# KarypisLab/SLIM

Measured on AMD Instinct MI355X. Metric: item-columns solved/sec (whole node), higher is better.
Workload: dtype f32

## Files before the change

### include/slim_gpu.h

```cpp
#ifndef SLIM_AMD_SLIM_GPU_H_
#define SLIM_AMD_SLIM_GPU_H_

#include "slim.h"

#ifdef __cplusplus
extern "C" {
#endif

typedef struct slim_csr_t {
  int32_t nrows, ncols;
  ssize_t *rowptr, *colptr;
  int32_t *rowind, *colind;
  int32_t *rowids, *colids;
  int32_t *rlabels, *clabels;
  int32_t *rmap, *cmap;
  float *rowval, *colval;
  float *rnorms, *cnorms;
  float *rsums, *csums;
  float *rsizes, *csizes;
  float *rvols, *cvols;
  float *rwgts, *cwgts;
} slim_csr_t;


// ... 61 lines not shown
                                           const int64_t *d_rowptr,
                                           const int32_t *d_rowind,
                                           const float *d_rowval,
                                           int32_t *ioptions, int32_t *r_status);
void SLIMGPU_MatrixFree(slimgpu_matrix_t **mat);
int32_t SLIMGPU_MatrixInfo(const slimgpu_matrix_t *mat, int32_t *nrows,
                           int32_t *ncols, int64_t *nnz);
int32_t SLIMGPU_MatrixGetColumnView(const slimgpu_matrix_t *mat, int64_t *colptr,
                                    int32_t *colind, float *colval,
                                    float *cnorms);

void SLIMGPU_MatrixExpectSolves(slimgpu_matrix_t *mat, int32_t nsolves);
int32_t SLIMGPU_MatrixDevice(const slimgpu_matrix_t *mat);

int32_t SLIMGPU_MatrixGramBuildRows(slimgpu_matrix_t *mat, int32_t row_begin, int32_t row_end);
int32_t SLIMGPU_MatrixGramView(slimgpu_matrix_t *mat, void **dptr, int64_t *ld, int32_t *nrows);
int32_t SLIMGPU_MatrixGramCommit(slimgpu_matrix_t *mat);

int32_t SLIMGPU_MatrixColumnCost(const slimgpu_matrix_t *mat, int64_t *cost);

slim_t *SLIMGPU_Learn(slimgpu_matrix_t *mat, int32_t *ioptions,
                      double *doptions, slim_t *imodel, int32_t *r_status);

slim_t *SLIMGPU_LearnColumns(slimgpu_matrix_t *mat, int32_t ncolumns,
                             const int32_t *columns, int32_t *ioptions,
                             double *doptions, slim_t *imodel, int32_t *r_status);

typedef struct slimgpu_model slimgpu_model_t;
slimgpu_model_t *SLIMGPU_LearnResident(slimgpu_matrix_t *mat, int32_t *ioptions, double *doptions,
                                       const slimgpu_model_t *warm, int32_t *r_status);
int64_t SLIMGPU_ModelNnz(const slimgpu_model_t *model);
int32_t SLIMGPU_ModelFetchBegin(slimgpu_model_t *model);
slim_t *SLIMGPU_ModelFetch(slimgpu_model_t *model, int32_t *r_status);
void SLIMGPU_ModelFree(slimgpu_model_t **model);
int32_t SLIMGPU_ModelPredict(int32_t nrcmds, const slimgpu_model_t *model, slim_t *trnhandle,
                             int32_t *output, float *scores);

int32_t SLIMGPU_Predict(int32_t nrcmds, slim_t *slimhandle, slim_t *trnhandle,
                        int32_t *output, float *scores);

int32_t SLIMGPU_Predict1vsK(int32_t nrcmds, int32_t nnegs, slim_t *slimhandle,
                            slim_t *trnhandle, int32_t *negitems, int32_t *output,
                            float *scores);

int32_t SLIMGPU_Evaluate(int32_t nusers, int32_t nrcmds, const int32_t *lists,
                         const int32_t *counts, slim_t *tsthandle,
                         const int32_t *fmarker, int32_t fm_ncols, double *metrics,
                         int32_t *nvalid);

typedef struct slimgpu_stats_t {
  int32_t ncols_solved;
  int32_t kernel;
  int32_t nwaves;
  int32_t lds_bytes;
  double setup_ms;
  double kernel_ms;
  double gather_ms;
  double total_ms;
  int64_t G, D, U, nnzW;
  int64_t sweeps;
  int64_t visits;
  double alg_bytes;
  double error, objval;
  double gram_build_ms;
  int64_t gram_rows;
  double gram_bytes;
  double gram_alloc_ms, gram_sums_ms, gram_sums_kernel_ms, gram_pack_ms;
} slimgpu_stats_t;
int32_t SLIMGPU_LastStats(slimgpu_stats_t *out);

int32_t SLIMGPU_LastColumnStats(int32_t ncols, int32_t *nacols, int32_t *sweeps,
                                int32_t *conv, int64_t *G, int64_t *D,
                                int64_t *U);

int32_t SLIMGPU_DeviceCount(void);
const char *SLIMGPU_LastError(void);

#ifdef __cplusplus
}
#endif

#include "slim_gpu_eval.h"
#include "slim_gpu_planes.h"
#include "slim_gpu_rank.h"
#include "slim_gpu_lists.h"
#include "slim_gpu_filter.h"
#include "slim_gpu_cand.h"

#endif
```

### slim_amd/_lib.py

```python
import ctypes as C
import os

import numpy as np

_HERE = os.path.dirname(os.path.abspath(__file__))
LIB_PATH = os.environ.get("SLIM_AMD_LIB") or os.path.join(_HERE, "libslim.so")

f64_1d = np.ctypeslib.ndpointer(dtype=np.float64, ndim=1, flags="C_CONTIGUOUS")
f32_1d = np.ctypeslib.ndpointer(dtype=np.float32, ndim=1, flags="C_CONTIGUOUS")
i32_1d = np.ctypeslib.ndpointer(dtype=np.int32, ndim=1, flags="C_CONTIGUOUS")
i64_1d = np.ctypeslib.ndpointer(dtype=np.int64, ndim=1, flags="C_CONTIGUOUS")
isz_1d = np.ctypeslib.ndpointer(dtype=np.intp, ndim=1, flags="C_CONTIGUOUS")


class Stats(C.Structure):
    _fields_ = [("ncols_solved", C.c_int32), ("kernel", C.c_int32), ("nwaves", C.c_int32),
                ("lds_bytes", C.c_int32), ("setup_ms", C.c_double), ("kernel_ms", C.c_double),
                ("gather_ms", C.c_double), ("total_ms", C.c_double),
                ("G", C.c_int64), ("D", C.c_int64), ("U", C.c_int64), ("nnzW", C.c_int64),
                ("sweeps", C.c_int64), ("visits", C.c_int64), ("alg_bytes", C.c_double),
                ("error", C.c_double), ("objval", C.c_double), ("gram_build_ms", C.c_double),
                ("gram_rows", C.c_int64), ("gram_bytes", C.c_double),
                ("gram_alloc_ms", C.c_double), ("gram_sums_ms", C.c_double),
                ("gram_sums_kernel_ms", C.c_double), ("gram_pack_ms", C.c_double)]

    def as_dict(self):
        return {k: getattr(self, k) for k, _ in self._fields_}


class EvalStats(C.Structure):
    _fields_ = [("path", C.c_int32), ("device_allocs", C.c_int32), ("h2d_bytes", C.c_int64),
                ("d2h_bytes", C.c_int64), ("kernel_ms", C.c_double), ("total_ms", C.c_double),
                ("w_rows_read", C.c_int64), ("w_bytes", C.c_double)]

    def as_dict(self):
        return {k: getattr(self, k) for k, _ in self._fields_}


class CsrView(C.Structure):
    _fields_ = ([("nrows", C.c_int32), ("ncols", C.c_int32),
                 ("rowptr", C.POINTER(C.c_ssize_t)), ("colptr", C.POINTER(C.c_ssize_t)),
                 ("rowind", C.POINTER(C.c_int32)), ("colind", C.POINTER(C.c_int32))] +
                [(n, C.POINTER(C.c_int32)) for n in
                 ("rowids", "colids", "rlabels", "clabels", "rmap", "cmap")] +
                [(n, C.POINTER(C.c_float)) for n in
                 ("rowval", "colval", "rnorms", "cnorms", "rsums", "csums", "rsizes",
                  "csizes", "rvols", "cvols", "rwgts", "cwgts")])


_SIGNATURES = {
    "SLIM_iSetDefaults": (C.c_int32, [i32_1d]),
    "SLIM_dSetDefaults": (C.c_int32, [f64_1d]),
    "SLIM_Learn": (C.c_void_p, [C.c_int32, isz_1d, i32_1d, C.c_void_p, C.c_void_p, C.c_void_p,
                                C.c_void_p, C.POINTER(C.c_int32)]),
    "SLIM_GetTopN": (C.c_int32, [C.c_void_p, C.c_int32, i32_1d, C.c_void_p, C.c_void_p,
                                 C.c_int32, i32_1d, f32_1d]),
    "SLIM_WriteModel": (C.c_int32, [C.c_void_p, C.c_char_p]),
    "SLIM_ReadModel": (C.c_void_p, [C.c_char_p]),
    "SLIM_FreeModel": (None, [C.POINTER(C.c_void_p)]),
    "SLIM_DetermineHeadAndTail": (C.POINTER(C.c_int32), [C.c_int32, C.c_int32, isz_1d, i32_1d]),
    "Py_csr_wrapper": (C.c_int32, [C.c_int32, isz_1d, i32_1d, C.c_void_p, C.c_void_p]),
    "Py_csr_save": (C.c_int32, [C.c_void_p, C.c_char_p]),
    "Py_csr_load": (C.c_int32, [C.c_void_p, C.c_char_p]),
    "Py_csr_free": (C.c_int32, [C.c_void_p]),
    "Py_csr_stat": (C.c_int32, [C.c_void_p, C.c_void_p]),
    "Py_csr_export": (C.c_int32, [C.c_void_p, i32_1d, i32_1d, f32_1d]),
    "Py_SLIM_Learn": (C.c_int32, [C.c_void_p, i32_1d, f64_1d, C.c_void_p]),
    "Py_SLIM_Mselect": (C.c_int32, [C.c_void_p, C.c_void_p, i32_1d, f64_1d, f64_1d, f64_1d,
                                    C.c_int32, C.c_int32] + [C.c_void_p] * 8),
    "Py_SLIM_GetTopN": (C.c_int32, [C.c_void_p, C.c_int32, i32_1d, C.c_void_p, C.c_int32,
                                    i32_1d, f32_1d, C.c_int32]),
    "Py_SLIM_GetTopN_1vsk": (C.c_int32, [C.c_void_p, C.c_int32, i32_1d, C.c_void_p, C.c_int32,
                                         i32_1d, f32_1d, C.c_int32, i32_1d, C.c_int32]),
    "Py_SLIM_Predict": (C.c_int32, [C.c_int32, C.c_void_p, C.c_void_p, i32_1d, f32_1d]),
    "Py_SLIM_Predict_1vsk": (C.c_int32, [C.c_int32, C.c_int32, C.c_void_p, C.c_void_p, i32_1d,
                                         i32_1d, f32_1d]),
    "SLIMGPU_MatrixFromHost": (C.c_void_p, [C.c_int32, isz_1d, i32_1d, C.c_void_p, C.c_void_p,
                                            C.POINTER(C.c_int32)]),
    "SLIMGPU_MatrixFromDevice": (C.c_void_p, [C.c_int32, C.c_int32, C.c_void_p, C.c_void_p,
                                              C.c_void_p, C.c_void_p, C.POINTER(C.c_int32)]),
    "SLIMGPU_MatrixFree": (None, [C.POINTER(C.c_void_p)]),
    "SLIMGPU_MatrixInfo": (C.c_int32, [C.c_void_p, C.POINTER(C.c_int32), C.POINTER(C.c_int32),
                                       C.POINTER(C.c_int64)]),
    "SLIMGPU_MatrixGetColumnView": (C.c_int32, [C.c_void_p] * 5),
    "SLIMGPU_MatrixColumnCost": (C.c_int32, [C.c_void_p, C.c_void_p]),
    "SLIMGPU_MatrixExpectSolves": (None, [C.c_void_p, C.c_int32]),
    "SLIMGPU_MatrixDevice": (C.c_int32, [C.c_void_p]),
    "SLIMGPU_MatrixGramBuildRows": (C.c_int32, [C.c_void_p, C.c_int32, C.c_int32]),
    "SLIMGPU_MatrixGramView": (C.c_int32, [C.c_void_p, C.POINTER(C.c_void_p), C.POINTER(C.c_int64),
                                           C.POINTER(C.c_int32)]),
    "SLIMGPU_MatrixGramCommit": (C.c_int32, [C.c_void_p]),
    "SLIMGPU_Learn": (C.c_void_p, [C.c_void_p, C.c_void_p, C.c_void_p, C.c_void_p,
                                   C.POINTER(C.c_int32)]),
    "SLIMGPU_LearnResident": (C.c_void_p, [C.c_void_p, C.c_void_p, C.c_void_p, C.c_void_p,
                                           C.POINTER(C.c_int32)]),
    "SLIMGPU_ModelNnz": (C.c_int64, [C.c_void_p]),
    "SLIMGPU_ModelFetchBegin": (C.c_int32, [C.c_void_p]),
    "SLIMGPU_ModelFetch": (C.c_void_p, [C.c_void_p, C.POINTER(C.c_int32)]),
    "SLIMGPU_ModelFree": (None, [C.POINTER(C.c_void_p)]),
    "SLIMGPU_ModelPredict": (C.c_int32, [C.c_int32, C.c_void_p, C.c_void_p, C.c_void_p, C.c_void_p]),
    "SLIMGPU_LearnColumns": (C.c_void_p, [C.c_void_p, C.c_int32, i32_1d, C.c_void_p, C.c_void_p,
                                          C.c_void_p, C.POINTER(C.c_int32)]),
    "SLIMGPU_Predict": (C.c_int32, [C.c_int32, C.c_void_p, C.c_void_p, i32_1d, f32_1d]),
    "SLIMGPU_Predict1vsK": (C.c_int32, [C.c_int32, C.c_int32, C.c_void_p, C.c_void_p, i32_1d,
                                        i32_1d, f32_1d]),
    "SLIMGPU_Evaluate": (C.c_int32, [C.c_int32, C.c_int32, i32_1d, i32_1d, C.c_void_p, i32_1d,
                                     C.c_int32, f64_1d, i32_1d]),
    "SLIMGPU_LastStats": (C.c_int32, [C.POINTER(Stats)]),
    "SLIMGPU_LastColumnStats": (C.c_int32, [C.c_int32] + [C.c_void_p] * 6),
    "SLIMGPU_DeviceCount": (C.c_int32, []),
    "SLIMGPU_LastError": (C.c_char_p, []),
}

EXPORTED_SYMBOLS = tuple(_SIGNATURES)

_EVAL_SIGNATURES = {
    "SLIMGPU_EvalSetCreate": (C.c_void_p, [C.c_void_p, C.c_void_p, i32_1d, C.c_int32, C.c_int32,
                                           C.POINTER(C.c_int32)]),
    "SLIMGPU_EvalSetFree": (None, [C.POINTER(C.c_void_p)]),
    "SLIMGPU_ModelEvaluate": (C.c_int32, [C.c_void_p, C.c_void_p, f64_1d, i32_1d]),
    "SLIMGPU_MatrixPredict": (C.c_int32, [C.c_int32, C.c_void_p, C.c_void_p, i32_1d, f32_1d]),
    "SLIMGPU_LastEvalStats": (C.c_int32, [C.POINTER(EvalStats)]),
}

EVAL_SYMBOLS = tuple(_EVAL_SIGNATURES)

_EVAL_AT_SIGNATURES = {
    "SLIMGPU_EvalSetCreateAt": (C.c_void_p, [C.c_void_p, C.c_void_p, i32_1d, C.c_int32, C.c_int32, C.c_void_p,
                                             C.c_int32, C.c_void_p, C.POINTER(C.c_int32)]),
    "SLIMGPU_ModelEvaluateAt": (C.c_int32, [C.c_void_p, C.c_void_p, C.c_int32, f64_1d, i32_1d]),
}

EVAL_AT_SYMBOLS = tuple(_EVAL_AT_SIGNATURES)


class GramPlanes(C.Structure):
    _fields_ = ([("ncols", C.c_int32), ("nchunks", C.c_int32), ("ldb", C.c_int64), ("hi_bytes", C.c_int64)] +
                [(n, C.c_void_p) for n in ("lo", "base", "hi", "hi_off", "hi_k", "hi2_k", "diag", "meta",
                                           "rank_of", "item_of")])


_PLANES_SIGNATURES = {
    "SLIMGPU_MatrixGramPlanes": (C.c_int32, [C.c_void_p, C.POINTER(GramPlanes)]),
}

PLANES_SYMBOLS = tuple(_PLANES_SIGNATURES)
MAX_CUTOFFS = 8

_RANK_SIGNATURES = {
    "SLIMGPU_EvalSetCreateRanked": (C.c_void_p, [C.c_void_p, C.c_void_p, i32_1d, C.c_int32, C.c_int32, C.c_void_p,
                                                 C.POINTER(C.c_int32)]),
    "SLIMGPU_EvalSetEntries": (C.c_int64, [C.c_void_p]),
    "SLIMGPU_ModelRanks": (C.c_int32, [C.c_void_p, C.c_void_p, C.c_void_p, C.c_void_p]),
    "SLIMGPU_ModelEvaluateRanked": (C.c_int32, [C.c_void_p, C.c_void_p, C.c_int32, C.c_void_p, f64_1d, i32_1d]),
    "SLIMGPU_ModelFromHost": (C.c_void_p, [C.c_void_p, C.c_void_p, C.POINTER(C.c_int32)]),
    "SLIMGPU_LastRankPrepassMs": (C.c_double, []),
}

RANK_SYMBOLS = tuple(_RANK_SIGNATURES)
MAX_RANK_CUTOFFS = 32


class ListStats(C.Structure):
    _fields_ = [("path", C.c_int32), ("slices", C.c_int32), ("candidates", C.c_int64), ("contenders", C.c_int64),
                ("refine_passes", C.c_int64), ("lds_sorts", C.c_int64), ("key_refines", C.c_int64)]

    def as_dict(self):
        return {k: getattr(self, k) for k, _ in self._fields_}


_LIST_SIGNATURES = {
    "SLIMGPU_PredictLists": (C.c_int32, [C.c_int32, C.c_void_p, C.c_void_p, C.c_void_p, C.c_void_p, C.c_void_p]),
    "SLIMGPU_ModelPredictLists": (C.c_int32, [C.c_int32, C.c_void_p, C.c_void_p, C.c_void_p, C.c_void_p,
                                              C.c_void_p]),
    "SLIMGPU_MatrixPredictLists": (C.c_int32, [C.c_int32, C.c_void_p, C.c_void_p, C.c_int32, C.c_void_p,
                                               C.c_void_p, C.c_void_p, C.c_void_p]),
    "SLIMGPU_LastListStats": (C.c_int32, [C.POINTER(ListStats)]),
}

LIST_SYMBOLS = tuple(_LIST_SIGNATURES)
MAX_LIST = 4096

_FILTER_SIGNATURES = {
    "SLIMGPU_FilterCreate": (C.c_int32, [C.c_int32, C.c_int32, C.c_void_p, C.c_int32, C.c_int32, C.c_void_p,
                                         C.c_void_p, C.POINTER(C.c_void_p)]),
    "SLIMGPU_FilterFree": (None, [C.c_void_p]),
    "SLIMGPU_PredictListsFiltered": (C.c_int32, [C.c_int32, C.c_void_p, C.c_void_p, C.c_void_p, C.c_void_p,
                                                 C.c_void_p, C.c_void_p]),
    "SLIMGPU_ModelPredictListsFiltered": (C.c_int32, [C.c_int32, C.c_void_p, C.c_void_p, C.c_void_p, C.c_void_p,
                                                      C.c_void_p, C.c_void_p]),
    "SLIMGPU_MatrixPredictListsFiltered": (C.c_int32, [C.c_int32, C.c_void_p, C.c_void_p, C.c_int32, C.c_void_p,
                                                       C.c_void_p, C.c_void_p, C.c_void_p, C.c_void_p]),
    "Py_SLIM_PredictFiltered": (C.c_int32, [C.c_int32, C.c_void_p, C.c_void_p, C.c_void_p, i32_1d, f32_1d]),
}

FILTER_SYMBOLS = tuple(_FILTER_SIGNATURES)

_FILTERED_EVAL_SIGNATURES = {
    "SLIMGPU_ModelEvaluateAtFiltered": (C.c_int32, [C.c_void_p, C.c_void_p, C.c_void_p, C.c_int32, f64_1d, i32_1d]),
    "SLIMGPU_ModelRanksFiltered": (C.c_int32, [C.c_void_p, C.c_void_p, C.c_void_p, C.c_void_p, C.c_void_p]),
    "SLIMGPU_ModelEvaluateRankedFiltered": (C.c_int32, [C.c_void_p, C.c_void_p, C.c_void_p, C.c_int32, C.c_void_p,
                                                        f64_1d, i32_1d]),
    "Py_SLIM_MselectFiltered": (C.c_int32, [C.c_void_p, C.c_void_p, i32_1d, f64_1d, f64_1d, f64_1d,
                                            C.c_int32, C.c_int32] + [C.c_void_p] * 9),
}

FILTERED_EVAL_SYMBOLS = tuple(_FILTERED_EVAL_SIGNATURES)

_CAND_SIGNATURES = {
    "SLIMGPU_CandSetCreate": (C.c_int32, [C.c_int32, C.c_int32, C.c_void_p, C.c_void_p, C.POINTER(C.c_void_p)]),
    "SLIMGPU_CandSetFree": (None, [C.c_void_p]),
    "SLIMGPU_ScoreCandidates": (C.c_int32, [C.c_void_p, C.c_void_p, C.c_void_p, C.c_int32, C.c_void_p, C.c_void_p,
                                            C.c_void_p, C.c_void_p]),
    "SLIMGPU_MatrixScoreCandidates": (C.c_int32, [C.c_void_p, C.c_void_p, C.c_void_p, C.c_int32, C.c_void_p,
                                                  C.c_int32, C.c_void_p, C.c_void_p, C.c_void_p, C.c_void_p]),
    "SLIMGPU_ModelEvaluateCandidates": (C.c_int32, [C.c_void_p, C.c_void_p, C.c_void_p, C.c_int32, f64_1d, i32_1d]),
    "Py_SLIM_ScoreCandidates": (C.c_int32, [C.c_void_p, C.c_void_p, C.c_void_p, C.c_int32, C.c_void_p, C.c_void_p,
                                            C.c_void_p, C.c_void_p]),
}

CAND_SYMBOLS = tuple(_CAND_SIGNATURES)

_SAMPLE_SIGNATURES = {
    "SLIMGPU_EvalSetSampleCandidates": (C.c_int32, [C.c_void_p, C.c_int32, C.c_uint64, C.POINTER(C.c_void_p)]),
    "SLIMGPU_CandSetSample": (C.c_int32, [C.c_int32, C.c_void_p, C.c_void_p, C.c_int32, C.c_void_p, C.c_int32,
                                          C.c_uint64, C.POINTER(C.c_void_p)]),
    "SLIMGPU_CandSetRows": (C.c_int32, [C.c_void_p, C.c_void_p, C.c_void_p]),
    "SLIMGPU_CandSetInfo": (C.c_int32, [C.c_void_p, C.POINTER(C.c_int32), C.POINTER(C.c_int32),
                                        C.POINTER(C.c_int64)]),
}

SAMPLE_SYMBOLS = tuple(_SAMPLE_SIGNATURES)

_WSAMPLE_SIGNATURES = {
    "SLIMGPU_EvalSetSampleCandidatesWeighted": (C.c_int32, [C.c_void_p, C.c_int32, C.c_uint64, C.c_void_p,
                                                            C.POINTER(C.c_void_p)]),
    "SLIMGPU_CandSetSampleWeighted": (C.c_int32, [C.c_int32, C.c_void_p, C.c_void_p, C.c_int32, C.c_void_p, C.c_int32,
                                                  C.c_uint64, C.c_void_p, C.POINTER(C.c_void_p)]),
    "SLIMGPU_LastSampleKernelMs": (C.c_double, []),
}

WSAMPLE_SYMBOLS = tuple(_WSAMPLE_SIGNATURES)

_EXPLAIN_SIGNATURES = {
    "SLIMGPU_ExplainCandidates": (C.c_int32, [C.c_void_p, C.c_void_p, C.c_void_p, C.c_int32, C.c_void_p, C.c_void_p,
                                              C.c_void_p]),
    "SLIMGPU_MatrixExplainCandidates": (C.c_int32, [C.c_void_p, C.c_void_p, C.c_void_p, C.c_int32, C.c_void_p,
                                                    C.c_int32, C.c_void_p, C.c_void_p, C.c_void_p]),
    "Py_SLIM_ExplainCandidates": (C.c_int32, [C.c_void_p, C.c_void_p, C.c_void_p, C.c_int32, C.c_void_p, C.c_void_p,
                                              C.c_void_p]),
}

EXPLAIN_SYMBOLS = tuple(_EXPLAIN_SIGNATURES)
MAX_WHY = 16

_lib = None


def load():
    global _lib
    if _lib is not None:
        return _lib
    if not os.path.exists(LIB_PATH):
        raise RuntimeError(
            "slim_amd: %s is missing -- build it with `python -c 'import __graft_entry__ as g; "
            "g.build()'` (hipcc, gfx950). There is no CPU fallback for SLIM training." % LIB_PATH)
    lib = C.CDLL(LIB_PATH)
    for name, (res, args) in (list(_SIGNATURES.items()) + list(_EVAL_SIGNATURES.items()) +
                              list(_EVAL_AT_SIGNATURES.items()) + list(_PLANES_SIGNATURES.items()) +
                              list(_RANK_SIGNATURES.items()) + list(_LIST_SIGNATURES.items()) +
                              list(_FILTER_SIGNATURES.items()) + list(_FILTERED_EVAL_SIGNATURES.items()) +
                              list(_CAND_SIGNATURES.items()) + list(_SAMPLE_SIGNATURES.items()) +
                              list(_WSAMPLE_SIGNATURES.items()) + list(_EXPLAIN_SIGNATURES.items())):
        if os.environ.get("SLIM_AMD_LIB") and not hasattr(lib, name):
            continue
        fn = getattr(lib, name)
        fn.restype = res
        fn.argtypes = args
    _lib = lib
    return lib


def last_error():
    msg = load().SLIMGPU_LastError()
    return msg.decode("utf-8", "replace") if msg else ""
```

### slim_amd/csrc/admm.hip

```cpp
#include <dlfcn.h>
#include <hip/hip_runtime.h>

#include <cstdio>
#include <cstdlib>
#include <chrono>
#include <cstring>
#include <mutex>
#include <string>
#include <vector>

#include "engine.hpp"
#include "hip_check.hpp"
#include "host_csr.hpp"

namespace slimamd {

namespace {

struct DenseLibs {
  void* blas = nullptr;
  int (*create_handle)(void**) = nullptr;
  int (*destroy_handle)(void*) = nullptr;
  int (*set_stream)(void*, hipStream_t) = nullptr;
  int (*dgemm)(void*, int, int, int, int, int, const double*, const double*, int, const double*,
// ... 134 lines not shown
  const int64_t nwaves = ((int64_t)gridDim.x * blockDim.x) >> 6;
  for (int64_t i = wave; i < m; i += nwaves) {
    int64_t n = 0;
    for (int j = lane; j < m; j += 64) n += W[i * m + j] > 0.0 ? 1 : 0;
    for (int off = 32; off > 0; off >>= 1) n += __shfl_xor(n, off);
    if (lane == 0) cnt[i] = n;
  }
}

__global__ void k_emit_rows(int32_t m, const double* __restrict__ W, const int64_t* __restrict__ ptr,
                            int32_t* __restrict__ ind, float* __restrict__ val) {
  const int lane = threadIdx.x & 63;
  const uint64_t lane_lt = (1ull << lane) - 1ull;
  const int64_t wave = ((int64_t)blockIdx.x * blockDim.x + threadIdx.x) >> 6;
  const int64_t nwaves = ((int64_t)gridDim.x * blockDim.x) >> 6;
  for (int64_t i = wave; i < m; i += nwaves) {
    int64_t at = ptr[i];
    for (int jb = 0; jb < m; jb += 64) {
      const int j = jb + lane;
      const double w = j < m ? W[i * m + j] : 0.0;
      const uint64_t mask = __ballot(w > 0.0);
      if (w > 0.0) {
        const int64_t dst = at + __popcll(mask & lane_lt);
        ind[dst] = j;
        val[dst] = (float)w;
      }
      at += __popcll(mask);
    }
  }
}

int grid_for(int64_t n, int block, int cap) {
  int64_t g = (n + block - 1) / block;
  if (g < 1) g = 1;
  if (g > cap) g = cap;
  return (int)g;
}

}

slim_csr_t* learn_admm(int32_t nrows, const ssize_t* rowptr, const int32_t* rowind,
                       const float* rowval, const LearnOptions& opt, int32_t* status) {
  auto fail = [&](int32_t code, const std::string& msg) -> slim_csr_t* {
    set_error(msg);
    if (status) *status = code;
    return nullptr;
  };
  if (nrows < 0 || !rowptr || (rowptr[nrows] > 0 && !rowind))
    return fail(SLIM_ERROR_INPUT, "SLIM_Learn(admm): bad CSR arguments");
  const int64_t nnz = rowptr[nrows];
  int32_t m = max_index_plus_one(nnz, rowind);
  if (m <= 0) m = 1;
  for (int64_t k = 0; k < nnz; ++k)
    if (rowind[k] < 0) return fail(SLIM_ERROR_INPUT, "SLIM_Learn(admm): negative item id");
  const int64_t n2 = (int64_t)m * m;
  {
    std::vector<int32_t> seen((size_t)m, -1);
    for (int32_t u = 0; u < nrows; ++u) {
      if (rowptr[u] > rowptr[u + 1] || rowptr[u] < 0 || rowptr[u + 1] > nnz)
        return fail(SLIM_ERROR_INPUT, "SLIM_Learn(admm): rowptr is not a non-decreasing offset array ending at nnz");
      for (ssize_t k = rowptr[u]; k < rowptr[u + 1]; ++k) {
        if (seen[(size_t)rowind[k]] == u)
          return fail(SLIM_ERROR_INPUT, "SLIM_Learn(admm): duplicate (user, item) entries in the rating matrix");
        seen[(size_t)rowind[k]] = u;
      }
    }
  }
  std::printf("Learning the model using ADMM... \n");
  std::fflush(stdout);
  const bool trace = std::getenv("SLIM_GPU_TRACE") != nullptr;
  const auto t_begin = std::chrono::steady_clock::now();
  auto mark = [&](const char* what) {
    if (trace)
      std::fprintf(stderr, "[trace] admm %-28s %8.1f ms\n", what,
                   std::chrono::duration<double, std::milli>(std::chrono::steady_clock::now() - t_begin).count());
  };
  try {
    (void)hipGetLastError();
    int ndev = 0;
    HIP_TRY(hipGetDeviceCount(&ndev));
    if (ndev <= 0) throw HipFail{hipErrorNoDevice, "hipGetDeviceCount"};
    if (opt.device >= 0) HIP_TRY(hipSetDevice(opt.device));
    size_t free_b = 0, total_b = 0;
    HIP_TRY(hipMemGetInfo(&free_b, &total_b));
    if ((double)n2 * 8.0 * 6.5 > (double)free_b)
      return fail(SLIM_ERROR_MEMORY, "SLIM_Learn(admm): six " + std::to_string(m) + " x " +
                                         std::to_string(m) + " fp64 matrices do not fit this GPU");
    static DenseLibs libs;
    static std::once_flag once;
    static bool loaded = false;
    static std::string load_err;
    std::call_once(once, [&]() { loaded = libs.load(&load_err); });
    if (!loaded) return fail(SLIM_ERROR, "SLIM_Learn: " + load_err);
    mark("libraries resolved");
    hipDeviceProp_t prop;
    int dev = 0;
    HIP_TRY(hipGetDevice(&dev));
    HIP_TRY(hipGetDeviceProperties(&prop, dev));
    const int cap = prop.multiProcessorCount * 8;
    hipStream_t st = nullptr;
    HIP_TRY(hipStreamCreateWithFlags(&st, hipStreamNonBlocking));
    void* handle = nullptr;
    if (libs.create_handle(&handle) != 0) {
      (void)hipStreamDestroy(st);
      return fail(SLIM_ERROR, "SLIM_Learn(admm): rocblas_create_handle failed");
    }
    libs.set_stream(handle, st);
    mark("rocblas handle");
    struct Cleanup {
      DenseLibs& l;
      void* h;
      hipStream_t s;
      ~Cleanup() {
        l.destroy_handle(h);
        (void)hipStreamDestroy(s);
      }
    } cleanup{libs, handle, st};

    DeviceBuffer<int64_t> d_ptr((size_t)nrows + 1), d_cnt((size_t)m + 1);
    DeviceBuffer<int32_t> d_ind((size_t)nnz), d_info(1);
    DeviceBuffer<float> d_val(rowval ? (size_t)nnz : 1);
    static_assert(sizeof(ssize_t) == sizeof(int64_t), "LP64 expected");
    HIP_TRY(hipMemcpyAsync(d_ptr.get(), rowptr, sizeof(int64_t) * ((size_t)nrows + 1), hipMemcpyHostToDevice, st));
    if (nnz) {
      HIP_TRY(hipMemcpyAsync(d_ind.get(), rowind, sizeof(int32_t) * (size_t)nnz, hipMemcpyHostToDevice, st));
      if (rowval)
        HIP_TRY(hipMemcpyAsync(d_val.get(), rowval, sizeof(float) * (size_t)nnz, hipMemcpyHostToDevice, st));
    }
    DeviceBuffer<double> T((size_t)n2), A((size_t)n2), P((size_t)n2), W((size_t)n2), C((size_t)n2), gam((size_t)m);
    HIP_TRY(hipMemsetAsync(T.get(), 0, sizeof(double) * (size_t)n2, st));
    HIP_TRY(hipMemsetAsync(W.get(), 0, sizeof(double) * (size_t)n2, st));
    HIP_TRY(hipMemsetAsync(C.get(), 0, sizeof(double) * (size_t)n2, st));

    const double rho = 10000.0;
    const int maxiters = 30;
    hipLaunchKernelGGL(k_gram_dense, dim3(grid_for((int64_t)nrows * 64, 256, cap)), dim3(256), 0, st,
                       nrows, m, d_ptr.get(), d_ind.get(), rowval ? d_val.get() : nullptr, T.get());
    HIP_TRY(hipGetLastError());
    hipLaunchKernelGGL(k_copy_add_diag, dim3(grid_for(n2, 256, cap)), dim3(256), 0, st, n2, m, T.get(), P.get(),
                       opt.l2r + rho);
    HIP_TRY(hipGetLastError());
    const double one = 1.0, zero = 0.0, minus_one = -1.0;
    HIP_TRY(hipMemsetAsync(d_info.get(), 0, sizeof(int32_t), st));
    for (int32_t k = 0; k < m; k += kNB) {
      const int32_t kb = std::min(kNB, m - k), rest = m - k - kb;
      double* Akk = P.get() + (int64_t)k * m + k;
      hipLaunchKernelGGL(k_potf2, dim3(1), dim3(kNB), 0, st, kb, k, m, Akk, d_info.get());
      if (rest > 0) {
        double* A21 = Akk + kb;
        double* A22 = Akk + (int64_t)kb * m + kb;
        if (libs.dtrsm(handle, kSideRight, kFillLower, kOpTrans, kNonUnit, rest, kb, &one, Akk, m, A21, m) != 0 ||
            libs.dsyrk(handle, kFillLower, kOpNone, rest, kb, &minus_one, A21, m, &one, A22, m) != 0)
          return fail(SLIM_ERROR, "SLIM_Learn(admm): rocBLAS dtrsm / dsyrk failed");
      }
    }
    HIP_TRY(hipGetLastError());
    int32_t info = 0;
    HIP_TRY(hipMemcpyAsync(&info, d_info.get(), sizeof(int32_t), hipMemcpyDeviceToHost, st));
    HIP_TRY(hipStreamSynchronize(st));
    if (info != 0) return fail(SLIM_ERROR, "SLIM_Learn(admm): R^T R + (l2 + rho) I is not positive definite");
    mark("R^T R + Cholesky");
    hipLaunchKernelGGL(k_identity, dim3(grid_for(n2, 256, cap)), dim3(256), 0, st, n2, m, W.get());
    if (libs.dtrsm(handle, kSideLeft, kFillLower, kOpNone, kNonUnit, m, m, &one, P.get(), m, W.get(), m) != 0 ||
        libs.dgemm(handle, kOpTrans, kOpNone, m, m, m, &one, W.get(), m, W.get(), m, &zero, P.get(), m) != 0)
      return fail(SLIM_ERROR, "SLIM_Learn(admm): rocBLAS dtrsm / dgemm failed");
    HIP_TRY(hipMemsetAsync(W.get(), 0, sizeof(double) * (size_t)n2, st));
    hipLaunchKernelGGL(k_symmetrize, dim3(grid_for(n2, 256, cap)), dim3(256), 0, st, m, P.get());
// ... 59 lines not shown
```

### slim_amd/csrc/engine.hip

```cpp
#include <hip/hip_runtime.h>

#include <algorithm>
#include <atomic>
#include <chrono>
#include <cmath>
#include <cstdio>
#include <cstdlib>
#include <cstring>
#include <functional>
#include <mutex>
#include <new>
#include <numeric>
#include <memory>
#include <string>
#include <thread>

#include <rocprim/device/device_radix_sort.hpp>

#include "tile_inst.hpp"
#include "gram_inst.hpp"
#include "gramr_inst.hpp"
#include "gram_sym.hpp"
#include "fslim_gram_inst.hpp"
#include "cd_wave.hpp"
#include "engine.hpp"
#include "hip_check.hpp"
#include "host_csr.hpp"

inline uint64_t slimgpu_next_uid() {
  static std::atomic<uint64_t> n{0};
  return ++n;
}

using slimamd::DeviceBuffer;

struct UserSplit {
  DeviceBuffer<int32_t> ubounds;
  DeviceBuffer<int64_t> csplit;
  int32_t nranges = 0, max_rows = 0;
};

struct slimgpu_matrix {
  const uint64_t uid = slimgpu_next_uid();
  int device = 0;
  hipStream_t stream = nullptr;
  int32_t nrows = 0, ncols = 0;
  int64_t nnz = 0;
  bool binary = false;
  bool owns_csr = false;
  bool exact_gram = false;
  bool nonpositive = false;
  bool merged = false;
  int64_t* d_rowptr = nullptr;
  int32_t* d_rowind = nullptr;
  float* d_rowval = nullptr;
  DeviceBuffer<int64_t> d_colptr;
  DeviceBuffer<int32_t> d_colind;
  DeviceBuffer<float> d_colval, d_cnorm, d_csq;
  std::vector<int64_t> h_cost;
  std::vector<int64_t> h_rowptr;
  UserSplit split[6];
  UserSplit gsplit;
  double setup_ms = 0;
  int num_cus = 256;
  std::vector<slimgpu_matrix*> replicas;
  DeviceBuffer<float> ws_gram;
  std::vector<int32_t> gram_order;
  int gram_geom[6] = {0, 0, 0, 0, 0, 0};
  DeviceBuffer<float> ws_G;
  DeviceBuffer<int32_t> ws_nunion;
  int64_t G_ld = 0;
  bool G_ready = false;
  double G_build_ms = 0, G_alloc_ms = 0, G_sums_ms = 0, G_sums_kernel_ms = 0, G_pack_ms = 0;
  DeviceBuffer<uint8_t> ws_Glo, ws_Ghi, ws_Gbase;
  DeviceBuffer<float> ws_Gdiag;
  DeviceBuffer<uint4> ws_Gmeta;
  DeviceBuffer<int64_t> ws_hioff, ws_hi2off;
  DeviceBuffer<int32_t> ws_hik, ws_hi2k, ws_rankof, ws_itemof;
  int64_t Gp_ldb = 0, Gp_pool_bytes = 0;
  int32_t Gp_nchunks = 0;
  bool Gp_ready = false, Gp_tried = false;
  bool Gf_dropped = false;
  double Gp_bytes_per_row = 0;
  int expect_solves = 0;
  std::vector<int32_t> last_order;
  DeviceBuffer<int32_t> ws_order, ws_cnt, ws_stat_i, ws_misc, ws_arena_i, ws_ulist;
  DeviceBuffer<int64_t> ws_off, ws_stat_l, ws_icolptr;
  DeviceBuffer<float> ws_stat_f, ws_arena_v, ws_slab, ws_xslab, ws_part, ws_icolval;
  DeviceBuffer<int32_t> ws_fn, ws_fid, ws_fslot;
  DeviceBuffer<float> ws_faty;
  DeviceBuffer<uint64_t> ws_trace;
  DeviceBuffer<uint4> ws_gview;
  DeviceBuffer<int64_t> ws_gvbase;
  DeviceBuffer<int32_t> ws_gvrows;
  DeviceBuffer<uint16_t> ws_gvcnt;
  DeviceBuffer<unsigned long long> ws_mailbox;
  DeviceBuffer<int32_t> ws_icolind;
  DeviceBuffer<uint32_t> ws_tkeys[2];
  DeviceBuffer<uint64_t> ws_tpay[2];
  DeviceBuffer<uint8_t> ws_ttmp;

  ~slimgpu_matrix() {
    (void)hipSetDevice(device);
    if (owns_csr) {
      (void)hipFree(d_rowptr);
      (void)hipFree(d_rowind);
      (void)hipFree(d_rowval);
    }
  }
};

struct slimgpu_model {
  int device = 0;
  int32_t n = 0;
  int64_t nnz = 0;
  int32_t max_row = 0;
  bool rows_sorted = true;
  DeviceBuffer<int64_t> d_colptr, d_rowptr;
  DeviceBuffer<int32_t> d_colind, d_rowind;
  DeviceBuffer<float> d_colval, d_rowval;
  mutable DeviceBuffer<float> d_gsave;
  mutable bool gsave_valid = false;
  int64_t gsave_stride = 0;
  double gsave_l1 = 0;
  uint64_t gsave_owner = 0;
  std::thread fetcher;
  bool fetch_begun = false;
  slim_csr_t* fetched = nullptr;
  int32_t fetch_status = 0;
  std::string fetch_error;
  double fetch_ms = 0;

  ~slimgpu_model() { (void)hipSetDevice(device); }
};

namespace slimamd {

namespace {

thread_local slimgpu_stats_t g_stats;
thread_local ColumnStats g_colstats;

struct InputError {
  std::string msg;
};

double now_ms() {
  using namespace std::chrono;
  return duration<double, std::milli>(steady_clock::now().time_since_epoch()).count();
}

void report(const HipFail& e, const char* what) {
  set_error(std::string(what) + ": HIP error '" + hipGetErrorString(e.code) + "' in " + e.where +
            " -- the SLIM CD path needs a gfx950 GPU; there is no CPU fallback");
}

void drop_screen_cache(slimgpu_matrix* m) {
  m->ws_gram.reset();
  m->gram_order.clear();
}

auto evict_cache(slimgpu_matrix* m) {
  return [m] {
    if (!m->ws_gram.get()) return false;
    drop_screen_cache(m);
    return true;
  };
}


__global__ void k_gview_rows(const int32_t* __restrict__ order, int32_t nwork, const int64_t* __restrict__ csplit,
                             int32_t stride, int32_t ngroups, int32_t nblocks, int32_t* __restrict__ rows,
                             uint16_t* __restrict__ cnt) {
  const int b = (int)blockIdx.x * ((int)blockDim.x >> 6) + ((int)threadIdx.x >> 6);
  if (b >= nblocks) return;
  const int r = b / ngroups, pl = (b % ngroups) * 64 + ((int)threadIdx.x & 63);
  int len = 0;
  if (pl < nwork) {
    const int64_t* const c = csplit + (int64_t)order[pl] * stride + r;
    len = (int)(c[1] - c[0]);
  }
  int n = (len + 7) >> 3;
  cnt[(int64_t)b * 64 + (threadIdx.x & 63)] = (uint16_t)n;
  for (int off = 32; off > 0; off >>= 1) n += __shfl_xor(n, off);
  if ((threadIdx.x & 63) == 0) rows[b] = n;
}

__global__ void k_gview_fill(const int32_t* __restrict__ order, int32_t nwork, const int64_t* __restrict__ csplit,
                             int32_t stride, const int32_t* __restrict__ ubounds, const int32_t* __restrict__ ci,
                             int32_t ngroups, int32_t nblocks, const int64_t* __restrict__ base, uint32_t sentinel,
                             uint4* __restrict__ view) {
  const int b = (int)blockIdx.x * ((int)blockDim.x >> 6) + ((int)threadIdx.x >> 6);
  if (b >= nblocks) return;
  const int lane = (int)threadIdx.x & 63;
  const int r = b / ngroups, pl = (b % ngroups) * 64 + lane;
  const int64_t end = base[b + 1];
  const int32_t u0 = ubounds[r];
  int64_t cs = 0;
  int len = 0;
  if (pl < nwork) {
    const int64_t* const c = csplit + (int64_t)order[pl] * stride + r;
    cs = c[0];
    len = (int)(c[1] - cs);
  }
  int64_t at = base[b];
  for (int c = 0;; ++c) {
    const bool mine = 8 * c < len;
    const uint64_t who = __ballot(mine);
    if (who == 0ull) break;
    if (mine) {
      const int64_t slot = at + __popcll(who & ((1ull << lane) - 1ull));
      uint32_t id[8];
#pragma unroll
      for (int j = 0; j < 8; ++j) id[j] = 8 * c + j < len ? (uint32_t)(ci[cs + 8 * c + j] - u0) : sentinel;
      if (slot < end)
        view[slot] = make_uint4(id[0] | (id[1] << 16), id[2] | (id[3] << 16), id[4] | (id[5] << 16),
                                id[6] | (id[7] << 16));
    }
    at += __popcll(who);
  }
}


__global__ void k_max_index(const int32_t* __restrict__ ind, int64_t n, int32_t* out) {
  int32_t m = -1;
  for (int64_t k = (int64_t)blockIdx.x * blockDim.x + threadIdx.x; k < n;
       k += (int64_t)gridDim.x * blockDim.x)
    m = max(m, ind[k]);
  for (int off = 32; off > 0; off >>= 1) m = max(m, __shfl_xor(m, off));
  if ((threadIdx.x & 63) == 0) atomicMax(out, m);
}

constexpr int kBadRowptr = 1;
constexpr int kBadColumn = 2;
constexpr int kDupEntry = 4;

__global__ void k_pack_rows(int32_t nrows, int32_t ncols, int64_t nnz,
// ... 255 lines not shown
}

void ensure_split(slimgpu_matrix* m, UserSplit& s, int nr, bool even_share) {
  if (s.nranges == nr) return;
  s.ubounds.reset();
  s.csplit.reset();
  s.nranges = 0;
  std::vector<int32_t> ub((size_t)nr + 1, 0);
  ub[(size_t)nr] = m->nrows;
  if (nr > 1) {
    if (m->h_rowptr.empty()) {
      m->h_rowptr.resize((size_t)m->nrows + 1);
      HIP_TRY(hipMemcpy(m->h_rowptr.data(), m->d_rowptr, sizeof(int64_t) * ((size_t)m->nrows + 1),
                        hipMemcpyDeviceToHost));
    }
    for (int j = 1; j < nr; ++j) {
      const int64_t want = even_share ? m->nnz / nr * j : (int64_t)((double)m->nnz / nr * j);
      ub[(size_t)j] = (int32_t)(std::lower_bound(m->h_rowptr.begin(), m->h_rowptr.end(), want) -
                                m->h_rowptr.begin());
      ub[(size_t)j] = std::min(std::max(ub[(size_t)j], ub[(size_t)j - 1]), m->nrows);
    }
  }
  int32_t mx = 1;
  for (int j = 0; j < nr; ++j) mx = std::max(mx, ub[(size_t)j + 1] - ub[(size_t)j]);
  s.max_rows = mx;
  s.ubounds = DeviceBuffer<int32_t>((size_t)nr + 1);
  HIP_TRY(hipMemcpy(s.ubounds.get(), ub.data(), sizeof(int32_t) * ((size_t)nr + 1), hipMemcpyHostToDevice));
  s.csplit = DeviceBuffer<int64_t>((size_t)m->ncols * ((size_t)nr + 1));
  hipLaunchKernelGGL(k_col_split, dim3(grid_for((int64_t)m->ncols * (nr + 1), 256, m->num_cus * 8)), dim3(256), 0,
                     m->stream, m->ncols, nr, s.ubounds.get(), m->d_colptr.get(), m->d_colind.get(),
                     s.csplit.get());
  HIP_TRY(hipGetLastError());
  HIP_TRY(hipStreamSynchronize(m->stream));
  s.nranges = nr;
}

void ensure_cluster_split(slimgpu_matrix* m, int lg) { ensure_split(m, m->split[lg], 1 << lg, true); }

void destroy(slimgpu_matrix* m) {
  if (!m) return;
  for (slimgpu_matrix* r : m->replicas) destroy(r);
  (void)hipSetDevice(m->device);
  if (m->stream) (void)hipStreamDestroy(m->stream);
  delete m;
}

}

slimgpu_stats_t& last_stats() { return g_stats; }
ColumnStats& last_column_stats() { return g_colstats; }

LearnOptions decode_options(const int32_t* io, const double* dopt) {
  LearnOptions o;
  auto geti = [&](int idx, int32_t def) { return (!io || io[idx] == -1) ? def : io[idx]; };
  auto getd = [&](int idx, double def) { return (!dopt || dopt[idx] == -1) ? def : dopt[idx]; };
  o.nthreads = geti(SLIM_OPTION_NTHREADS, 1);
  o.nnbrs = geti(SLIM_OPTION_NNBRS, 0);
  o.simtype = geti(SLIM_OPTION_SIMTYPE, SLIM_SIMTYPE_COS);
  o.dbglvl = geti(SLIM_OPTION_DBGLVL, 0);
  o.algo = geti(SLIM_OPTION_ALGO, SLIM_ALGO_CD);
  o.ordered = geti(SLIM_OPTION_ORDERED, 0);
  o.maxniters = geti(SLIM_OPTION_MAXNITERS, 10000);
  o.l1r = getd(SLIM_OPTION_L1R, 1.0);
  o.l2r = getd(SLIM_OPTION_L2R, 1.0);
  o.optTol = getd(SLIM_OPTION_OPTTOL, 1e-7);
  o.col_begin = geti(SLIM_OPTION_GPU_COLBEGIN, 0);
  o.col_end = geti(SLIM_OPTION_GPU_COLEND, -1);
  o.seed = (uint32_t)geti(SLIM_OPTION_GPU_SEED, 1);
  o.device = geti(SLIM_OPTION_GPU_DEVICE, -1);
  o.kernel = geti(SLIM_OPTION_GPU_KERNEL, SLIMGPU_KERNEL_AUTO);
  o.cluster = geti(SLIM_OPTION_GPU_CLUSTER, 0);
  o.heavy_tiles = geti(SLIM_OPTION_GPU_HEAVYTILES, -1);
  o.heavy_cluster = geti(SLIM_OPTION_GPU_HEAVYCLUSTER, 0);
  o.ngpus = std::max(1, geti(SLIM_OPTION_GPU_NGPUS, 1));
  o.shard_count = std::max(1, geti(SLIM_OPTION_GPU_SHARDCOUNT, 1));
  o.shard_index = geti(SLIM_OPTION_GPU_SHARDINDEX, 0);
  return o;
}

int32_t device_count() {
  int n = 0;
  if (hipGetDeviceCount(&n) != hipSuccess) return 0;
  return n;
}

namespace {
template <class Fill>
slimgpu_matrix_t* make_matrix(const char* who, int32_t* status, Fill&& fill) {
  slimgpu_matrix* m = nullptr;
  try {
    m = new slimgpu_matrix();
    fill(m);
    if (status) *status = SLIM_OK;
    return m;
  } catch (const HipFail& e) {
    report(e, who);
    if (status) *status = status_of(e);
  } catch (const InputError& e) {
    set_error(std::string(who) + ": " + e.msg);
    if (status) *status = SLIM_ERROR_INPUT;
  } catch (const std::bad_alloc&) {
    set_error(std::string(who) + ": out of host memory");
    if (status) *status = SLIM_ERROR_MEMORY;
  }
  destroy(m);
  return nullptr;
}
}

slimgpu_matrix_t* matrix_from_host(int32_t nrows, const ssize_t* rowptr, const int32_t* rowind,
                                   const float* rowval, const LearnOptions& opt,
                                   int32_t* status) {
  if (nrows < 0 || !rowptr || (rowptr[nrows] > 0 && !rowind)) {
    set_error("SLIMGPU_MatrixFromHost: bad CSR arguments");
    if (status) *status = SLIM_ERROR_INPUT;
    return nullptr;
  }
  const double t0 = now_ms();
  std::vector<int64_t> mptr;
  std::vector<int32_t> mind;
  std::vector<float> mval;
  try {
  if (const char* e = std::getenv("SLIM_GPU_DUPLICATES"); e && std::strcmp(e, "sum") == 0 && nrows > 0) {
    bool any = false;
    std::vector<std::pair<int32_t, float>> row;
    mptr.assign((size_t)nrows + 1, 0);
    mind.reserve((size_t)rowptr[nrows]);
    if (rowval) mval.reserve((size_t)rowptr[nrows]);
    for (int32_t u = 0; u < nrows; ++u) {
      const int64_t s0 = rowptr[u], e0 = rowptr[u + 1];
      row.clear();
      for (int64_t k = s0; k < e0; ++k) row.emplace_back(rowind[k], rowval ? rowval[k] : 1.0f);
      bool sorted = true;
      for (size_t k = 1; k < row.size(); ++k) sorted = sorted && row[k - 1].first < row[k].first;
      if (!sorted) {
        std::stable_sort(row.begin(), row.end(),
                         [](const auto& a, const auto& b) { return a.first < b.first; });
        size_t w = 0;
        for (size_t k = 0; k < row.size(); ++k) {
          if (w > 0 && row[w - 1].first == row[k].first) {
            if (rowval) row[w - 1].second += row[k].second;
            any = true;
          } else {
            row[w++] = row[k];
          }
        }
        row.resize(w);
      }
      for (const auto& pr : row) {
        mind.push_back(pr.first);
        if (rowval) mval.push_back(pr.second);
      }
      mptr[(size_t)u + 1] = (int64_t)mind.size();
    }
    if (any) {
      rowptr = reinterpret_cast<const ssize_t*>(mptr.data());
      rowind = mind.data();
      if (rowval) rowval = mval.data();
    }
  }
  } catch (const std::bad_alloc&) {
    set_error("SLIMGPU_MatrixFromHost: out of host memory while merging repeated pairs");
    if (status) *status = SLIM_ERROR_MEMORY;
    return nullptr;
  }
  return make_matrix("SLIMGPU_MatrixFromHost", status, [&](slimgpu_matrix* m) {
    pick_device(m, opt);
    m->nrows = nrows;
    m->nnz = rowptr[nrows];
    m->binary = rowval == nullptr;
    m->merged = !mptr.empty() && rowptr == reinterpret_cast<const ssize_t*>(mptr.data());
    m->ncols = max_index_plus_one(m->nnz, rowind);
    if (m->ncols <= 0) m->ncols = 1;
    m->owns_csr = true;
    m->d_rowptr = DeviceBuffer<int64_t>((size_t)nrows + 1).release();
    m->d_rowind = DeviceBuffer<int32_t>((size_t)m->nnz).release();
    m->d_rowval = m->binary ? nullptr : DeviceBuffer<float>((size_t)m->nnz).release();
    static_assert(sizeof(ssize_t) == sizeof(int64_t), "LP64 expected");
    HIP_TRY(hipMemcpyAsync(m->d_rowptr, rowptr, sizeof(int64_t) * ((size_t)nrows + 1),
                           hipMemcpyHostToDevice, m->stream));
    if (m->nnz > 0) {
      HIP_TRY(hipMemcpyAsync(m->d_rowind, rowind, sizeof(int32_t) * (size_t)m->nnz,
                             hipMemcpyHostToDevice, m->stream));
      if (!m->binary)
        HIP_TRY(hipMemcpyAsync(m->d_rowval, rowval, sizeof(float) * (size_t)m->nnz,
                               hipMemcpyHostToDevice, m->stream));
    }
    build_column_view(m);
    m->setup_ms = now_ms() - t0;
  });
}

slimgpu_matrix_t* matrix_from_device(int32_t nrows, int32_t ncols, const int64_t* d_rowptr,
                                     const int32_t* d_rowind, const float* d_rowval,
                                     const LearnOptions& opt, int32_t* status) {
  if (nrows < 0 || !d_rowptr) {
    set_error("SLIMGPU_MatrixFromDevice: bad CSR arguments");
    if (status) *status = SLIM_ERROR_INPUT;
    return nullptr;
  }
  const double t0 = now_ms();
  return make_matrix("SLIMGPU_MatrixFromDevice", status, [&](slimgpu_matrix* m) {
    pick_device(m, opt);
    m->nrows = nrows;
    m->owns_csr = false;
    m->d_rowptr = const_cast<int64_t*>(d_rowptr);
    m->d_rowind = const_cast<int32_t*>(d_rowind);
    m->d_rowval = const_cast<float*>(d_rowval);
    m->binary = d_rowval == nullptr;
    HIP_TRY(hipMemcpy(&m->nnz, d_rowptr + nrows, sizeof(int64_t), hipMemcpyDeviceToHost));
    if (ncols <= 0) {
      DeviceBuffer<int32_t> d_max(1);
      int32_t init = -1;
      HIP_TRY(hipMemcpy(d_max.get(), &init, sizeof(int32_t), hipMemcpyHostToDevice));
      if (m->nnz > 0) {
        hipLaunchKernelGGL(k_max_index, dim3(grid_for(m->nnz, 256, m->num_cus * 8)), dim3(256), 0,
                           m->stream, m->d_rowind, m->nnz, d_max.get());
        HIP_TRY(hipGetLastError());
        HIP_TRY(hipStreamSynchronize(m->stream));
      }
      HIP_TRY(hipMemcpy(&init, d_max.get(), sizeof(int32_t), hipMemcpyDeviceToHost));
      ncols = init + 1;
    }
    m->ncols = ncols > 0 ? ncols : 1;
    build_column_view(m);
    m->setup_ms = now_ms() - t0;
  });
}

void matrix_free(slimgpu_matrix_t* m) { destroy(m); }

slimgpu_matrix_t* matrix_clone_to_device(const slimgpu_matrix_t* src, int32_t device,
                                         int32_t* status) {
  const double t0 = now_ms();
  return make_matrix("SLIMGPU_MatrixFromHost (device-to-device copy of the staged matrix)", status,
                     [&](slimgpu_matrix* m) {
    (void)hipGetLastError();
    LearnOptions o;
    o.device = device;
    pick_device(m, o);
    m->nrows = src->nrows;
    m->ncols = src->ncols;
    m->nnz = src->nnz;
    m->binary = src->binary;
    m->exact_gram = src->exact_gram;
    m->nonpositive = src->nonpositive;
    m->merged = src->merged;
    m->owns_csr = true;
    m->h_cost = src->h_cost;
    const size_t nz = (size_t)std::max<int64_t>(m->nnz, 1);
    m->d_rowptr = DeviceBuffer<int64_t>((size_t)m->nrows + 1).release();
    m->d_rowind = DeviceBuffer<int32_t>(nz).release();
    m->d_rowval = m->binary ? nullptr : DeviceBuffer<float>(nz).release();
    m->d_colptr = DeviceBuffer<int64_t>((size_t)m->ncols + 1);
    m->d_colind = DeviceBuffer<int32_t>(nz + 64);
    if (!m->binary) m->d_colval = DeviceBuffer<float>(nz);
    m->d_cnorm = DeviceBuffer<float>((size_t)m->ncols);
    m->d_csq = DeviceBuffer<float>((size_t)m->ncols);
    int can_peer = m->device == src->device ? 1 : 0;
    if (!can_peer) {
      if (hipDeviceCanAccessPeer(&can_peer, m->device, src->device) != hipSuccess) can_peer = 0;
      (void)hipGetLastError();
    }
    if (const char* e = std::getenv("SLIM_GPU_PEER")) can_peer = can_peer && std::atoi(e) != 0;
    void* bounce = nullptr;
    const size_t bounce_bytes = size_t(256) << 20;
    struct BounceFree {
      void** p;
      ~BounceFree() {
        if (*p) (void)hipHostFree(*p);
      }
    } bounce_guard{&bounce};
    auto peer = [&](void* dst, const void* from, size_t bytes) {
      if (bytes == 0 || !dst || !from) return;
      if (can_peer) {
        HIP_TRY(hipMemcpyPeerAsync(dst, m->device, from, src->device, bytes, m->stream));
        return;
      }
      if (!bounce) HIP_TRY(hipHostMalloc(&bounce, bounce_bytes, hipHostMallocDefault));
      for (size_t off = 0; off < bytes; off += bounce_bytes) {
        const size_t n = std::min(bounce_bytes, bytes - off);
        HIP_TRY(hipSetDevice(src->device));
        HIP_TRY(hipMemcpy(bounce, static_cast<const char*>(from) + off, n, hipMemcpyDeviceToHost));
        HIP_TRY(hipSetDevice(m->device));
        HIP_TRY(hipMemcpy(static_cast<char*>(dst) + off, bounce, n, hipMemcpyHostToDevice));
      }
    };
    peer(m->d_rowptr, src->d_rowptr, sizeof(int64_t) * ((size_t)m->nrows + 1));
    peer(m->d_colptr.get(), src->d_colptr.get(), sizeof(int64_t) * ((size_t)m->ncols + 1));
    peer(m->d_cnorm.get(), src->d_cnorm.get(), sizeof(float) * (size_t)m->ncols);
    peer(m->d_csq.get(), src->d_csq.get(), sizeof(float) * (size_t)m->ncols);
    if (m->nnz > 0) {
      peer(m->d_rowind, src->d_rowind, sizeof(int32_t) * (size_t)m->nnz);
      peer(m->d_colind.get(), src->d_colind.get(), sizeof(int32_t) * (size_t)m->nnz);
      peer(m->d_rowval, src->d_rowval, sizeof(float) * (size_t)m->nnz);
      peer(m->d_colval.get(), src->d_colval.get(), sizeof(float) * (size_t)m->nnz);
    }
    HIP_TRY(hipStreamSynchronize(m->stream));
    m->setup_ms = now_ms() - t0;
  });
}

void matrix_add_replica(slimgpu_matrix_t* m, slimgpu_matrix_t* replica) {
  m->replicas.push_back(replica);
}
const std::vector<slimgpu_matrix_t*>& matrix_replicas(const slimgpu_matrix_t* m) {
  return m->replicas;
}
void matrix_adopt_csr(slimgpu_matrix_t* m) { m->owns_csr = true; }
int32_t matrix_device(const slimgpu_matrix_t* m) { return m ? m->device : -1; }
void matrix_set_setup_ms(slimgpu_matrix_t* m, double ms) { m->setup_ms = ms; }

int32_t matrix_info(const slimgpu_matrix_t* m, int32_t* nrows, int32_t* ncols, int64_t* nnz) {
  if (!m) return SLIM_ERROR_INPUT;
  if (nrows) *nrows = m->nrows;
  if (ncols) *ncols = m->ncols;
  if (nnz) *nnz = m->nnz;
  return SLIM_OK;
}

double matrix_setup_ms(const slimgpu_matrix_t* m) { return m ? m->setup_ms : 0.0; }

void matrix_expect_solves(slimgpu_matrix_t* m, int32_t n) {
  if (!m) return;
  m->expect_solves = n;
  for (slimgpu_matrix* r : m->replicas) r->expect_solves = n;
}

int32_t matrix_column_cost(const slimgpu_matrix_t* m, int64_t* cost) {
  if (!m || !cost) return SLIM_ERROR_INPUT;
  std::memcpy(cost, m->h_cost.data(), sizeof(int64_t) * m->h_cost.size());
  return SLIM_OK;
}

int32_t matrix_get_column_view(const slimgpu_matrix_t* m, int64_t* colptr, int32_t* colind,
                               float* colval, float* cnorms) {
// ... 23 lines not shown
namespace {

KernelFn pick_kernel(bool lds, bool has_val) {
  if (lds) return has_val ? cd_wave_kernel<true, true> : cd_wave_kernel<true, false>;
  return has_val ? cd_wave_kernel<false, true> : cd_wave_kernel<false, false>;
}

int round_up(int v, int q) { return (v + q - 1) / q * q; }

bool test_hook(const char* name) {
  const char* master = std::getenv("SLIM_GPU_TEST_HOOKS");
  return master && std::atoi(master) == 1 && std::getenv(name) != nullptr;
}

constexpr int kBitmapBytes = 64 * 1024;

}

namespace {

bool pack_gram(slimgpu_matrix* m) {
  if (std::getenv("SLIM_GPU_NO_GRAMR")) return false;
  m->Gp_tried = true;
  const int32_t ncols = m->ncols;
  hipStream_t st = m->stream;
  const double t0 = now_ms();
  std::vector<int64_t> cp((size_t)ncols + 1);
  HIP_TRY(hipMemcpy(cp.data(), m->d_colptr.get(), sizeof(int64_t) * cp.size(), hipMemcpyDeviceToHost));
  const int32_t nchunks = (ncols + 15) / 16;
  static_assert(kGramrMaxGroups <= 15 && kGramrMaxGroups * kPackGroup <= (1 << 17),
                "row record: 17 bits of rank, 4 bits per plane length; base bytes: 16 groups per thread");
  if ((nchunks + kGramrNT - 1) / kGramrNT > kGramrMaxGroups) return false;
  std::vector<int32_t> item_of((size_t)nchunks * 16, -1), rank_of((size_t)ncols);
  std::iota(item_of.begin(), item_of.begin() + ncols, 0);
  std::stable_sort(item_of.begin(), item_of.begin() + ncols, [&](int32_t a, int32_t b) {
    return cp[(size_t)a + 1] - cp[(size_t)a] > cp[(size_t)b + 1] - cp[(size_t)b];
  });
  for (int32_t r = 0; r < ncols; ++r) rank_of[(size_t)item_of[(size_t)r]] = r;
  int32_t* d_item_of = m->ws_itemof.reserve(item_of.size());
  int32_t* d_rank_of = m->ws_rankof.reserve(rank_of.size());
  HIP_TRY(hipMemcpyAsync(d_item_of, item_of.data(), sizeof(int32_t) * item_of.size(), hipMemcpyHostToDevice, st));
  HIP_TRY(hipMemcpyAsync(d_rank_of, rank_of.data(), sizeof(int32_t) * rank_of.size(), hipMemcpyHostToDevice, st));
  int32_t* d_hik = m->ws_hik.reserve((size_t)ncols + 1);
  int32_t* d_hi2k = m->ws_hi2k.reserve((size_t)ncols);
  int32_t* d_flag = d_hik + ncols;
  HIP_TRY(hipMemsetAsync(d_flag, 0, sizeof(int32_t), st));
  const float* dG = m->ws_G.get();
  int use_base = 1;
  if (const char* e = std::getenv("SLIM_GPU_PACK_BASE")) use_base = std::atoi(e) != 0;
  bool gather = false;
  if (const char* e = std::getenv("SLIM_GPU_PACK_GATHER")) gather = std::atoi(e) != 0;
  const dim3 tgrid(kGramrNT / kPackTS, (ncols + kPackJT - 1) / kPackJT);
  if (gather) {
    hipLaunchKernelGGL(gram_pack_scan_fn(), dim3(ncols), dim3(256), 0, st, dG, m->G_ld, ncols, d_item_of, nchunks,
                       use_base, d_hik, d_hi2k, d_flag);
    HIP_TRY(hipGetLastError());
  } else {
    HIP_TRY(hipMemsetAsync(d_hik, 0xff, sizeof(int32_t) * (size_t)ncols, st));
    HIP_TRY(hipMemsetAsync(d_hi2k, 0xff, sizeof(int32_t) * (size_t)ncols, st));
    hipLaunchKernelGGL(gram_pack_scan_t_fn(), tgrid, dim3(256), 0, st, dG, m->G_ld, ncols, d_item_of, d_rank_of,
                       nchunks, use_base, d_hik, d_hi2k, d_flag);
    HIP_TRY(hipGetLastError());
    hipLaunchKernelGGL(gram_pack_groups_fn(), dim3((ncols + 255) / 256), dim3(256), 0, st, ncols, d_hik, d_hi2k);
    HIP_TRY(hipGetLastError());
  }
  std::vector<int32_t> hk((size_t)ncols + 1), h2k((size_t)ncols);
  HIP_TRY(hipMemcpyAsync(hk.data(), d_hik, sizeof(int32_t) * hk.size(), hipMemcpyDeviceToHost, st));
  HIP_TRY(hipMemcpyAsync(h2k.data(), d_hi2k, sizeof(int32_t) * h2k.size(), hipMemcpyDeviceToHost, st));
  HIP_TRY(hipStreamSynchronize(st));
  if (hk[(size_t)ncols] != 0) return false;
  std::vector<int64_t> off1((size_t)ncols), off2((size_t)ncols);
  int64_t n1 = 0, n2 = 0, npool = 0;
  for (int32_t i = 0; i < ncols; ++i) {
    off1[(size_t)i] = npool;
    npool += (int64_t)hk[(size_t)i] * kPackGroup;
    off2[(size_t)i] = npool;
    npool += (int64_t)h2k[(size_t)i] * kPackGroup;
    n1 += (int64_t)hk[(size_t)i] * kPackGroup;
    n2 += (int64_t)h2k[(size_t)i] * kPackGroup;
  }
  const int64_t ldb = (int64_t)nchunks * 16;
  const size_t need = (size_t)ncols * ((size_t)ldb + kPackGroup) + (size_t)n1 + (size_t)n2 + 2 * (size_t)kPackGroup;
  size_t free_b = 0, total_b = 0;
  HIP_TRY(hipMemGetInfo(&free_b, &total_b));
  if (need + (size_t(4) << 30) > free_b + m->ws_Glo.bytes() + m->ws_Ghi.bytes() + m->ws_Gbase.bytes()) return false;
  uint8_t* d_lo = m->ws_Glo.reserve((size_t)ncols * (size_t)ldb);
  uint8_t* d_hi = m->ws_Ghi.reserve((size_t)npool + kPackGroup);
  uint8_t* d_hi2 = d_hi;
  uint8_t* d_base = m->ws_Gbase.reserve((size_t)ncols * kPackGroup);
  if (gather) {
    HIP_TRY(hipMemsetAsync(d_base, 0, (size_t)ncols * kPackGroup, st));
  }
  float* d_diag = m->ws_Gdiag.reserve((size_t)ncols);
  HIP_TRY(hipMemsetAsync(d_diag, 0, sizeof(float) * (size_t)ncols, st));
  int64_t* d_off1 = m->ws_hioff.reserve((size_t)ncols);
  int64_t* d_off2 = m->ws_hi2off.reserve((size_t)ncols);
  HIP_TRY(hipMemcpyAsync(d_off1, off1.data(), sizeof(int64_t) * off1.size(), hipMemcpyHostToDevice, st));
  HIP_TRY(hipMemcpyAsync(d_off2, off2.data(), sizeof(int64_t) * off2.size(), hipMemcpyHostToDevice, st));
  HIP_TRY(hipMemsetAsync(d_hi + npool, 0, kPackGroup, st));
  if (gather) {
    hipLaunchKernelGGL(gram_pack_write_fn(), dim3(ncols), dim3(256), 0, st, dG, m->G_ld, ncols, d_item_of, nchunks,
                       d_lo, ldb, d_hi, d_off1, d_hik, d_hi2, d_off2, d_hi2k, d_base, d_diag);
  } else {
    hipLaunchKernelGGL(gram_pack_write_t_fn(), tgrid, dim3(256), 0, st, dG, m->G_ld, ncols, d_item_of, d_rank_of,
                       nchunks, d_lo, ldb, d_hi, d_off1, d_hik, d_hi2, d_off2, d_hi2k, d_base, d_diag);
  }
  HIP_TRY(hipGetLastError());
  uint4* d_meta = m->ws_Gmeta.reserve((size_t)ncols);
  hipLaunchKernelGGL(gram_pack_meta_fn(), dim3((ncols + 255) / 256), dim3(256), 0, st, ncols, d_rank_of, d_hik,
                     d_hi2k, d_off1, d_diag, m->d_colptr.get(), m->d_csq.get(), m->d_cnorm.get(), d_meta, d_flag);
  HIP_TRY(hipGetLastError());
  int32_t meta_flag = 0;
  HIP_TRY(hipMemcpyAsync(&meta_flag, d_flag, sizeof(int32_t), hipMemcpyDeviceToHost, st));
  HIP_TRY(hipStreamSynchronize(st));
  if (meta_flag & 2) return false;
  m->Gp_ldb = ldb;
  m->Gp_pool_bytes = npool + kPackGroup;
  m->Gp_nchunks = nchunks;
  m->Gp_bytes_per_row = (double)ldb + 16.0 * std::min(nchunks, kGramrNT) + (double)(n1 + n2) / std::max(1, ncols);
  m->Gp_ready = true;
  if (const char* te = std::getenv("SLIM_GPU_TRACE"); te && std::atoi(te) >= 1)
    std::fprintf(stderr, "[trace] G packed (%s): lo %.2f GB + base %.2f GB + hi %.2f GB + hi2 %.3f GB = %.3f bytes per entry, %.1f ms\n",
                 gather ? "gathers" : "streamed tiles", (double)ncols * ldb * 1e-9, (double)ncols * kPackGroup * 1e-9, n1 * 1e-9, n2 * 1e-9,
                 m->Gp_bytes_per_row / std::max(1, ncols), now_ms() - t0);
  return true;
}

void drop_float_gram(slimgpu_matrix* m) {
  if (!m->Gp_ready || !m->ws_G.get() || std::getenv("SLIM_GPU_KEEP_G") || std::getenv("SLIM_GPU_NO_GRAMR")) return;
  if ((m->Gp_nchunks + kGramrNT - 1) / kGramrNT > kGramrMaxGroups) return;
  double min_gb = 8.0;
  if (const char* e = std::getenv("SLIM_GPU_DROP_G_MIN_GB")) min_gb = std::atof(e);
  if ((double)m->ws_G.bytes() < min_gb * 1073741824.0) return;
  (void)hipStreamSynchronize(m->stream);
  m->ws_G.reset();
  m->Gf_dropped = true;
}


struct Refusal {
  int32_t status;
  std::string msg;
};

int64_t gram_ld(int32_t ncols) { return round_up(round_up(ncols, 64), 64); }

struct WorkList {
  std::vector<int32_t> order;
  int32_t G_block = 0;
};

WorkList work_list(const slimgpu_matrix* m, const LearnOptions& opt, const int32_t* columns,
                   int32_t ncolumns) {
  const int32_t ncols = m->ncols;
  WorkList w;
  if (columns) {
    std::vector<char> seen((size_t)ncols, 0);
    for (int32_t k = 0; k < ncolumns; ++k) {
      if (columns[k] < 0 || columns[k] >= ncols || seen[(size_t)columns[k]])
        throw Refusal{SLIM_ERROR_INPUT, "SLIMGPU_LearnColumns: column ids must be distinct and inside [0, ncols)"};
      seen[(size_t)columns[k]] = 1;
    }
    w.order.assign(columns, columns + ncolumns);
  } else {
    int32_t cb = std::max(0, opt.col_begin);
    const int32_t ce = opt.col_end < 0 ? ncols : std::min(opt.col_end, ncols);
    if (cb > ce) cb = ce;
    w.order.resize((size_t)(ce - cb));
    std::iota(w.order.begin(), w.order.end(), cb);
  }
  if (opt.shard_index < 0 || opt.shard_index >= opt.shard_count)
    throw Refusal{SLIM_ERROR_INPUT, "SLIMGPU_Learn: shard index outside [0, shard count)"};
  std::vector<int32_t>& order = w.order;
  std::stable_sort(order.begin(), order.end(),
                   [&](int32_t a, int32_t b) { return m->h_cost[a] > m->h_cost[b]; });
  if (opt.shard_count > 1) {
    std::vector<int32_t> mine;
    for (int32_t t = 0; t < (int32_t)order.size(); ++t)
      if ((t / 32) % opt.shard_count == opt.shard_index) mine.push_back(order[(size_t)t]);
    order.swap(mine);
  }
  if (opt.build_G && opt.G_rows_end >= 0) {
    auto in_block = [&](int32_t c) { return c >= opt.G_rows_begin && c < opt.G_rows_end; };
    std::stable_partition(order.begin(), order.end(), in_block);
    w.G_block = (int32_t)std::count_if(order.begin(), order.end(), in_block);
  }
  return w;
}

int32_t build_gram(slimgpu_matrix* m, LearnOptions bo, bool zero_first, double* alloc_ms = nullptr) {
  if (zero_first) {
    const double t0 = now_ms();
    const int64_t G_ld = gram_ld(m->ncols);
    drop_screen_cache(m);
    float* dG = m->ws_G.reserve((size_t)m->ncols * (size_t)G_ld);
    if (alloc_ms) *alloc_ms = now_ms() - t0;
    HIP_TRY(hipMemsetAsync(dG, 0, sizeof(float) * (size_t)m->ncols * (size_t)G_ld, m->stream));
    m->G_ld = G_ld;
  }
  if (bo.G_rows_end >= 0 && bo.G_rows_begin == bo.G_rows_end) return SLIM_OK;
  bo.kernel = SLIMGPU_KERNEL_TILE;
  bo.build_G = true;
  bo.heavy_tiles = 0;
  int32_t st = SLIM_OK;
  if (slim_csr_t* none = learn_cd(m, bo, nullptr, &st, nullptr, 0, false)) csr_free(none);
  return st;
}

struct Path {
  int kernel = 0;
  bool use_gram = false, use_gramr = false, use_tile = false, use_lds = false;
  int nrows_pad = 0, ncols_pad = 0;
  size_t vec_floats = 0, lds_need = 0;
  int gram_nw = 0, gram_v = 0;
  GramrFn fn_r = nullptr;
  int gramr_kr = 0, gramr_kl = 0;
  size_t gram_lds = 0;
  KernelFn fn = nullptr;
  int tileP = 32, tileNW = 16;
  int req_cluster = 0;
  size_t gram_bits_lds = 0;
  size_t gram_stage_lds = 0;
  const char* gram_stage_why = "";
  int gram_passes = 1;
  int wg_slots = 0;
  int nwaves = 1;
  int trace_level = 0;
  bool has_imodel = false;
  bool exact_gram = false;
  bool use_fgram = false, f_block = false;
  int f_stride = 0, f_ustride = 0, f_tab_n = 0, f_waves = 1;
  size_t f_wave_lds = 0, f_union_lds = 0;
  FslimFn fn_f = nullptr;
};

Path choose_kernel(slimgpu_matrix* m, const LearnOptions& opt, int32_t nwork) {
  const int32_t ncols = m->ncols;
  Path p;
  p.nrows_pad = round_up(std::max(m->nrows, 1), 64);
  p.ncols_pad = round_up(ncols, 64);
  p.vec_floats = (size_t)p.nrows_pad + 2 * (size_t)p.ncols_pad;
  p.lds_need = p.vec_floats * sizeof(float);
  p.kernel = opt.kernel;
  const bool gram_fits =
      gram_geometry(p.ncols_pad, &p.gram_nw, &p.gram_v) && opt.nnbrs == 0 && !opt.build_G && ncols > 0;
  const size_t G_bytes = sizeof(float) * (size_t)ncols * (size_t)gram_ld(ncols);
  if (p.kernel == SLIMGPU_KERNEL_GRAM_FSLIM) {
    if (opt.nnbrs <= 0 || opt.build_G)
      throw Refusal{SLIM_ERROR_INPUT, "SLIMGPU_Learn: the item-space FSLIM kernel needs nnbrs > 0"};
    if (m->nonpositive)
      throw Refusal{SLIM_ERROR_INPUT, "SLIMGPU_Learn: the item-space FSLIM kernel needs ratings > 0: with a rating <= 0 "
                                      "a co-rating sum can cancel to 0 and G cannot mark the column as co-rated "
                                      "(the tile kernel solves such matrices)"};
    if (std::min(opt.nnbrs, ncols - 1) > kFslimMaxNbrs)
      throw Refusal{SLIM_ERROR_INPUT, "SLIMGPU_Learn: the item-space FSLIM kernel holds at most 4096 neighbours per "
                                      "problem in LDS (min(nnbrs, ncols - 1) is larger)"};
    if (m->G_ready && m->Gf_dropped) {
      m->G_ready = false;
      m->Gf_dropped = false;
    }
    size_t free_b = 0, total_b = 0;
    HIP_TRY(hipMemGetInfo(&free_b, &total_b));
    if (!m->G_ready && G_bytes + (size_t(4) << 30) > free_b + m->ws_gram.bytes())
      throw Refusal{SLIM_ERROR_MEMORY, "SLIMGPU_Learn: G = R^T R (4 ncols^2 bytes) does not fit the free HBM"};
    p.use_fgram = true;
    return p;
  }
  if (p.kernel == SLIMGPU_KERNEL_GRAM) {
    if (!gram_fits) throw Refusal{SLIM_ERROR_INPUT, "SLIMGPU_Learn: the item-space kernel has no FSLIM form"};
    size_t free_b = 0, total_b = 0;
    HIP_TRY(hipMemGetInfo(&free_b, &total_b));
    if (!m->G_ready && G_bytes + (size_t(4) << 30) > free_b + m->ws_gram.bytes())
      throw Refusal{SLIM_ERROR_MEMORY, "SLIMGPU_Learn: G = R^T R (4 ncols^2 bytes) does not fit the free HBM"};
    p.use_gram = true;
  } else if (p.kernel == SLIMGPU_KERNEL_AUTO && gram_fits && p.lds_need > 64 * 1024 &&
             !std::getenv("SLIM_GPU_NO_GRAMCD")) {
    const double rho = (double)ncols * (double)ncols / std::max(1.0, (double)m->nnz) / 45.0;
    const double solves = (double)std::max(1, m->expect_solves);
    const bool tile_geometry_asked = opt.cluster != 0 || opt.heavy_tiles >= 0 || opt.heavy_cluster != 0;
    bool item_space = rho < 1.0 && !tile_geometry_asked &&
                      (m->G_ready || (double)nwork * solves * (1.0 - rho) > (double)ncols / 32.0);
    if (const char* e = std::getenv("SLIM_GPU_GRAMCD"); e && std::strcmp(e, "never-first") == 0)
      item_space = item_space && (m->G_ready || m->expect_solves >= 2);
    if (item_space) {
      size_t free_b = 0, total_b = 0;
      HIP_TRY(hipMemGetInfo(&free_b, &total_b));
      p.use_gram = m->G_ready || G_bytes + (size_t(8) << 30) <= free_b + m->ws_gram.bytes();
    }
  }
  if (p.use_gram) p.kernel = SLIMGPU_KERNEL_GRAM;
  if (p.use_gram && m->G_ready && m->Gf_dropped && std::getenv("SLIM_GPU_NO_GRAMR")) {
    m->G_ready = false;
    m->Gf_dropped = false;
  }
  return p;
}

int32_t gram_for_solve(slimgpu_matrix* m, const LearnOptions& opt, int32_t trace_level, bool floats_only) {
  const double tb = now_ms();
  LearnOptions bo = opt;
  bo.col_begin = 0;
  bo.col_end = -1;
  bo.shard_count = 1;
  bo.shard_index = 0;
  bo.nnbrs = 0;
  bo.cluster = 0;
  bo.dbglvl = 0;
  double alloc_ms = 0;
  const int32_t st = build_gram(m, bo, true, &alloc_ms);
  if (st != SLIM_OK) return st;
  const double t_sums = now_ms();
  const double sums_kernel_ms = last_stats().kernel_ms;
  m->G_ready = true;
  m->Gf_dropped = false;
  if (!floats_only) {
    if (!m->Gp_ready) {
      m->Gp_tried = false;
      if (!pack_gram(m)) m->Gp_ready = false;
    }
    drop_float_gram(m);
  }
  m->G_build_ms = now_ms() - tb;
  m->G_alloc_ms = alloc_ms;
  m->G_sums_ms = t_sums - tb - alloc_ms;
  m->G_sums_kernel_ms = sums_kernel_ms;
  m->G_pack_ms = now_ms() - t_sums;
  if (trace_level >= 1)
    std::fprintf(stderr, "[trace] G = R^T R (%d x %d, %.2f GB) built in %.1f ms: allocation %.1f, sums %.1f "
                 "(kernel %.1f), byte planes %.1f\n", m->ncols, m->ncols,
                 sizeof(float) * (double)m->ncols * (double)m->G_ld * 1e-9, m->G_build_ms, m->G_alloc_ms,
                 m->G_sums_ms, sums_kernel_ms, m->G_pack_ms);
  return SLIM_OK;
}

void finish_path(slimgpu_matrix* m, const LearnOptions& opt, int32_t nwork, const slim_csr_t* imodel,
                 const slimgpu_model* warm_dev, Path& p) {
  p.exact_gram = m->exact_gram || std::getenv("SLIM_GPU_EXACT_GRAM") || (opt.nnbrs > 0 && m->nonpositive);
  if (p.kernel == SLIMGPU_KERNEL_AUTO)
    p.kernel = p.lds_need <= 64 * 1024 ? SLIMGPU_KERNEL_WAVE_LDS : SLIMGPU_KERNEL_TILE;
  if (p.kernel == SLIMGPU_KERNEL_WAVE_LDS && p.lds_need > 160 * 1024)
    throw Refusal{SLIM_ERROR_INPUT, "SLIMGPU_Learn: work vectors do not fit the 160 KiB LDS of a CU"};
  if (p.kernel < SLIMGPU_KERNEL_WAVE_LDS || p.kernel > SLIMGPU_KERNEL_GRAM_FSLIM)
    throw Refusal{SLIM_ERROR_INPUT, "SLIMGPU_Learn: unknown kernel selection"};
  if (p.use_fgram) {
    p.f_stride = std::max(64, round_up(std::min(opt.nnbrs, m->ncols - 1), 64));
    p.f_ustride = (int)std::min<int64_t>((int64_t)32 * p.f_stride, p.ncols_pad);
    p.f_block = p.f_stride <= kFslimBlockMaxStride;
    if (const char* e = std::getenv("SLIM_GPU_FSLIM_BLOCK")) p.f_block = p.f_block && std::atoi(e) != 0;
    p.f_tab_n = p.f_block ? round_up(p.f_ustride, 8) : 0;
    p.f_wave_lds = fslim_wave_lds(p.f_stride, p.f_block, p.f_tab_n);
    p.f_waves = (int)std::max<size_t>(1, std::min<size_t>(p.f_block ? kFslimMaxWaves : 4, (size_t(150) << 10) / p.f_wave_lds));
    p.fn_f = fslim_solve_fn(p.f_block);
    p.f_union_lds = fslim_union_lds(m->ncols);
    if (p.f_union_lds > (size_t(150) << 10))
      throw Refusal{SLIM_ERROR_INPUT, "SLIMGPU_Learn: the item-space FSLIM kernel's item bitmap does not fit the LDS of a CU"};
    HIP_TRY(hipFuncSetAttribute(reinterpret_cast<const void*>(fslim_union_fn()),
                                hipFuncAttributeMaxDynamicSharedMemorySize, (int)p.f_union_lds));
    const size_t lds = p.f_wave_lds * (size_t)p.f_waves;
    int per_cu = 0;
    HIP_TRY(hipFuncSetAttribute(reinterpret_cast<const void*>(p.fn_f), hipFuncAttributeMaxDynamicSharedMemorySize, (int)lds));
    HIP_TRY(hipOccupancyMaxActiveBlocksPerMultiprocessor(&per_cu, reinterpret_cast<const void*>(p.fn_f), 64 * p.f_waves, lds));
    if (per_cu < 1)
      throw Refusal{SLIM_ERROR, "SLIMGPU_Learn: the item-space FSLIM kernel does not fit a compute unit of this device"};
    p.nwaves = std::max(1, std::min((nwork + p.f_waves - 1) / p.f_waves, m->num_cus * per_cu));
    if (warm_dev && warm_dev->device != m->device)
      throw Refusal{SLIM_ERROR_INPUT, "SLIMGPU_LearnResident: the warm-start model lives on another device"};
    p.has_imodel = false;
    if (p.trace_level >= 1)
      std::fprintf(stderr, "[trace] item-space FSLIM: form %s, lists of %d, %d wavefronts per workgroup (%zu KB of LDS "
// ... 155 lines not shown
                                      hipFuncAttributeMaxDynamicSharedMemorySize, (int)stage));
          HIP_TRY(hipOccupancyMaxActiveBlocksPerMultiprocessor(&per_cu_s, reinterpret_cast<const void*>(p.fn),
                                                               64 * p.tileNW, stage));
        }
        if (per_cu_s >= std::min(per_cu, 16 / p.tileNW)) {
          p.gram_stage_lds = stage;
          per_cu = per_cu_s;
        } else {
          p.gram_stage_why = "no room in LDS";
        }
      } else {
        p.gram_stage_lds = stage;
      }
    }
    if (per_cu < 1)
      throw Refusal{SLIM_ERROR, "SLIMGPU_Learn: the tile kernel does not fit a compute unit of this device"};
    p.wg_slots = m->num_cus * std::min(per_cu, 16 / p.tileNW);
  }
}

struct TileGeom {
  bool force_k1 = false;
  int clusterK = 1, cluster_lg = 0, nclusters = 0;
  int clusterHi = 0, hi_lg = 0, nheavy = 0, nclusters_hi = 0;
  size_t tile_r = 0, tile_x = 0, tile_u = 0;
  int nwaves = 0;
};

TileGeom plan_tiles(slimgpu_matrix* m, const LearnOptions& opt, const Path& p,
                    const std::vector<int32_t>& order, bool force_k1) {
  const int32_t ncols = m->ncols, nwork = (int32_t)order.size();
  const int tileP = p.tileP;
  TileGeom t;
  t.force_k1 = force_k1;
  int auto_heavy = 0;
  const int ngroups_all = (nwork + tileP - 1) / tileP;
  const int req = p.req_cluster;
  if (force_k1) {
    t.clusterK = 1;
  } else if (req == 1 || req == 2 || req == 4 || req == 8 || req == 16 || req == 32) {
    t.clusterK = req;
  } else {
    int cap = 1;
    while (cap < 16 && (m->nnz / std::max(ncols, 1)) / (2 * cap) >= 512) cap *= 2;
    if (opt.heavy_tiles < 0 && p.tileNW == 16 && ngroups_all >= 16) {
      auto tile_cost = [&](int gI) {
        int64_t c = 0;
        for (int k = gI * tileP; k < std::min((gI + 1) * tileP, nwork); ++k) c += m->h_cost[order[(size_t)k]];
        return c;
      };
      const int64_t med = tile_cost(ngroups_all / 2);
      while (auto_heavy < ngroups_all / 16 && tile_cost(auto_heavy) >= 12 * med) ++auto_heavy;
    }
    const int64_t fill = auto_heavy > 0 ? 4 : 8;
    while (t.clusterK < cap && (int64_t)ngroups_all * t.clusterK < fill * (int64_t)p.wg_slots) t.clusterK *= 2;
  }
  while (t.clusterK > 1 && p.wg_slots / t.clusterK < 1) t.clusterK /= 2;
  for (t.cluster_lg = 0; (1 << t.cluster_lg) < t.clusterK; ++t.cluster_lg) {}
  ensure_cluster_split(m, t.cluster_lg);
  t.tile_r = (size_t)(round_up(m->split[t.cluster_lg].max_rows, 64) + 64) * tileP;
  if (opt.build_G && p.gram_bits_lds && t.clusterK == 32 && !force_k1) t.tile_r = (size_t)64 * tileP;
  t.tile_x = (size_t)p.ncols_pad * tileP;
  t.tile_u = (size_t)p.ncols_pad;
  t.nclusters = std::max(1, std::min(ngroups_all, p.wg_slots / t.clusterK));
  t.nheavy = std::min(opt.heavy_tiles < 0 ? auto_heavy : opt.heavy_tiles, ngroups_all);
  t.clusterHi = opt.heavy_cluster;
  if (const char* e = std::getenv("SLIM_GPU_HEAVY")) {
    int a = 0, b = 0;
    if (std::sscanf(e, "%d,%d", &a, &b) == 2) {
      t.nheavy = std::min(std::max(a, 0), ngroups_all);
      t.clusterHi = b;
    }
  }
  if (t.clusterHi != 2 && t.clusterHi != 4 && t.clusterHi != 8 && t.clusterHi != 16 && t.clusterHi != 32)
    t.clusterHi = std::max(16, std::min(4 * t.clusterK, kTileKMax));
  if (t.clusterHi <= t.clusterK || t.nclusters * t.clusterK < t.clusterHi || force_k1) t.nheavy = 0;
  if (t.nheavy > 0) {
    for (t.hi_lg = 0; (1 << t.hi_lg) < t.clusterHi; ++t.hi_lg) {}
    ensure_cluster_split(m, t.hi_lg);
    t.nclusters_hi = t.nclusters * t.clusterK / t.clusterHi;
    t.tile_r = std::max(t.tile_r, (size_t)(round_up(m->split[t.hi_lg].max_rows, 64) + 64) * tileP);
  }
  size_t free_b = 0, total_b = 0;
  HIP_TRY(hipMemGetInfo(&free_b, &total_b));
  const size_t per_cl = ((t.tile_r + 2 * t.tile_x) * sizeof(float) + t.tile_u * sizeof(int32_t)) * t.clusterK;
  const size_t have = free_b + m->ws_slab.bytes() + m->ws_xslab.bytes() + m->ws_ulist.bytes() +
                      m->ws_part.bytes() + m->ws_gram.bytes();
  const size_t budget = have > (size_t(6) << 30) ? have - (size_t(6) << 30) : have / 2;
  if ((size_t)t.nclusters * per_cl > budget) {
    t.nclusters = (int)std::max<size_t>(1, budget / per_cl);
    t.nclusters_hi = t.nclusters * t.clusterK / std::max(t.clusterHi, 1);
    if (t.nclusters_hi < 1) t.nheavy = 0;
  }
  t.nwaves = t.nclusters * t.clusterK;
  return t;
}

size_t mailbox_stride(int tileP) { return 2 * (size_t)kTileKMax * (size_t)tileP + 8; }

struct Slabs {
  float *slab = nullptr, *xslab = nullptr, *part = nullptr;
  int32_t *ulist = nullptr, *nunion = nullptr;
  unsigned long long* mailbox = nullptr;
  size_t mailbox_words = 0;
  int bm_shift = 0, bm_words = 1;
  size_t tile_lds = 0;
  bool gram_words = false;
  int32_t *f_n = nullptr, *f_id = nullptr, *f_slot = nullptr;
  float* f_aty = nullptr;
  int f_slice_tiles = 0;
};

Slabs alloc_slabs(slimgpu_matrix* m, const LearnOptions& opt, const Path& p, const TileGeom& t, int32_t nwork,
                  int nwaves) {
  Slabs s;
  const auto evict = evict_cache(m);
  if (p.use_fgram) {
    const size_t ngroups0 = std::max<size_t>(1, ((size_t)nwork + 31) / 32);
    const size_t per_tile = (size_t)32 * (size_t)p.f_stride * 12;
    size_t free_b = 0, total_b = 0;
    HIP_TRY(hipMemGetInfo(&free_b, &total_b));
    const size_t have = free_b + m->ws_fid.bytes() + m->ws_faty.bytes() + m->ws_fslot.bytes();
    size_t tiles = ngroups0;
    if (tiles * per_tile > have / 4) tiles = std::max<size_t>(1, have / 4 / per_tile);
    if (const char* e = std::getenv("SLIM_GPU_FSLIM_SLICE_TILES"); e && std::atoi(e) > 0)
      tiles = std::min<size_t>(tiles, (size_t)std::atoi(e));
    s.f_slice_tiles = (int)tiles;
    const size_t npos = std::min<size_t>((size_t)std::max(nwork, 1), tiles * 32);
    s.f_n = m->ws_fn.reserve(npos, evict);
    s.f_id = m->ws_fid.reserve(npos * (size_t)p.f_stride, evict);
    s.f_aty = m->ws_faty.reserve(npos * (size_t)p.f_stride, evict);
    s.f_slot = m->ws_fslot.reserve(npos * (size_t)p.f_stride, evict);
    s.ulist = m->ws_ulist.reserve((size_t)p.f_ustride * tiles, evict);
    s.nunion = m->ws_nunion.reserve(tiles, evict);
  } else if (p.use_gram) {
    const size_t ngroups0 = ((size_t)nwork + 31) / 32;
    s.xslab = m->ws_xslab.reserve((size_t)p.ncols_pad * (size_t)nwaves, evict);
    if (p.gram_v == 0) s.slab = m->ws_slab.reserve((size_t)p.ncols_pad * (size_t)nwaves, evict);
    s.ulist = m->ws_ulist.reserve((size_t)p.ncols_pad * ngroups0, evict);
    s.nunion = m->ws_nunion.reserve(ngroups0, evict);
  } else if (p.use_tile) {
    s.mailbox_words = (size_t)(std::max(t.nclusters, 1) + t.nclusters_hi) * mailbox_stride(p.tileP);
    s.slab = m->ws_slab.reserve(t.tile_r * (size_t)nwaves, evict);
    s.xslab = m->ws_xslab.reserve(t.tile_x * (size_t)nwaves, evict);
    s.ulist = m->ws_ulist.reserve(t.tile_u * (size_t)nwaves, evict);
    s.mailbox = m->ws_mailbox.reserve(s.mailbox_words, evict);
    s.part = m->ws_part.reserve(t.tile_x * (size_t)nwaves, evict);
    const int64_t range = (int64_t)(t.tile_r / (size_t)p.tileP);
    auto words_at = [&](int sh) { return ((range >> sh) + 1 + 31) / 32; };
    while (words_at(s.bm_shift) * 4 > kBitmapBytes) ++s.bm_shift;
    s.bm_words = (int)words_at(s.bm_shift);
    if (opt.nnbrs > 0) s.bm_words = std::max(s.bm_words, p.tileP * 256);
    s.tile_lds = sizeof(uint32_t) * (size_t)s.bm_words;
    if (p.gram_bits_lds && t.clusterK == 32 && !t.force_k1) {
      s.bm_shift = 0;
      s.bm_words = (int)(p.gram_bits_lds / sizeof(uint32_t));
      s.tile_lds = p.gram_bits_lds;
      s.gram_words = true;
    }
    if (opt.build_G) s.tile_lds = std::max(s.tile_lds, p.gram_stage_lds);
  } else if (!p.use_lds) {
    s.slab = m->ws_slab.reserve(p.vec_floats * (size_t)nwaves);
  }
  return s;
}

struct ArenaSeg {
  const int32_t* ind;
  const float* val;
  int64_t n;
  DeviceBuffer<int32_t> own_i;
  DeviceBuffer<float> own_v;
};

struct Launch {
  Path p;
  TileGeom t;
  Slabs s;
  int nwaves = 1;
  int32_t *order = nullptr, *cnt = nullptr, *sti = nullptr, *misc = nullptr;
  int64_t *off = nullptr, *stl = nullptr;
  float* stf = nullptr;
  const int64_t* icolptr = nullptr;
  const int32_t* icolind = nullptr;
  const float* icolval = nullptr;
  int32_t incols = 0;
  int gram_mode = 0;
  float* gram = nullptr;
  int gram_geom[6] = {0, 0, 0, 0, 0, 0};
  int gram_pass = 0;
  DeviceBuffer<float> carry;
  int64_t carry_stride = 0;
  bool carry_from_warm = false;
  bool cluster_fallback = false;
  int64_t arena_cap = 0;
  int32_t G_block = 0;
  bool gview_tried = false;
  const uint4* gview = nullptr;
  const int64_t* gview_base = nullptr;
  const uint16_t* gview_cnt = nullptr;
  int32_t gview_ngroups = 0, gview_sentinel = 0;
  size_t gview_bytes = 0;
  double gview_ms = 0;
  const char* gview_why = "";
};

void prepare_launch(slimgpu_matrix* m, const LearnOptions& opt, const std::vector<int32_t>& order,
                    const slim_csr_t* imodel, const slimgpu_model* warm_dev, bool resident, bool all_columns,
                    Launch& L) {
  const int32_t ncols = m->ncols, nwork = (int32_t)order.size();
  const Path& p = L.p;
  hipStream_t stream = m->stream;
  L.nwaves = p.nwaves;
  if (p.use_tile) {
    L.t = plan_tiles(m, opt, p, order, false);
    L.nwaves = L.t.nwaves;
  }
  L.order = m->ws_order.reserve((size_t)nwork);
  L.cnt = m->ws_cnt.reserve((size_t)ncols);
  L.off = m->ws_off.reserve((size_t)ncols);
  L.sti = m->ws_stat_i.reserve(3 * (size_t)ncols);
  L.stl = m->ws_stat_l.reserve(4 * (size_t)ncols);
  L.stf = m->ws_stat_f.reserve(2 * (size_t)ncols);
  L.misc = m->ws_misc.reserve(16);
  L.s = alloc_slabs(m, opt, p, L.t, nwork, L.nwaves);

  L.arena_cap = std::max<int64_t>(1 << 20, (int64_t)nwork * std::min<int64_t>(ncols, 8192));
  if (const char* env_cap = std::getenv("SLIM_GPU_ARENA")) L.arena_cap = std::max<int64_t>(1, std::atoll(env_cap));

  if (p.has_imodel && warm_dev) {
    L.incols = warm_dev->n;
    L.icolptr = warm_dev->d_colptr.get();
    L.icolind = warm_dev->d_colind.get();
    L.icolval = warm_dev->d_colval.get();
  } else if (p.has_imodel) {
    L.incols = imodel->ncols;
    const int64_t innz = imodel->colptr[L.incols];
    int64_t* cp = m->ws_icolptr.reserve((size_t)L.incols + 1);
    int32_t* ci = m->ws_icolind.reserve((size_t)innz);
    float* cv = m->ws_icolval.reserve((size_t)innz);
    HIP_TRY(hipMemcpyAsync(cp, imodel->colptr, sizeof(int64_t) * ((size_t)L.incols + 1),
                           hipMemcpyHostToDevice, stream));
    if (innz > 0) {
      HIP_TRY(hipMemcpyAsync(ci, imodel->colind, sizeof(int32_t) * (size_t)innz, hipMemcpyHostToDevice, stream));
      HIP_TRY(hipMemcpyAsync(cv, imodel->colval, sizeof(float) * (size_t)innz, hipMemcpyHostToDevice, stream));
    }
    L.icolptr = cp;
    L.icolind = ci;
    L.icolval = cv;
  }
  HIP_TRY(hipMemsetAsync(L.cnt, 0, sizeof(int32_t) * (size_t)ncols, stream));
  HIP_TRY(hipMemsetAsync(L.off, 0, sizeof(int64_t) * (size_t)ncols, stream));
  HIP_TRY(hipMemsetAsync(L.sti, 0, sizeof(int32_t) * 3 * (size_t)ncols, stream));
  HIP_TRY(hipMemsetAsync(L.stl, 0, sizeof(int64_t) * 4 * (size_t)ncols, stream));
  HIP_TRY(hipMemsetAsync(L.stf, 0, sizeof(float) * 2 * (size_t)ncols, stream));

  const TileGeom& t = L.t;
  const int geom[6] = {p.tileP, t.clusterK, t.nheavy > 0 ? t.clusterHi : 0, t.nheavy, opt.shard_count,
                       opt.shard_index};
  std::copy(geom, geom + 6, L.gram_geom);
  if (p.use_tile && !opt.build_G && !std::getenv("SLIM_GPU_NO_GRAM")) {
    const size_t ngroups0 = ((size_t)nwork + p.tileP - 1) / p.tileP;
    const size_t need = ngroups0 * t.tile_x * sizeof(float);
    if (!m->gram_order.empty() && m->gram_order == order && m->ws_gram.bytes() >= need &&
        std::equal(geom, geom + 6, m->gram_geom)) {
      L.gram_mode = 2;
      L.gram = m->ws_gram.get();
    } else {
      size_t free_b = 0, total_b = 0;
      HIP_TRY(hipMemGetInfo(&free_b, &total_b));
      if (need <= (size_t(32) << 30) && need <= (free_b + m->ws_gram.bytes()) / 4) {
        m->gram_order.clear();
        L.gram = m->ws_gram.reserve(need / sizeof(float));
        L.gram_mode = 1;
      }
    }
  }

  const int carry_groups = std::max(p.gramr_kr, 1) + p.gramr_kl;
  if (resident && p.use_gramr && carry_groups <= kGramrCarryMaxGroups && all_columns && nwork == ncols &&
      opt.shard_count == 1 && !std::getenv("SLIM_GPU_NO_CARRY")) {
    L.carry_stride = (int64_t)carry_groups * 8192;
    const size_t carry_bytes = sizeof(float) * (size_t)ncols * (size_t)L.carry_stride;
    if (warm_dev && warm_dev->d_gsave.get() && warm_dev->gsave_owner == m->uid &&
        warm_dev->gsave_stride == L.carry_stride && warm_dev->n == ncols) {
      L.carry_from_warm = warm_dev->gsave_valid && warm_dev->gsave_l1 == opt.l1r;
      L.carry = std::move(warm_dev->d_gsave);
      warm_dev->gsave_valid = false;
    } else {
      size_t free_b = 0, total_b = 0;
      HIP_TRY(hipMemGetInfo(&free_b, &total_b));
      if (carry_bytes <= (size_t(8) << 30) && carry_bytes * 4 <= free_b)
        L.carry = DeviceBuffer<float>((size_t)ncols * (size_t)L.carry_stride);
    }
  }
}

SolveArgs solve_args(slimgpu_matrix* m, const LearnOptions& opt, Launch& L, const std::vector<int32_t>& pending,
                     int attempt, int32_t* d_ai, float* d_av) {
  const Path& p = L.p;
  const TileGeom& t = L.t;
  const int32_t ncols = m->ncols, npend = (int32_t)pending.size();
  hipStream_t stream = m->stream;
  SolveArgs S;
  S.l1 = (float)opt.l1r;
  S.l2 = (float)opt.l2r;
  S.opt_tol = (float)opt.optTol;
  S.maxniters = opt.maxniters;
  S.seed = opt.seed;
  S.nnbrs = opt.nnbrs;
  S.simtype = opt.simtype;
  S.order = L.order;
  S.nwork = npend;
  S.queue = L.misc;
  S.icolptr = L.icolptr;
  S.icolind = L.icolind;
  S.icolval = L.icolval;
  S.incols = L.incols;
  S.slab = L.s.slab;
  S.slab_stride = p.use_tile ? (int64_t)t.tile_r : (int64_t)p.vec_floats;
  S.nrows_pad = p.nrows_pad;
  S.ncols_pad = p.ncols_pad;
  S.xslab = L.s.xslab;
  S.x_stride = (int64_t)t.tile_x;
  S.ulist = L.s.ulist;
  S.u_stride = (int64_t)t.tile_u;
  S.ngroups = (npend + p.tileP - 1) / p.tileP;
  if (opt.build_G && opt.G_rows_end >= 0) S.ngroups = (L.G_block + p.tileP - 1) / p.tileP;
  S.cluster = t.clusterK;
  S.ubounds = p.use_tile ? m->split[t.cluster_lg].ubounds.get() : nullptr;
  S.csplit = p.use_tile ? m->split[t.cluster_lg].csplit.get() : nullptr;
  S.mailbox = L.s.mailbox;
  S.exact_gram = p.exact_gram ? 1 : 0;
  S.atypart = L.s.part;
  S.bm_shift = L.s.bm_shift;
  S.bm_words = L.s.bm_words;
  S.nheavy = p.use_tile ? t.nheavy : 0;
  S.cluster_hi = t.clusterHi;
  S.ubounds_hi = t.nheavy > 0 ? m->split[t.hi_lg].ubounds.get() : nullptr;
  S.csplit_hi = t.nheavy > 0 ? m->split[t.hi_lg].csplit.get() : nullptr;
  S.mailbox_hi = L.s.mailbox ? L.s.mailbox + (size_t)std::max(t.nclusters, 1) * mailbox_stride(p.tileP) : nullptr;
  S.queue_hi = L.misc + 4;
  S.hi_prefetch = 1;
  S.shard_count = opt.shard_count;
  S.shard_index = opt.shard_index;
  S.nnz_last = m->nnz > 0 ? m->nnz - 1 : 0;
  S.xcd_swizzle = 0;
  S.gram_mode = (attempt == 0 && !L.cluster_fallback) ? L.gram_mode : 0;
  S.gram = L.gram;
  S.G = m->ws_G.get();
  S.G_ld = m->G_ld;
  S.tile_nunion = L.s.nunion;
  S.gram_pos = nullptr;
  S.gram_bits = (p.gram_bits_lds && t.clusterK == 32 && L.s.gram_words) ? 2 : 0;
  if (const char* e = std::getenv("SLIM_GPU_GBITS"); e && S.gram_bits) S.gram_bits = std::atoi(e) == 1 ? 1 : 2;
  S.gram_split_stride = t.clusterK + 1;
  S.gram_accum = 0;
  S.gram_store = 0;
  S.gram_read = 0;
  S.gview = nullptr;
  S.gview_base = nullptr;
  S.gview_cnt = nullptr;
  S.gview_ngroups = 0;
  S.gview_range0 = 0;
  S.gview_sentinel = 0;
  S.gram_part16 = S.gram_bits == 2 ? 1 : 0;
  if (const char* e = std::getenv("SLIM_GPU_GPART16"); e && std::atoi(e) == 0) S.gram_part16 = 0;
  S.g_save = nullptr;
  S.g_load = nullptr;
  S.g_stride = 0;
  if (L.carry.get()) {
    S.g_save = L.carry.get();
    S.g_stride = L.carry_stride;
    S.g_load = (L.carry_from_warm && attempt == 0) ? L.carry.get() : nullptr;
// ... 581 lines not shown
      double r = 0.0;
      for (int64_t e = hp[(size_t)u]; e < hp[(size_t)u + 1]; ++e) {
        if (hi[(size_t)e] == c) has = true;
        r += xd[(size_t)hi[(size_t)e]] * (m->binary ? 1.0 : (double)hv[(size_t)e]);
      }
      if (!has) scores.push_back((float)r);
    }
    const size_t ntop = std::min<size_t>(10, scores.size());
    std::partial_sort(scores.begin(), scores.begin() + (ptrdiff_t)ntop, scores.end(), std::greater<float>());
    float a0 = 0.0f;
    for (size_t j = 0; j < ntop; ++j) a0 += scores[j];
    for (ssize_t e = colptr[c]; e < colptr[c + 1]; ++e) xd[(size_t)colind[e]] = 0.0;
    const size_t i = (size_t)c;
    std::printf("Col: %5d %5zd rs: %3d nits: %4d nnz: %4d rsd: %.2le obj: %.2le ff: %.3lf nrm1: "
                "%.3lf a0s: %.3lf tmr: %.2le\n",
                c, (ssize_t)(hcp[i + 1] - hcp[i]), cs.conv[i], cs.sweeps[i], (int)(colptr[c + 1] - colptr[c]),
                (double)k.err[i], (double)k.obj[i], k.obj[i] != 0 ? (double)k.err[i] / (double)k.obj[i] : 0.0,
                nrm1, ntop ? (double)a0 / (double)ntop : 0.0, 0.0);
  }
  std::fflush(stdout);
}

slimgpu_stats_t solve_stats(slimgpu_matrix* m, const Launch& L, const Entries& E, const Counters& k,
                            const ColumnStats& cs, const std::vector<int32_t>& requested, int64_t tnnz) {
  const Path& p = L.p;
  slimgpu_stats_t st;
  std::memset(&st, 0, sizeof(st));
  st.ncols_solved = (int32_t)requested.size();
  st.kernel = p.kernel;
  st.nwaves = L.nwaves;
  st.lds_bytes = p.use_lds ? (int32_t)p.lds_need : 0;
  st.setup_ms = m->setup_ms;
  st.kernel_ms = E.kernel_ms;
  for (int32_t c : requested) {
    st.G += cs.G[c];
    st.D += cs.D[c];
    st.U += cs.U[c];
    st.sweeps += cs.sweeps[c];
    st.error += k.err[c];
    st.objval += k.obj[c];
  }
  st.nnzW = tnnz;
  st.alg_bytes = m->binary ? 4.0 * st.G + 8.0 * st.D + 4.0 * st.U + 8.0 * st.nnzW
                           : 8.0 * st.G + 12.0 * st.D + 4.0 * st.U + 8.0 * st.nnzW;
  if (p.use_gram || p.use_fgram) {
    st.gram_build_ms = m->G_build_ms;
    st.gram_alloc_ms = m->G_alloc_ms;
    st.gram_sums_ms = m->G_sums_ms;
    st.gram_sums_kernel_ms = m->G_sums_kernel_ms;
    st.gram_pack_ms = m->G_pack_ms;
    m->G_build_ms = m->G_alloc_ms = m->G_sums_ms = m->G_sums_kernel_ms = m->G_pack_ms = 0.0;
  }
  st.gram_rows = k.gram_rows;
  st.gram_bytes = k.gram_bytes;
  return st;
}

}

slim_csr_t* learn_cd(slimgpu_matrix_t* m, const LearnOptions& opt, const slim_csr_t* imodel,
                     int32_t* status, const int32_t* columns, int32_t ncolumns, bool row_view,
                     ResidentIO* rio) {
  const double t_begin = now_ms();
  auto fail = [&](int32_t code) -> slim_csr_t* {
    if (status) *status = code;
    return nullptr;
  };
  if (!m) {
    set_error("SLIMGPU_Learn: null matrix");
    return fail(SLIM_ERROR_INPUT);
  }
  try {
    const WorkList w = work_list(m, opt, columns, ncolumns);
    const std::vector<int32_t>& requested = w.order;
    const int32_t nwork = (int32_t)requested.size();
    (void)hipGetLastError();
    HIP_TRY(hipSetDevice(m->device));
    static std::recursive_mutex device_lock[64];
    std::lock_guard<std::recursive_mutex> solve_guard(device_lock[m->device & 63]);

    const slimgpu_model* warm_dev = rio ? rio->warm : nullptr;
    const bool resident = rio && rio->out;
    const char* trace_env = std::getenv("SLIM_GPU_TRACE");
    Launch L;
    L.G_block = w.G_block;
    L.p = choose_kernel(m, opt, nwork);
    L.p.trace_level = trace_env ? std::atoi(trace_env) : 0;
    if ((L.p.use_gram || L.p.use_fgram) && !m->G_ready) {
      if (const int32_t st = gram_for_solve(m, opt, L.p.trace_level, L.p.use_fgram); st != SLIM_OK) return fail(st);
    }
    finish_path(m, opt, nwork, imodel, warm_dev, L.p);
    prepare_launch(m, opt, requested, imodel, warm_dev, resident, columns == nullptr, L);
    const double t_prep_done = now_ms();

    Entries E = run_launches(m, opt, requested, resident, L);
    const double t_kernel_done = now_ms();
    ColumnStats& cs = g_colstats;
    const Counters k = read_counters(m, L, requested, cs);
    const double t_counters_done = now_ms();
    int64_t tnnz = 0;
    for (int32_t c = 0; c < m->ncols; ++c) tnnz += E.cnt[c];
    slim_csr_t* model = nullptr;
    double t_columns_done = t_counters_done;
    if (resident) {
      *rio->out = assemble_resident_model(m, opt, E, tnnz, L, row_view, &t_columns_done).release();
    } else {
      model = assemble_host_model(m->ncols, E, tnnz, row_view);
      t_columns_done = now_ms();
    }
    if (L.p.trace_level >= 1)
      std::fprintf(stderr, "[slim_gpu trace] host phases: prep %.0f ms, launches + D2H %.0f ms (kernel %.0f, D2H of "
                   "%lld entries %.0f), counters %.0f ms, columns %.0f ms, row view %.0f ms\n",
                   t_prep_done - t_begin, t_kernel_done - t_prep_done, E.kernel_ms, (long long)E.total, E.d2h_ms,
                   t_counters_done - t_kernel_done, t_columns_done - t_counters_done, now_ms() - t_columns_done);
    if ((opt.dbglvl & SLIM_DBG_PROGRESS) && model) print_progress(m, model, requested, cs, k);

    slimgpu_stats_t st = solve_stats(m, L, E, k, cs, requested, tnnz);
    st.gather_ms = now_ms() - t_kernel_done;
    if (!opt.build_G) m->last_order = requested;
    st.total_ms = now_ms() - t_begin;
    g_stats = st;
    if (opt.dbglvl & SLIM_DBG_INFO)
      std::printf("Done estimation: loss: %.5le, fit: %.5le, ffrac: %.3lf,  #nzs: %zd\n", st.objval,
                  st.error, st.objval != 0 ? st.error / st.objval : 0.0, (ssize_t)tnnz);
    if (status) *status = SLIM_OK;
    return model;
  } catch (const Refusal& r) {
    set_error(r.msg);
    return fail(r.status);
  } catch (const HipFail& e) {
    report(e, "SLIMGPU_Learn");
    return fail(status_of(e));
  } catch (const std::bad_alloc&) {
    set_error("SLIMGPU_Learn: out of host memory");
    return fail(SLIM_ERROR_MEMORY);
  }
}

slimgpu_model* learn_resident(slimgpu_matrix_t* m, const LearnOptions& opt, const slimgpu_model* warm,
                              int32_t* status) {
  if (m && !m->replicas.empty()) {
    set_error("SLIMGPU_LearnResident: a model resident in HBM belongs to one device (ngpus = 1)");
    if (status) *status = SLIM_ERROR_INPUT;
    return nullptr;
  }
  slimgpu_model* out = nullptr;
  ResidentIO rio;
  rio.warm = warm;
  rio.out = &out;
  int32_t st = SLIM_ERROR;
  (void)learn_cd(m, opt, nullptr, &st, nullptr, 0, true, &rio);
  if (status) *status = st;
  if (st != SLIM_OK && out) {
    model_free(out);
    out = nullptr;
  }
  return out;
}

slimgpu_model* model_from_host(slimgpu_matrix_t* m, const slim_csr_t* W, int32_t* status) {
  auto fail = [&](int32_t st, const std::string& why) {
    set_error("SLIMGPU_ModelFromHost: " + why);
    if (status) *status = st;
    return static_cast<slimgpu_model*>(nullptr);
  };
  if (!m || !W || !W->rowptr || W->nrows < 0 || W->ncols < 0)
    return fail(SLIM_ERROR_INPUT, "bad arguments (a staged matrix, a model handle with a row view)");
  if (!m->replicas.empty()) return fail(SLIM_ERROR_INPUT, "a model resident in HBM belongs to one device (ngpus = 1)");
  const int32_t n = std::max(W->nrows, W->ncols);
  const int64_t nnz = W->rowptr[W->nrows];
  if (W->rowptr[0] != 0) return fail(SLIM_ERROR_INPUT, "the row pointer does not start at 0");
  for (int32_t r = 0; r < W->nrows; ++r)
    if (W->rowptr[r + 1] < W->rowptr[r]) return fail(SLIM_ERROR_INPUT, "the row pointer descends");
  if (nnz > 0 && (!W->rowind || !W->rowval)) return fail(SLIM_ERROR_INPUT, "the model has no values");
  for (int64_t j = 0; j < nnz; ++j)
    if (W->rowind[j] < 0 || W->rowind[j] >= n) return fail(SLIM_ERROR_INPUT, "an item id outside the model");
  try {
    (void)hipGetLastError();
    HIP_TRY(hipSetDevice(m->device));
    hipStream_t stream = m->stream;
    std::unique_ptr<slimgpu_model> dm(new slimgpu_model());
    dm->device = m->device;
    dm->n = n;
    dm->nnz = nnz;
    std::vector<int64_t> h_ptr((size_t)n + 1, nnz);
    for (int32_t r = 0; r <= W->nrows; ++r) h_ptr[(size_t)r] = W->rowptr[r];
    dm->d_rowptr = DeviceBuffer<int64_t>((size_t)n + 1);
    dm->d_rowind = DeviceBuffer<int32_t>((size_t)std::max<int64_t>(nnz, 1));
    dm->d_rowval = DeviceBuffer<float>((size_t)std::max<int64_t>(nnz, 1));
    HIP_TRY(hipMemcpyAsync(dm->d_rowptr.get(), h_ptr.data(), sizeof(int64_t) * ((size_t)n + 1), hipMemcpyHostToDevice,
                           stream));
    if (nnz > 0) {
      HIP_TRY(hipMemcpyAsync(dm->d_rowind.get(), W->rowind, sizeof(int32_t) * (size_t)nnz, hipMemcpyHostToDevice, stream));
      HIP_TRY(hipMemcpyAsync(dm->d_rowval.get(), W->rowval, sizeof(float) * (size_t)nnz, hipMemcpyHostToDevice, stream));
    }
    int32_t* d_facts = m->ws_misc.reserve(16);
    int32_t facts[2] = {0, 0};
// ... 82 lines not shown
      HIP_TRY(hipMemcpyAsync(ri, w->d_rowind.get(), sizeof(int32_t) * (size_t)w->nnz, hipMemcpyDeviceToHost, cs));
      HIP_TRY(hipMemcpyAsync(rv, w->d_rowval.get(), sizeof(float) * (size_t)w->nnz, hipMemcpyDeviceToHost, cs));
    }
    HIP_TRY(hipStreamSynchronize(cs));
    (void)hipStreamDestroy(cs);
    cs = nullptr;
    slim_csr_t* hm = model_from_columns(w->n, cp, ci, cv, false);
    if (!hm) throw std::bad_alloc();
    hm->rowptr = rp;
    hm->rowind = ri;
    hm->rowval = rv;
    w->fetched = hm;
    w->fetch_status = SLIM_OK;
  } catch (const HipFail& e) {
    w->fetch_error = "SLIMGPU_ModelFetch: " + e.where + ": " + hipGetErrorString(e.code);
    w->fetch_status = SLIM_ERROR;
  } catch (const std::bad_alloc&) {
    w->fetch_error = "SLIMGPU_ModelFetch: out of host memory";
    w->fetch_status = SLIM_ERROR_MEMORY;
  }
  if (w->fetch_status != SLIM_OK) {
    if (cs) (void)hipStreamDestroy(cs);
    std::free(cp); std::free(rp); std::free(ci); std::free(ri); std::free(cv); std::free(rv);
  }
  w->fetch_ms = now_ms() - t0;
}
}

int32_t model_fetch_begin(slimgpu_model* w) {
  if (!w || !w->d_rowptr.get()) {
    set_error("SLIMGPU_ModelFetchBegin: null model");
    return SLIM_ERROR_INPUT;
  }
  if (w->fetch_begun) return SLIM_OK;
  w->fetch_begun = true;
  w->fetched = nullptr;
  w->fetch_status = SLIM_OK;
  try {
    w->fetcher = std::thread(fetch_now, w);
  } catch (const std::system_error&) {
    w->fetch_begun = false;
  }
  return SLIM_OK;
}

slim_csr_t* model_fetch(slimgpu_model* w, int32_t* status, double* ms) {
  if (!w || !w->d_rowptr.get()) {
    set_error("SLIMGPU_ModelFetch: null model");
    if (status) *status = SLIM_ERROR_INPUT;
    return nullptr;
  }
  if (w->fetch_begun) {
    if (w->fetcher.joinable()) w->fetcher.join();
    w->fetch_begun = false;
  } else {
    fetch_now(w);
  }
  slim_csr_t* hm = w->fetched;
  w->fetched = nullptr;
  if (w->fetch_status != SLIM_OK) set_error(w->fetch_error);
  if (status) *status = w->fetch_status;
  if (ms) *ms = w->fetch_ms;
  return hm;
}

void model_free(slimgpu_model* w) {
  if (!w) return;
  if (w->fetcher.joinable()) w->fetcher.join();
  if (w->fetched) csr_free(w->fetched);
  delete w;
}

int32_t gram_build_rows(slimgpu_matrix_t* m, int32_t row_begin, int32_t row_end) {
  if (!m || row_begin < 0 || row_end > m->ncols || row_begin > row_end) {
    set_error("SLIMGPU_MatrixGramBuildRows: rows outside [0, ncols)");
    return SLIM_ERROR_INPUT;
  }
  try {
    HIP_TRY(hipSetDevice(m->device));
    const size_t G_bytes = sizeof(float) * (size_t)m->ncols * (size_t)gram_ld(m->ncols);
    const bool fresh = m->G_ready || m->ws_G.bytes() < G_bytes;
    if (fresh) {
      size_t free_b = 0, total_b = 0;
      HIP_TRY(hipMemGetInfo(&free_b, &total_b));
      if (G_bytes + (size_t(8) << 30) > free_b + m->ws_G.bytes() + m->ws_gram.bytes()) {
        set_error("SLIMGPU_MatrixGramBuildRows: G = R^T R (4 ncols^2 bytes) does not fit the free HBM");
        return SLIM_ERROR_MEMORY;
      }
      m->G_ready = false;
      m->Gp_ready = false;
      m->Gp_tried = false;
    }
    LearnOptions bo;
    bo.G_rows_begin = row_begin;
    bo.G_rows_end = row_end;
    return build_gram(m, bo, fresh);
  } catch (const HipFail& e) {
    report(e, "SLIMGPU_MatrixGramBuildRows");
    return status_of(e);
  }
}

int32_t gram_view(slimgpu_matrix_t* m, void** dptr, int64_t* ld, int32_t* nrows) {
  if (!m || !m->ws_G.get() || m->G_ld <= 0) {
    set_error("SLIMGPU_MatrixGramView: no G on this handle (SLIMGPU_MatrixGramBuildRows first)");
    return SLIM_ERROR_INPUT;
  }
  if (dptr) *dptr = m->ws_G.get();
  if (ld) *ld = m->G_ld;
  if (nrows) *nrows = m->ncols;
  return SLIM_OK;
}

int32_t gram_commit(slimgpu_matrix_t* m) {
  if (!m || !m->ws_G.get() || m->G_ld <= 0) {
    set_error("SLIMGPU_MatrixGramCommit: no G on this handle");
    return SLIM_ERROR_INPUT;
  }
  try {
    HIP_TRY(hipSetDevice(m->device));
    HIP_TRY(hipStreamSynchronize(m->stream));
    m->G_ready = true;
    m->Gp_ready = false;
    m->Gp_tried = false;
    m->Gf_dropped = false;
    (void)pack_gram(m);
    drop_float_gram(m);
    return SLIM_OK;
  } catch (const HipFail& e) {
    report(e, "SLIMGPU_MatrixGramCommit");
    return status_of(e);
  }
}

int32_t gram_planes(slimgpu_matrix_t* m, slimgpu_gram_planes_t* out) {
  if (!m || !out || !m->Gp_ready) {
    set_error("SLIMGPU_MatrixGramPlanes: no byte planes on this handle (no G committed, or a G that could not be packed)");
    return SLIM_ERROR_INPUT;
  }
  out->ncols = m->ncols;
  out->nchunks = m->Gp_nchunks;
  out->ldb = m->Gp_ldb;
  out->hi_bytes = m->Gp_pool_bytes;
  out->lo = m->ws_Glo.get();
  out->base = m->ws_Gbase.get();
  out->hi = m->ws_Ghi.get();
  out->hi_off = m->ws_hioff.get();
  out->hi_k = m->ws_hik.get();
  out->hi2_k = m->ws_hi2k.get();
  out->diag = m->ws_Gdiag.get();
  out->meta = reinterpret_cast<const uint32_t*>(m->ws_Gmeta.get());
  out->rank_of = m->ws_rankof.get();
  out->item_of = m->ws_itemof.get();
  return SLIM_OK;
}

}
```

### slim_amd/csrc/engine.hpp

```cpp
#pragma once
#include <cstdint>
#include <vector>

#include "../../include/slim_gpu.h"

namespace slimamd {

struct EvalResult;

struct LearnOptions {
  int32_t nthreads = 1, nnbrs = 0, simtype = 0, dbglvl = 0, algo = SLIM_ALGO_CD;
  int32_t ordered = 0, maxniters = 10000;
  double l1r = 1.0, l2r = 1.0, optTol = 1e-7;
  int32_t col_begin = 0, col_end = -1;
  uint32_t seed = 1;
  int32_t device = -1;
  int32_t kernel = SLIMGPU_KERNEL_AUTO;
  int32_t cluster = 0;
  int32_t heavy_tiles = -1;
  int32_t heavy_cluster = 0;
  int32_t ngpus = 1;
  int32_t shard_count = 1, shard_index = 0;
  bool build_G = false;
  int32_t G_rows_begin = 0, G_rows_end = -1;
};
LearnOptions decode_options(const int32_t* ioptions, const double* doptions);

struct ColumnStats {
  std::vector<int32_t> nacols, sweeps, conv;
  std::vector<int64_t> G, D, U;
};

slimgpu_stats_t& last_stats();
ColumnStats& last_column_stats();

slimgpu_matrix_t* matrix_from_host(int32_t nrows, const ssize_t* rowptr,
                                   const int32_t* rowind, const float* rowval,
                                   const LearnOptions& opt, int32_t* status);
slimgpu_matrix_t* matrix_from_device(int32_t nrows, int32_t ncols,
                                     const int64_t* d_rowptr, const int32_t* d_rowind,
                                     const float* d_rowval, const LearnOptions& opt,
                                     int32_t* status);
void matrix_free(slimgpu_matrix_t* m);
slimgpu_matrix_t* matrix_clone_to_device(const slimgpu_matrix_t* src, int32_t device,
                                         int32_t* status);
int32_t matrix_info(const slimgpu_matrix_t* m, int32_t* nrows, int32_t* ncols, int64_t* nnz);
int32_t matrix_get_column_view(const slimgpu_matrix_t* m, int64_t* colptr, int32_t* colind,
                               float* colval, float* cnorms);
double matrix_setup_ms(const slimgpu_matrix_t* m);
int32_t matrix_column_cost(const slimgpu_matrix_t* m, int64_t* cost);
void matrix_expect_solves(slimgpu_matrix_t* m, int32_t n);
int32_t gram_build_rows(slimgpu_matrix_t* m, int32_t row_begin, int32_t row_end);
int32_t gram_view(slimgpu_matrix_t* m, void** dptr, int64_t* ld, int32_t* nrows);
int32_t gram_commit(slimgpu_matrix_t* m);
int32_t gram_planes(slimgpu_matrix_t* m, slimgpu_gram_planes_t* out);

struct ResidentIO {
  const slimgpu_model* warm = nullptr;
  slimgpu_model** out = nullptr;
};
slim_csr_t* learn_cd(slimgpu_matrix_t* m, const LearnOptions& opt, const slim_csr_t* imodel,
                     int32_t* status, const int32_t* columns = nullptr, int32_t ncolumns = 0,
                     bool row_view = true, ResidentIO* rio = nullptr);

slimgpu_model* learn_resident(slimgpu_matrix_t* m, const LearnOptions& opt, const slimgpu_model* warm,
                              int32_t* status);
slimgpu_model* model_from_host(slimgpu_matrix_t* m, const slim_csr_t* W, int32_t* status);
int64_t model_nnz(const slimgpu_model* w);
int32_t model_ncols(const slimgpu_model* w);
int32_t model_fetch_begin(slimgpu_model* w);
slim_csr_t* model_fetch(slimgpu_model* w, int32_t* status, double* ms = nullptr);
void model_free(slimgpu_model* w);

void matrix_add_replica(slimgpu_matrix_t* m, slimgpu_matrix_t* replica);
const std::vector<slimgpu_matrix_t*>& matrix_replicas(const slimgpu_matrix_t* m);
void matrix_adopt_csr(slimgpu_matrix_t* m);
int32_t matrix_device(const slimgpu_matrix_t* m);
void matrix_set_setup_ms(slimgpu_matrix_t* m, double ms);

slimgpu_matrix_t* multi_from_host(int32_t nrows, const ssize_t* rowptr, const int32_t* rowind,
                                  const float* rowval, const LearnOptions& opt, int32_t* status);
slim_csr_t* multi_learn(slimgpu_matrix_t* m, const LearnOptions& opt, const slim_csr_t* imodel,
                        int32_t* status, const int32_t* columns = nullptr, int32_t ncolumns = 0);

int32_t device_count();

int32_t predict_device(const slim_csr_t* W, const slim_csr_t* hist, int32_t nrcmds,
                       int32_t* output, float* scores, int32_t* counts);
struct DeviceRowView {
  int32_t nrows = 0, ncols = 0;
  int64_t nnz = 0, max_row = 0;
  bool rows_sorted = false;
  int32_t device = -1;
  const int64_t* d_ptr = nullptr;
  const int32_t* d_ind = nullptr;
  const float* d_val = nullptr;
};
int32_t predict_device_view(const DeviceRowView& W, const slim_csr_t* hist, int32_t nrcmds,
                            int32_t* output, float* scores, int32_t* counts);
int32_t predict_lists(const slim_csr_t* W, const slim_csr_t* hist, int32_t nrcmds,
                      int32_t* output, float* scores, int32_t* counts, slimgpu_filter* filter = nullptr);
int32_t predict_lists_view(const DeviceRowView& W, const slim_csr_t* hist, int32_t nrcmds,
                           int32_t* output, float* scores, int32_t* counts, slimgpu_filter* filter = nullptr);
struct HostFilter;
slimgpu_filter* filter_create(int32_t ncols, int32_t nitems, const int32_t* items, int32_t blocked, int32_t xusers,
                              const int64_t* xptr, const int32_t* xind, int32_t* status);
void filter_free(slimgpu_filter* f);
HostFilter filter_host(const slimgpu_filter* f);
int32_t filter_check(const char* who, const slimgpu_filter* f, int32_t model_ncols);
struct HostCandSet;
slimgpu_candset* candset_create(int32_t ncols, int32_t nusers, const int64_t* cptr, const int32_t* cind,
                                int32_t* status);
void candset_free(slimgpu_candset* cs);
HostCandSet candset_host(const slimgpu_candset* cs);
int32_t candset_check(const char* who, const slimgpu_candset* cs, int32_t model_ncols, int32_t nsel,
                      const int32_t* users, int32_t nrcmds, const int32_t* output, const float* scores);
void candset_need_ids(slimgpu_candset* cs);
int32_t candset_fetch_ids(const char* who, slimgpu_candset* cs);
int32_t candset_rows(slimgpu_candset* cs, int64_t* cptr, int32_t* cind);
int32_t candset_info(const slimgpu_candset* cs, int32_t* nrows, int32_t* ncols, int64_t* entries);
slimgpu_candset* evalset_sample_candidates(slimgpu_evalset_t* es, int32_t nnegs, uint64_t seed, int32_t* status);
slimgpu_candset* evalset_sample_candidates_weighted(slimgpu_evalset_t* es, int32_t nnegs, uint64_t seed,
                                                    const uint32_t* weights, int32_t* status);
double last_weighted_sample_kernel_ms();
int32_t score_candidates(const slim_csr_t* W, const slim_csr_t* trn, slimgpu_candset* cs, int32_t nrcmds,
                         float* slot_scores, int32_t* output, float* scores, int32_t* counts);
int32_t matrix_score_candidates(const slimgpu_model* model, slimgpu_matrix_t* mat, slimgpu_candset* cs, int32_t nusers,
                                const int32_t* users, int32_t nrcmds, float* slot_scores, int32_t* output,
                                float* scores, int32_t* counts);
int32_t explain_check(const char* who, int32_t nwhy, const int32_t* why_items, const float* why_terms);
int32_t explain_candidates(const slim_csr_t* W, const slim_csr_t* trn, slimgpu_candset* cs, int32_t nwhy,
                           int32_t* why_items, float* why_terms, int32_t* support);
int32_t matrix_explain_candidates(const slimgpu_model* model, slimgpu_matrix_t* mat, slimgpu_candset* cs,
                                  int32_t nusers, const int32_t* users, int32_t nwhy, int32_t* why_items,
                                  float* why_terms, int32_t* support);
slimgpu_list_stats_t& last_list_stats();
int32_t model_row_view(const slimgpu_model* w, DeviceRowView* out);
struct DeviceCsrView {
  int32_t device = -1, num_cus = 256;
  void* stream = nullptr;
  int32_t nrows = 0, ncols = 0;
  int64_t nnz = 0;
  bool merged = false;
  const int64_t* d_ptr = nullptr;
  const int32_t* d_ind = nullptr;
  const float* d_val = nullptr;
};
int32_t matrix_csr_view(const slimgpu_matrix_t* m, DeviceCsrView* out);

slimgpu_evalset_t* evalset_create(slimgpu_matrix_t* mat, const slim_csr_t* tst, const int32_t* fmarker,
                                  int32_t fm_ncols, int32_t ncutoffs, const int32_t* cutoffs, int32_t nusers,
                                  const int32_t* users, int32_t* status);
slimgpu_evalset_t* evalset_create_ranked(slimgpu_matrix_t* mat, const slim_csr_t* tst, const int32_t* fmarker,
                                         int32_t fm_ncols, int32_t nusers, const int32_t* users, int32_t* status);
int64_t evalset_entries(const slimgpu_evalset_t* es);
int32_t model_ranks(slimgpu_evalset_t* es, const slimgpu_model* model, int32_t* ranks, float* scores,
                    slimgpu_filter* filter = nullptr);
int32_t model_evaluate_ranked(slimgpu_evalset_t* es, const slimgpu_model* model, int32_t ncutoffs,
                              const int32_t* cutoffs, EvalResult* out, slimgpu_filter* filter = nullptr);
double last_rank_prepass_ms();
void evalset_free(slimgpu_evalset_t* es);
int32_t evalset_cutoffs(const slimgpu_evalset_t* es);
int32_t model_evaluate(slimgpu_evalset_t* es, const slimgpu_model* model, int32_t ncutoffs, EvalResult* out,
                       slimgpu_filter* filter = nullptr);
int32_t model_evaluate_candidates(slimgpu_evalset_t* es, const slimgpu_model* model, slimgpu_candset* cs,
                                  int32_t ncutoffs, EvalResult* out);
int32_t matrix_predict(int32_t nrcmds, const slimgpu_model* model, slimgpu_matrix_t* mat, int32_t* output,
                       float* scores);
// ... 20 lines not shown
```

### slim_amd/csrc/explain.hip

```cpp
#include <hip/hip_runtime.h>

#include <algorithm>
#include <chrono>
#include <cstdint>
#include <cstdlib>
#include <new>
#include <string>
#include <vector>

#include "explain_kernels.hpp"
#include "host_csr.hpp"
#include "host_stage.hpp"
#include "scorer.hpp"

namespace slimamd {
namespace {
constexpr int kStageDefault = 1024, kStageMax = 2048;

int stage_entries() {
  const char* s = std::getenv("SLIM_EXPLAIN_STAGE");
  if (!s || !*s) return kStageDefault;
  char* end = nullptr;
  const long v = std::strtol(s, &end, 10);
  if (*end || v < 1) return kStageDefault;
  return (int)std::min<long>(v, kStageMax);
}
bool form16_forced() {
  const char* s = std::getenv("SLIM_EXPLAIN_FORM");
  return s && std::string(s) == "16";
}

int32_t explain_rows(const char* who, const DeviceRowView& W, HistoryView H, const int32_t* h_users,
                     slimgpu_candset* cs, int device, int num_cus, hipStream_t stream, int32_t nwhy,
                     int32_t* why_items, float* why_terms, int32_t* support, slimgpu_eval_stats_t& st) {
  const std::string w(who);
  if (W.nnz > 0 && !W.rows_sorted)
    return refuse(w + ": the ids of some model row do not ascend strictly: the explanation kernel looks ids up by "
                      "binary search (SLIM_PREDICT=cpu explains any model)");
  if (W.nnz >= (int64_t)1 << 31) return refuse(w + ": the model has 2^31 entries or more");
  if (H.max_hist >= INT32_MAX) return refuse(w + ": a history has 2^31 - 1 entries or more");
  const int32_t nsel = H.nusers;
  const int64_t* cptr = candset_row_pointer(cs);
  int64_t entries = 0;
  for (int32_t q = 0; q < nsel; ++q) {
    const int32_t u = h_users ? h_users[q] : q;
    entries += cptr[u + 1] - cptr[u];
  }
  const bool places = why_items != nullptr;
  hipEvent_t ev0 = nullptr, ev1 = nullptr;
  int32_t rc = SLIM_OK;
  try {
    int set_allocs = 0;
    const CandidateRows rows = candset_on_device(cs, device, num_cus, stream, &set_allocs, &st.h2d_bytes);
    ExplainWorkspace& E = candset_explain_workspace(cs);
    E.allocs = 0;
    const size_t want = (size_t)entries * (places ? 8 * (size_t)nwhy + 4 : 4);
    size_t free_b = 0, total_b = 0;
    HIP_TRY(hipMemGetInfo(&free_b, &total_b));
    if (want > (free_b + E.held()) / 2) {
      set_error(w + ": the outputs of " + std::to_string(entries) + " candidate entries at nwhy = " +
                std::to_string(nwhy) + " need " + std::to_string(want) + " bytes of device memory, more than half of "
                "the " + std::to_string(free_b + E.held()) + " that are free: pass user sub-lists");
      return SLIM_ERROR_MEMORY;
    }
    ExplainArgs A = {};
    A.wrows = W.nrows; A.wptr = W.d_ptr; A.wind = W.d_ind; A.wval = W.d_val;
    A.npos = nsel; A.hptr = H.ptr; A.hind = H.ind; A.hval = H.val;
    A.cptr = rows.cptr; A.lptr = rows.lptr; A.pairs = rows.pairs;
    A.nwhy = nwhy;
    A.stage = stage_entries();
    if (h_users) {
      int32_t* d_users = E.need(E.users, (size_t)nsel);
      HIP_TRY(hipMemcpyAsync(d_users, h_users, sizeof(int32_t) * (size_t)nsel, hipMemcpyHostToDevice, stream));
      st.h2d_bytes += (int64_t)(sizeof(int32_t) * (size_t)nsel);
      int64_t* d_obase = E.need(E.obase, (size_t)nsel + 1);
      hipLaunchKernelGGL(k_explain_base, dim3(1), dim3(256), 0, stream, nsel, d_users, rows.cptr, d_obase);
      HIP_TRY(hipGetLastError());
      A.users = d_users;
      A.obase = d_obase;
    }
    A.support = E.need(E.support, (size_t)entries);
    if (places) {
      A.items = E.need(E.items, (size_t)entries * nwhy);
      A.terms = E.need(E.terms, (size_t)entries * nwhy);
    }
    HIP_TRY(hipMemsetAsync(A.support, 0, sizeof(int32_t) * (size_t)std::max<int64_t>(entries, 1), stream));
    HIP_TRY(hipEventCreate(&ev0));
    HIP_TRY(hipEventCreate(&ev1));
    HIP_TRY(hipEventRecord(ev0, stream));
    if (nsel > 0 && entries > 0) {
      const dim3 grid((unsigned)std::min<int64_t>(nsel, (int64_t)num_cus * 8)), block(64 * kExplainWaves);
      const size_t lds = sizeof(int4) * (size_t)A.stage;
      if (nwhy > 4 || form16_forced())
        hipLaunchKernelGGL(k_explain<16>, grid, block, lds, stream, A);
      else
        hipLaunchKernelGGL(k_explain<4>, grid, block, lds, stream, A);
      HIP_TRY(hipGetLastError());
    }
    HIP_TRY(hipEventRecord(ev1, stream));
    size_t down = 0;
    auto fetch = [&](auto& image, const auto* d, size_t n) {
      if (image.size() < n) image.resize(n);
      if (n == 0) return;
      HIP_TRY(hipMemcpyAsync(image.data(), d, sizeof(*d) * n, hipMemcpyDeviceToHost, stream));
      down += sizeof(*d) * n;
    };
    fetch(E.h_support, A.support, (size_t)entries);
    if (places) {
      fetch(E.h_items, A.items, (size_t)entries * nwhy);
      fetch(E.h_terms, A.terms, (size_t)entries * nwhy);
    }
    HIP_TRY(hipStreamSynchronize(stream));
    float ms = 0;
    HIP_TRY(hipEventElapsedTime(&ms, ev0, ev1));
    st.kernel_ms = ms;
    st.d2h_bytes += (int64_t)down;
    st.path = kExplain;
    st.device_allocs = set_allocs + E.allocs;
    int64_t ob = 0;
    for (int32_t q = 0; q < nsel; ++q) {
      const int32_t u = h_users ? h_users[q] : q;
      const int64_t e0 = cptr[u], len = cptr[u + 1] - e0;
      for (int64_t j = 0; j < len; ++j) {
        const int32_t n = E.h_support[ob + j];
        if (support) support[e0 + j] = n;
        if (!places) continue;
        const int64_t m = std::min<int64_t>(n, nwhy);
        std::copy_n(E.h_items.data() + (ob + j) * nwhy, m, why_items + (e0 + j) * nwhy);
        std::copy_n(E.h_terms.data() + (ob + j) * nwhy, m, why_terms + (e0 + j) * nwhy);
      }
      ob += len;
    }
  } catch (...) {
    if (ev0) (void)hipEventDestroy(ev0);
    if (ev1) (void)hipEventDestroy(ev1);
    throw;
  }
  if (ev0) (void)hipEventDestroy(ev0);
  if (ev1) (void)hipEventDestroy(ev1);
  return rc;
}
// ... 95 lines not shown
```

### slim_amd/csrc/hip_check.hpp

```cpp
#pragma once

#include <hip/hip_runtime.h>

#include <cstddef>
#include <string>
#include <utility>

#include "../../include/slim.h"

namespace slimamd {

struct HipFail {
  hipError_t code;
  std::string where;
};

#define HIP_TRY(expr)                                                              \
  do {                                                                             \
    hipError_t _e = (expr);                                                        \
    if (_e != hipSuccess) throw ::slimamd::HipFail{_e, std::string(#expr)};        \
  } while (0)

inline int32_t status_of(const HipFail& e) {
  return e.code == hipErrorOutOfMemory ? SLIM_ERROR_MEMORY : SLIM_ERROR;
}

template <class T>
class DeviceBuffer {
 public:
  DeviceBuffer() = default;
  explicit DeviceBuffer(size_t n) {
    HIP_TRY(hipMalloc(reinterpret_cast<void**>(&p), sizeof(T) * (n ? n : 1)));
    bytes_ = sizeof(T) * (n ? n : 1);
  }
  ~DeviceBuffer() { reset(); }
  DeviceBuffer(DeviceBuffer&& o) noexcept
      : p(std::exchange(o.p, nullptr)), bytes_(std::exchange(o.bytes_, 0)) {}
  DeviceBuffer& operator=(DeviceBuffer&& o) noexcept {
    if (this != &o) {
      reset();
      p = std::exchange(o.p, nullptr);
      bytes_ = std::exchange(o.bytes_, 0);
    }
    return *this;
  }
  DeviceBuffer(const DeviceBuffer&) = delete;
  DeviceBuffer& operator=(const DeviceBuffer&) = delete;

  T* get() const { return p; }
  size_t bytes() const { return bytes_; }
  T* release() {
    bytes_ = 0;
    return std::exchange(p, nullptr);
  }
  void reset() {
    if (p) (void)hipFree(p);
    p = nullptr;
    bytes_ = 0;
  }

  T* reserve(size_t n) {
    return reserve(n, [] { return false; });
  }
  template <class Evict>
  T* reserve(size_t n, Evict&& evict) {
    const size_t need = sizeof(T) * (n ? n : 1);
    if (bytes_ >= need) return p;
    if (p) HIP_TRY(hipFree(p));
    p = nullptr;
    bytes_ = 0;
    hipError_t e = hipMalloc(reinterpret_cast<void**>(&p), need);
    if (e == hipErrorOutOfMemory && evict()) {
      (void)hipGetLastError();
      e = hipMalloc(reinterpret_cast<void**>(&p), need);
    }
    if (e != hipSuccess) {
      p = nullptr;
      throw HipFail{e, "hipMalloc(workspace)"};
    }
    bytes_ = need;
    return p;
  }

 private:
  T* p = nullptr;
  size_t bytes_ = 0;
};

}
```

### slim_amd/csrc/slim_abi.cpp

```cpp
#include <cstdio>
#include <cstdlib>
#include <algorithm>
#include <cstring>
#include <string>
#include <vector>

#include "engine.hpp"
#include "host_csr.hpp"

using namespace slimamd;

static int predict_policy();

namespace {

slim_csr_t* as_csr(slim_t* h) { return static_cast<slim_csr_t*>(h); }

slim_csr_t* learn_from_host(int32_t nrows, const ssize_t* rowptr, const int32_t* rowind,
                            const float* rowval, int32_t* ioptions, double* doptions,
                            const slim_csr_t* imodel, int32_t* status) {
  set_error("");
  LearnOptions opt = decode_options(ioptions, doptions);
  if (opt.algo == SLIM_ALGO_ADMM)
    return learn_admm(nrows, rowptr, rowind, rowval, opt, status);
// ... 1084 lines not shown
double SLIMGPU_LastSampleKernelMs(void) { return last_weighted_sample_kernel_ms(); }

int32_t SLIMGPU_CandSetRows(slimgpu_candset_t* cs, int64_t* cptr, int32_t* cind) {
  set_error("");
  return candset_rows(cs, cptr, cind);
}

int32_t SLIMGPU_CandSetInfo(slimgpu_candset_t* cs, int32_t* nrows, int32_t* ncols, int64_t* entries) {
  set_error("");
  return candset_info(cs, nrows, ncols, entries);
}

int32_t SLIMGPU_LastListStats(slimgpu_list_stats_t* out) {
  if (!out) return SLIM_ERROR_INPUT;
  *out = last_list_stats();
  return SLIM_OK;
}

int32_t SLIMGPU_LastEvalStats(slimgpu_eval_stats_t* out) {
  if (!out) return SLIM_ERROR_INPUT;
  *out = last_eval_stats();
  return SLIM_OK;
}

slim_t* SLIMGPU_LearnColumns(slimgpu_matrix_t* mat, int32_t ncolumns, const int32_t* columns,
                             int32_t* ioptions, double* doptions, slim_t* imodel,
                             int32_t* r_status) {
  set_error("");
  int32_t status = SLIM_ERROR;
  LearnOptions opt = decode_options(ioptions, doptions);
  slim_csr_t* model = nullptr;
  if (opt.algo != SLIM_ALGO_CD || ncolumns < 0 || (ncolumns > 0 && !columns)) {
    set_error("SLIMGPU_LearnColumns: algo must be cd and the column list non-null");
    status = SLIM_ERROR_INPUT;
  } else {
    static const int32_t none = 0;
    model = multi_learn(mat, opt, as_csr(imodel), &status, columns ? columns : &none, ncolumns);
  }
  if (r_status) *r_status = status;
  return model;
}

int32_t SLIMGPU_Predict1vsK(int32_t nrcmds, int32_t nnegs, slim_t* slimhandle, slim_t* trnhandle,
                            int32_t* negitems, int32_t* output, float* scores) {
  set_error("");
  return predict_1vsk_device(as_csr(slimhandle), as_csr(trnhandle), nrcmds, nnegs, negitems, output,
                             scores);
}

int32_t SLIMGPU_Evaluate(int32_t nusers, int32_t nrcmds, const int32_t* lists,
                         const int32_t* counts, slim_t* tsthandle, const int32_t* fmarker,
                         int32_t fm_ncols, double* metrics, int32_t* nvalid) {
  set_error("");
  if (!metrics || !nvalid) return SLIM_ERROR_INPUT;
  EvalResult ev;
  const int32_t rc =
      evaluate_device(nusers, nrcmds, lists, counts, as_csr(tsthandle), fmarker, fm_ncols, &ev);
  if (rc != SLIM_OK) return rc;
  metrics[0] = ev.hr; metrics[1] = ev.hr_head; metrics[2] = ev.hr_tail; metrics[3] = ev.arhr;
  nvalid[0] = ev.nvalid; nvalid[1] = ev.nvalid_head; nvalid[2] = ev.nvalid_tail;
  return SLIM_OK;
}

int32_t SLIMGPU_LastStats(slimgpu_stats_t* out) {
  if (!out) return SLIM_ERROR_INPUT;
  *out = last_stats();
  return SLIM_OK;
}

int32_t SLIMGPU_LastColumnStats(int32_t ncols, int32_t* nacols, int32_t* sweeps, int32_t* conv,
                                int64_t* G, int64_t* D, int64_t* U) {
  const ColumnStats& cs = last_column_stats();
  if ((size_t)ncols > cs.nacols.size()) return SLIM_ERROR_INPUT;
  const size_t n = (size_t)ncols;
  if (nacols) std::memcpy(nacols, cs.nacols.data(), sizeof(int32_t) * n);
  if (sweeps) std::memcpy(sweeps, cs.sweeps.data(), sizeof(int32_t) * n);
  if (conv) std::memcpy(conv, cs.conv.data(), sizeof(int32_t) * n);
  if (G) std::memcpy(G, cs.G.data(), sizeof(int64_t) * n);
  if (D) std::memcpy(D, cs.D.data(), sizeof(int64_t) * n);
  if (U) std::memcpy(U, cs.U.data(), sizeof(int64_t) * n);
  return SLIM_OK;
}

int32_t SLIMGPU_DeviceCount(void) { return device_count(); }

const char* SLIMGPU_LastError(void) { return last_error(); }

}
```

### slim_amd/csrc/topn.hip

```cpp
#include <hip/hip_runtime.h>

#include <algorithm>
#include <chrono>
#include <cstdio>
#include <cstdlib>
#include <cstring>
#include <new>
#include <string>
#include <vector>

#include "host_stage.hpp"
#include "scorer.hpp"
#include "topn_kernels.hpp"

namespace slimamd {
bool rows_ascend_strictly(int num_cus, int32_t nrows, const int64_t* d_ptr, const int32_t* d_ind) {
  DeviceBuffer<int32_t> d_unsorted(1);
  HIP_TRY(hipMemset(d_unsorted.get(), 0, sizeof(int32_t)));
  hipLaunchKernelGGL(k_rows_sorted, dim3(std::max(1, std::min(nrows / 4 + 1, num_cus * 8))), dim3(256), 0, 0, nrows,
                     d_ptr, d_ind, d_unsorted.get());
  HIP_TRY(hipGetLastError());
  int32_t unsorted = 0;
  HIP_TRY(hipMemcpy(&unsorted, d_unsorted.get(), sizeof(int32_t), hipMemcpyDeviceToHost));
  return unsorted == 0;
// ... 278 lines not shown
      for (int64_t g0 = 0; g0 < rk.max_test; g0 += A.gsize) {
        if (g0 > 0) HIP_TRY(hipMemsetAsync(ws.queue.get(), 0, 2 * sizeof(int32_t), stream));
        A.g0 = (int32_t)g0;
        launch_scorer(pick_kernel<TopNRankArgs>(P), L, 64 * P.t2w, P.lds, stream, A);
      }
      break;
    }
    case kCand: {
      const CandidateRows& cr = std::get<CandTargets>(rq).rows;
      L.groups = chunk_groups(P.lds, P.t2w, H.nusers, num_cus);
      ws.need(ws.cand, (size_t)cr.entries);
      HIP_TRY(hipMemsetAsync(ws.cand.get(), 0, sizeof(float) * (size_t)std::max<int64_t>(cr.entries, 1), stream));
      if (cr.entries <= 0) break;
      TopNCandArgs A{};
      fill_common(A, W, H, C, ws);
      A.cptr = cr.cptr; A.lptr = cr.lptr; A.pairs = cr.pairs; A.out = ws.cand.get();
      const char* benv = std::getenv("SLIM_CAND_BOUNDS");
      A.bounds_table = ((size_t)P.nchunks + 1) * sizeof(int) <= (size_t)P.t2w * kT2MaxN * 16 + P.t2w * sizeof(int) &&
                       !(benv && std::strcmp(benv, "search") == 0);
      launch_scorer(pick_kernel<TopNCandArgs>(P), L, 64 * P.t2w, P.lds, stream, A);
      break;
    }
    default: {
      size_t lds = 0;
      L.groups = wave_kernel_waves(H.nusers, nrcmds, num_cus, &lds);
      TopNArgs T;
      fill_views(T, W, H, C, ws);
      T.score = ws.score.get(); T.disc = ws.disc.get();
      T.out_ids = ws.oid.get(); T.out_scores = ws.osc.get(); T.out_cnt = ws.ocnt.get();
      fill_filter(T.flt, F);
      launch_scorer(&topn_kernel, L, 64, lds, stream, T);
      if (ev)
        launch_user_terms(stream, num_cus, H.nusers, H.users, nrcmds, ev->cut, ws.oid.get(), ws.ocnt.get(), ev->tptr,
                          ev->tind, ev->fmarker, ev->fm_ncols, ev->terms);
    }
  }
  return L;
}

ScorerPath queue_candidates(const DeviceRowView& W, const HistoryView& H, const CandidateRows& rows, int32_t nrcmds,
                            int num_cus, hipStream_t stream, ScorerWorkspace& ws) {
  const ScorerRequest rq = CandTargets{rows};
  if (queue_scorer(W, H, choose_scorer(W, H, rq), rq, num_cus, stream, ws).path != kCand) return kRefused;
  if (nrcmds > 0 && H.nusers > 0) {
    ws.need(ws.oid, (size_t)H.nusers * nrcmds); ws.need(ws.osc, (size_t)H.nusers * nrcmds);
    ws.need(ws.ocnt, (size_t)H.nusers);
    const size_t lds = (size_t)kLongMaxN * sizeof(uint4);
    hipLaunchKernelGGL(k_cand_lists, dim3(std::max(1, std::min<int>(H.nusers, num_cus * 8))),
                       dim3(64 * kCandListWaves), lds, stream, H.nusers, H.users, nrcmds, rows.cptr, rows.cind,
                       ws.cand.get(), ws.oid.get(), ws.osc.get(), ws.ocnt.get());
    HIP_TRY(hipGetLastError());
  }
  return kCand;
}

size_t fetch_lists(const ScorerWorkspace& ws, int32_t nusers, int32_t nrcmds, hipStream_t stream, int32_t* output,
                   float* scores, int32_t* counts) {
  if (nusers <= 0) return 0;
  std::vector<int32_t> h_id((size_t)nusers * nrcmds), h_cnt((size_t)nusers);
  std::vector<float> h_sc((size_t)nusers * nrcmds);
  HIP_TRY(hipMemcpyAsync(h_id.data(), ws.oid.get(), sizeof(int32_t) * h_id.size(), hipMemcpyDeviceToHost, stream));
  HIP_TRY(hipMemcpyAsync(h_sc.data(), ws.osc.get(), sizeof(float) * h_sc.size(), hipMemcpyDeviceToHost, stream));
  HIP_TRY(hipMemcpyAsync(h_cnt.data(), ws.ocnt.get(), sizeof(int32_t) * h_cnt.size(), hipMemcpyDeviceToHost, stream));
  HIP_TRY(hipStreamSynchronize(stream));
  for (int32_t u = 0; u < nusers; ++u) {
    for (int32_t r = 0; r < h_cnt[u]; ++r) {
      output[(int64_t)u * nrcmds + r] = h_id[(size_t)u * nrcmds + r];
      scores[(int64_t)u * nrcmds + r] = h_sc[(size_t)u * nrcmds + r];
    }
    if (counts) counts[u] = h_cnt[u];
  }
  return sizeof(int32_t) * (h_id.size() + h_cnt.size()) + sizeof(float) * h_sc.size();
}

namespace {
thread_local slimgpu_list_stats_t g_list_stats;

int32_t long_slice_users(int32_t nusers, int32_t nrcmds) {
  if (const char* e = std::getenv("SLIM_TOPN_LONG_SLICE")) {
    const long v = std::atol(e);
    if (v >= 1) return (int32_t)std::min<long>(v, std::max(nusers, 1));
  }
  size_t free_b = 0, total_b = 0;
  HIP_TRY(hipMemGetInfo(&free_b, &total_b));
  const size_t per_user = (size_t)nrcmds * (sizeof(int32_t) + sizeof(float)) + sizeof(int32_t);
  return (int32_t)std::max<size_t>(1, std::min<size_t>((size_t)std::max(nusers, 1), free_b / 4 / per_user));
}
}

slimgpu_list_stats_t& last_list_stats() { return g_list_stats; }

ScorerPath score_lists(const DeviceRowView& W, const HistoryView& H, const ScorerChoice& C, int num_cus,
                       hipStream_t stream, ScorerWorkspace& ws, int32_t* output, float* scores, int32_t* counts,
                       size_t* down, const CandidateFilter& F) {
  slimgpu_list_stats_t ls = {};
  const int32_t nrcmds = C.nrcmds;
  const ScorerRequest rq = LongListsRequest{nrcmds};
  size_t bytes = 0;
  if (C.path != kLong) {
    const ScorerLaunch L = queue_scorer(W, H, C, rq, num_cus, stream, ws, F);
    if (L.path == kRefused) return kRefused;
    bytes = fetch_lists(ws, H.nusers, nrcmds, stream, output, scores, counts);
    ls.slices = 1;
  } else {
    ws.need(ws.lstats, 8);
    HIP_TRY(hipMemsetAsync(ws.lstats.get(), 0, 8 * sizeof(unsigned long long), stream));
    const int32_t step = long_slice_users(H.nusers, nrcmds);
    for (int32_t s0 = 0; s0 < H.nusers; s0 += step) {
      HistoryView S = H;
      S.nusers = std::min(step, H.nusers - s0);
      if (H.users) S.users = H.users + s0; else S.user0 = H.user0 + s0;
      queue_scorer(W, S, C, rq, num_cus, stream, ws, F);
      bytes += fetch_lists(ws, S.nusers, nrcmds, stream, output + (int64_t)s0 * nrcmds, scores + (int64_t)s0 * nrcmds,
                           counts ? counts + s0 : nullptr);
      ++ls.slices;
    }
    unsigned long long h[5] = {};
    HIP_TRY(hipMemcpyAsync(h, ws.lstats.get(), sizeof(h), hipMemcpyDeviceToHost, stream));
    HIP_TRY(hipStreamSynchronize(stream));
    bytes += sizeof(h);
    ls.candidates = (int64_t)h[0]; ls.contenders = (int64_t)h[1]; ls.refine_passes = (int64_t)h[2];
    ls.lds_sorts = (int64_t)h[3]; ls.key_refines = (int64_t)h[4];
  }
  ls.path = C.path;
  if (down) *down = bytes;
  g_list_stats = ls;
  return C.path;
}

namespace {
const char* predict_name(bool long_ok) { return long_ok ? "SLIMGPU_PredictLists" : "SLIMGPU_Predict"; }

int32_t check_predict_args(bool long_ok, bool model_ok, const slim_csr_t* hist, int32_t nrcmds, const int32_t* output,
                           const float* scores) {
  const bool hist_ok = model_ok && hist && hist->rowptr && nrcmds >= 1;
  if (!long_ok && !(hist_ok && nrcmds <= 128)) return refuse("SLIMGPU_Predict: bad arguments (1 <= nrcmds <= 128)");
  if (long_ok && !(hist_ok && output && scores && nrcmds <= SLIMGPU_MAX_LIST))
    return refuse("SLIMGPU_PredictLists: bad arguments (a model, a history, output arrays, 1 <= nrcmds <= " +
              std::to_string(SLIMGPU_MAX_LIST) + ")");
  return SLIM_OK;
}
bool host_model_ok(const slim_csr_t* W) { return W && W->rowptr && (W->rowval || W->rowptr[W->nrows] <= 0); }

int32_t predict_view_impl(const DeviceRowView& W, const slim_csr_t* hist, int32_t nrcmds, int32_t* output,
                          float* scores, int32_t* counts, bool long_ok, slimgpu_filter* filter = nullptr) {
  const int32_t nusers = hist->nrows;
  if (const int32_t rc = filter_check("SLIMGPU_PredictLists", filter, W.ncols); rc != SLIM_OK) return rc;
  const auto t_begin = std::chrono::steady_clock::now();
  try {
    (void)hipGetLastError();
    int ndev = 0;
    HIP_TRY(hipGetDeviceCount(&ndev));
    if (ndev <= 0) throw HipFail{hipErrorNoDevice, "hipGetDeviceCount"};
    if (W.device >= 0) HIP_TRY(hipSetDevice(W.device));
    const int num_cus = cu_count();
    const StagedCsr h = stage_csr(hist, nusers, true, nullptr);
    HistoryView H;
    H.nusers = nusers; H.max_hist = h.max_row;
    H.ptr = h.ptr.get(); H.ind = h.ind.get(); H.val = h.val.get();
    DeviceRowView V = W;
    if (!V.rows_sorted && V.nnz > 0) V.rows_sorted = rows_ascend_strictly(num_cus, V.nrows, V.d_ptr, V.d_ind);
    const ScorerRequest rq = long_ok ? ScorerRequest(LongListsRequest{nrcmds}) : ScorerRequest(ListsRequest{nrcmds});
    const ScorerChoice C = choose_scorer(V, H, rq);
    if (C.chunk_pin_missed)
      return refuse("SLIMGPU_Predict: SLIM_TOPN_KERNEL=chunk needs nrcmds <= 64 and model rows sorted by id");
    ScorerWorkspace ws;
    if (long_ok) {
// ... 65 lines not shown
```

### slim_amd/engine.py

```python
import ctypes as C

import numpy as np
import scipy.sparse as sp

from . import _lib
from .constants import SLIM_NOPTIONS, SLIM_OK, Opt

KERNEL_AUTO, KERNEL_WAVE_LDS, KERNEL_WAVE_HBM, KERNEL_TILE, KERNEL_TILE16, KERNEL_GRAM = 0, 1, 2, 3, 4, 5
KERNEL_GRAM_FSLIM = 6


def make_options(l1r=1.0, l2r=1.0, optTol=1e-7, niters=10000, seed=1, col_begin=None,
                 col_end=None, kernel=KERNEL_AUTO, device=None, dbglvl=0, cluster=None, nnbrs=0,
                 simtype=0, heavy_tiles=None, heavy_cluster=None, ngpus=None, shard=None):
    iopt = np.full(SLIM_NOPTIONS, -1, dtype=np.int32)
    dopt = np.full(SLIM_NOPTIONS, -1.0, dtype=np.float64)
    iopt[Opt.DBGLVL] = dbglvl
    iopt[Opt.MAXNITERS] = niters
    iopt[Opt.GPU_SEED] = seed
    iopt[Opt.GPU_KERNEL] = kernel
    iopt[Opt.NNBRS] = nnbrs
    iopt[Opt.SIMTYPE] = simtype
    if col_begin is not None:
        iopt[Opt.GPU_COLBEGIN] = col_begin
# ... 233 lines not shown
            raise RuntimeError("SLIMGPU_CandSetRows failed (%d): %s" % (st, _lib.last_error()))
        return self

    def rows(self):
        ind = np.zeros(self.size + 1, np.int32)
        st = self._lib.SLIMGPU_CandSetRows(self.handle, None, ind.ctypes.data_as(C.c_void_p))
        if st != SLIM_OK:
            raise RuntimeError("SLIMGPU_CandSetRows failed (%d): %s" % (st, _lib.last_error()))
        return self.indptr.copy(), ind[:self.size]

    def close(self):
        if self.handle is not None and self.handle.value:
            self._lib.SLIMGPU_CandSetFree(self.handle)
        self.handle = None

    def __del__(self):
        try:
            self.close()
        except Exception:
            pass


def popularity_weights(R, alpha=1.0):
    R = sp.csr_matrix(R)
    counts = np.bincount(R.indices, minlength=R.shape[1]).astype(np.int64)
    if alpha == 1:
        return counts.astype(np.uint32)
    w = np.rint(counts.astype(np.float64) ** float(alpha) * 1024.0)
    if w.size and w.max() >= 2.0 ** 32:
        raise ValueError("popularity_weights: a weight reaches 2^32")
    return w.astype(np.uint32)


def _sampling_weights(weights, ncols):
    if weights is None:
        return False, None
    if isinstance(weights, str):
        if weights != "popularity":
            raise ValueError('weights: None, "popularity" or an array of ncols integers, not %r' % weights)
        return True, None
    w = np.asarray(weights)
    if w.ndim != 1 or w.size != ncols:
        raise ValueError("weights: %d items need %d weights, not an array of shape %s" % (ncols, ncols, w.shape))
    if w.dtype.kind not in "iu" or (w.size and (int(w.min()) < 0 or int(w.max()) >= 2 ** 32)):
        raise ValueError("weights: non-negative integers below 2^32")
    return True, np.ascontiguousarray(w, dtype=np.uint32)


def sample_candidates(trn, tst, nnegs, seed=1, users=None, ncols=None, lib=None, weights=None):
    lib = lib or _lib.load()
    trn, tst = sp.csr_matrix(trn), sp.csr_matrix(tst)
    ncols = max(trn.shape[1], tst.shape[1]) if ncols is None else int(ncols)
    weighted, w = _sampling_weights(weights, ncols)
    sel = None if users is None else np.ascontiguousarray(users, dtype=np.int32).ravel()
    ht, hs = _wrap_rows(lib, trn), _wrap_rows(lib, tst)
    h = C.c_void_p()
    name = "SLIMGPU_CandSetSampleWeighted" if weighted else "SLIMGPU_CandSetSample"
    args = (ncols, ht, hs, 0 if sel is None else sel.size, None if sel is None else sel.ctypes.data_as(C.c_void_p),
            int(nnegs), int(seed))
    try:
        if weighted:
            st = lib.SLIMGPU_CandSetSampleWeighted(*(args + (None if w is None else w.ctypes.data_as(C.c_void_p),
                                                             C.byref(h))))
        else:
            st = lib.SLIMGPU_CandSetSample(*(args + (C.byref(h),)))
    finally:
        lib.Py_csr_free(ht)
        lib.Py_csr_free(hs)
    if st != SLIM_OK:
        raise ValueError("%s failed (%d): %s" % (name, st, _lib.last_error()))
    return CandidateSet.from_handle(h, lib=lib)


def eval_stats(lib=None):
    st = _lib.EvalStats()
    (lib or _lib.load()).SLIMGPU_LastEvalStats(C.byref(st))
    return st.as_dict()


def list_stats(lib=None):
    st = _lib.ListStats()
    (lib or _lib.load()).SLIMGPU_LastListStats(C.byref(st))
    return st.as_dict()


def _wrap_rows(lib, M):
    M = sp.csr_matrix(M)
    ptr = np.ascontiguousarray(M.indptr, dtype=np.intp)
    ind = np.ascontiguousarray(M.indices, dtype=np.int32)
    val = np.ascontiguousarray(M.data, dtype=np.float32)
    h = C.c_void_p()
    st = lib.Py_csr_wrapper(M.shape[0], ptr, ind, val.ctypes.data_as(C.c_void_p), C.byref(h))
    if st != SLIM_OK:
        raise RuntimeError("Py_csr_wrapper failed (%d)" % st)
    return h


class Evaluator(object):

    def __init__(self, lib, handle, matrix, cutoffs=(10,), indptr=None):
        self._lib = lib
        self.handle = C.c_void_p(handle)
        self._matrix = matrix
        self.cutoffs = tuple(int(c) for c in cutoffs)
        self.indptr = indptr

    def evaluate(self, model, filter=None):
        if filter is not None:
            return {k: v for k, v in self.evaluate_at(model, filter=filter)[-1].items() if k != "nrcmds"}
        met = np.zeros(4, np.float64)
        nv = np.zeros(3, np.int32)
        st = self._lib.SLIMGPU_ModelEvaluate(self.handle, model.handle, met, nv)
        if st != SLIM_OK:
            raise RuntimeError("SLIMGPU_ModelEvaluate failed (%d): %s" % (st, _lib.last_error()))
        return {"hr": met[0], "hr_head": met[1], "hr_tail": met[2], "arhr": met[3],
                "nvalid": int(nv[0]), "nvalid_head": int(nv[1]), "nvalid_tail": int(nv[2])}

    def evaluate_at(self, model, filter=None):
        n = len(self.cutoffs)
        met = np.zeros(4 * n, np.float64)
        nv = np.zeros(3 * n, np.int32)
        if filter is None:
            st = self._lib.SLIMGPU_ModelEvaluateAt(self.handle, model.handle, n, met, nv)
        else:
            st = self._lib.SLIMGPU_ModelEvaluateAtFiltered(self.handle, model.handle, filter.handle, n, met, nv)
        if st != SLIM_OK:
            raise RuntimeError("SLIMGPU_ModelEvaluateAt%s failed (%d): %s"
                               % ("" if filter is None else "Filtered", st, _lib.last_error()))
        return [{"nrcmds": c, "hr": met[4 * k], "hr_head": met[4 * k + 1], "hr_tail": met[4 * k + 2],
                 "arhr": met[4 * k + 3], "nvalid": int(nv[3 * k]), "nvalid_head": int(nv[3 * k + 1]),
                 "nvalid_tail": int(nv[3 * k + 2])} for k, c in enumerate(self.cutoffs)]

    def ranks(self, model, scores=False, filter=None):
        n = int(self._lib.SLIMGPU_EvalSetEntries(self.handle))
        rk = np.zeros(max(n, 1), np.int32)
        sc = np.zeros(max(n, 1), np.float32) if scores else None
        out = (rk.ctypes.data_as(C.c_void_p), None if sc is None else sc.ctypes.data_as(C.c_void_p))
        if filter is None:
            st = self._lib.SLIMGPU_ModelRanks(self.handle, model.handle, *out)
        else:
            st = self._lib.SLIMGPU_ModelRanksFiltered(self.handle, model.handle, filter.handle, *out)
        if st != SLIM_OK:
            raise RuntimeError("SLIMGPU_ModelRanks%s failed (%d): %s"
                               % ("" if filter is None else "Filtered", st, _lib.last_error()))
        return (rk[:n], self.indptr, sc[:n]) if scores else (rk[:n], self.indptr)

    def evaluate_ranked(self, model, cutoffs, filter=None):
        cut = np.ascontiguousarray(cutoffs, dtype=np.int32).ravel()
        n = cut.size
        met = np.zeros(4 * max(n, 1), np.float64)
        nv = np.zeros(3 * max(n, 1), np.int32)
        if filter is None:
            st = self._lib.SLIMGPU_ModelEvaluateRanked(self.handle, model.handle, n, cut.ctypes.data_as(C.c_void_p),
                                                       met, nv)
        else:
            st = self._lib.SLIMGPU_ModelEvaluateRankedFiltered(self.handle, model.handle, filter.handle, n,
                                                               cut.ctypes.data_as(C.c_void_p), met, nv)
        if st != SLIM_OK:
            raise RuntimeError("SLIMGPU_ModelEvaluateRanked%s failed (%d): %s"
                               % ("" if filter is None else "Filtered", st, _lib.last_error()))
        return [{"nrcmds": int(c), "hr": met[4 * k], "hr_head": met[4 * k + 1], "hr_tail": met[4 * k + 2],
                 "arhr": met[4 * k + 3], "nvalid": int(nv[3 * k]), "nvalid_head": int(nv[3 * k + 1]),
                 "nvalid_tail": int(nv[3 * k + 2])} for k, c in enumerate(cut)]

    def evaluate_candidates(self, model, cset):
        n = len(self.cutoffs)
# ... 315 lines not shown
```

Before: 2246.

## Add per-device caching allocator to reuse freed large device blocks

Routes DeviceBuffer allocation and release through a process-wide per-device block cache. Freed buffers of at least 16 MB are parked instead of passed to hipFree, and later requests are served from a parked block within 25% of the requested size. Free-memory queries add parked bytes so existing fit checks still pass. The aim is to remove repeated hipMalloc/hipFree costs across matrix builds and solves, at the price of holding up to half of HBM idle and a device-wide synchronize on every park.

```diff
diff --git a/include/slim_gpu.h b/include/slim_gpu.h
--- a/include/slim_gpu.h
+++ b/include/slim_gpu.h
@@ -167,6 +167,7 @@
 
 #include "slim_gpu_eval.h"
 #include "slim_gpu_planes.h"
+#include "slim_gpu_cache.h"
 #include "slim_gpu_rank.h"
 #include "slim_gpu_lists.h"
 #include "slim_gpu_filter.h"
diff --git a/include/slim_gpu_cache.h b/include/slim_gpu_cache.h
--- /dev/null
+++ b/include/slim_gpu_cache.h
@@ -0,0 +1,22 @@
+#ifndef SLIM_AMD_SLIM_GPU_CACHE_H_
+#define SLIM_AMD_SLIM_GPU_CACHE_H_
+
+#include "slim.h"
+
+#ifdef __cplusplus
+extern "C" {
+#endif
+
+typedef struct {
+  int64_t parked_bytes, parked_blocks;
+  int64_t hits, misses;
+  int64_t hit_bytes;
+} slimgpu_cache_stats_t;
+int64_t SLIMGPU_DeviceCacheTrim(int32_t device);
+int32_t SLIMGPU_DeviceCacheStats(int32_t device, slimgpu_cache_stats_t *out);
+
+#ifdef __cplusplus
+}
+#endif
+
+#endif
diff --git a/slim_amd/_lib.py b/slim_amd/_lib.py
--- a/slim_amd/_lib.py
+++ b/slim_amd/_lib.py
@@ -23,6 +23,14 @@
                 ("gram_rows", C.c_int64), ("gram_bytes", C.c_double),
                 ("gram_alloc_ms", C.c_double), ("gram_sums_ms", C.c_double),
                 ("gram_sums_kernel_ms", C.c_double), ("gram_pack_ms", C.c_double)]
+
+    def as_dict(self):
+        return {k: getattr(self, k) for k, _ in self._fields_}
+
+
+class CacheStats(C.Structure):
+    _fields_ = [("parked_bytes", C.c_int64), ("parked_blocks", C.c_int64), ("hits", C.c_int64),
+                ("misses", C.c_int64), ("hit_bytes", C.c_int64)]
 
     def as_dict(self):
         return {k: getattr(self, k) for k, _ in self._fields_}
@@ -145,6 +153,13 @@
 }
 
 PLANES_SYMBOLS = tuple(_PLANES_SIGNATURES)
+
+_CACHE_SIGNATURES = {
+    "SLIMGPU_DeviceCacheTrim": (C.c_int64, [C.c_int32]),
+    "SLIMGPU_DeviceCacheStats": (C.c_int32, [C.c_int32, C.POINTER(CacheStats)]),
+}
+
+CACHE_SYMBOLS = tuple(_CACHE_SIGNATURES)
 MAX_CUTOFFS = 8
 
 _RANK_SIGNATURES = {
@@ -271,7 +286,8 @@
                               list(_RANK_SIGNATURES.items()) + list(_LIST_SIGNATURES.items()) +
                               list(_FILTER_SIGNATURES.items()) + list(_FILTERED_EVAL_SIGNATURES.items()) +
                               list(_CAND_SIGNATURES.items()) + list(_SAMPLE_SIGNATURES.items()) +
-                              list(_WSAMPLE_SIGNATURES.items()) + list(_EXPLAIN_SIGNATURES.items())):
+                              list(_WSAMPLE_SIGNATURES.items()) + list(_EXPLAIN_SIGNATURES.items()) +
+                              list(_CACHE_SIGNATURES.items())):
         if os.environ.get("SLIM_AMD_LIB") and not hasattr(lib, name):
             continue
         fn = getattr(lib, name)
diff --git a/slim_amd/csrc/admm.hip b/slim_amd/csrc/admm.hip
--- a/slim_amd/csrc/admm.hip
+++ b/slim_amd/csrc/admm.hip
@@ -240,7 +240,7 @@
     if (ndev <= 0) throw HipFail{hipErrorNoDevice, "hipGetDeviceCount"};
     if (opt.device >= 0) HIP_TRY(hipSetDevice(opt.device));
     size_t free_b = 0, total_b = 0;
-    HIP_TRY(hipMemGetInfo(&free_b, &total_b));
+    HIP_TRY(device_mem_info(&free_b, &total_b));
     if ((double)n2 * 8.0 * 6.5 > (double)free_b)
       return fail(SLIM_ERROR_MEMORY, "SLIM_Learn(admm): six " + std::to_string(m) + " x " +
                                          std::to_string(m) + " fp64 matrices do not fit this GPU");
diff --git a/slim_amd/csrc/device_cache.cpp b/slim_amd/csrc/device_cache.cpp
--- /dev/null
+++ b/slim_amd/csrc/device_cache.cpp
@@ -0,0 +1,169 @@
+#include "device_cache.hpp"
+
+#include <algorithm>
+#include <cstdlib>
+
+namespace slimamd {
+namespace devcache {
+
+bool enabled() {
+  const char* e = std::getenv("SLIM_GPU_BLOCK_CACHE");
+  return !(e && e[0] == '0' && e[1] == '\0');
+}
+
+size_t min_block_bytes() {
+  double mb = 16.0;
+  if (const char* e = std::getenv("SLIM_GPU_BLOCK_CACHE_MIN_MB")) mb = std::atof(e);
+  return mb > 0 ? (size_t)(mb * 1048576.0) : 0;
+}
+
+namespace {
+bool in_range(int device) { return device >= 0 && device < kMaxDevices; }
+}
+
+size_t BlockCache::cap_bytes(int device) {
+  if (const char* e = std::getenv("SLIM_GPU_BLOCK_CACHE_GB")) {
+    const double gb = std::atof(e);
+    return gb > 0 ? (size_t)(gb * 1073741824.0) : 0;
+  }
+  Device& d = dev_[device];
+  {
+    std::lock_guard<std::mutex> lk(d.mu);
+    if (d.total_b) return d.total_b / 2;
+  }
+  size_t free_b = 0, total_b = 0;
+  if (be_.mem_info(be_.ctx, device, &free_b, &total_b) != 0) return 0;
+  std::lock_guard<std::mutex> lk(d.mu);
+  d.total_b = total_b;
+  return total_b / 2;
+}
+
+void BlockCache::free_blocks(int device, const std::vector<Block>& blocks) {
+  for (const Block& b : blocks) (void)be_.free_block(be_.ctx, device, b.p);
+}
+
+int BlockCache::take(int device, size_t need, void** p, size_t* got, const std::function<bool()>& evict) {
+  *p = nullptr;
+  *got = 0;
+  const bool counted = in_range(device) && need >= min_block_bytes();
+  if (counted && enabled()) {
+    Device& d = dev_[device];
+    std::lock_guard<std::mutex> lk(d.mu);
+    const size_t most = need + need / 4;
+    size_t best = d.parked.size();
+    for (size_t i = 0; i < d.parked.size(); ++i) {
+      const size_t b = d.parked[i].bytes;
+      if (b >= need && b <= most && (best == d.parked.size() || b < d.parked[best].bytes)) best = i;
+    }
+    if (best != d.parked.size()) {
+      *p = d.parked[best].p;
+      *got = d.parked[best].bytes;
+      d.parked.erase(d.parked.begin() + (std::ptrdiff_t)best);
+      d.st.parked_bytes -= *got;
+      d.st.parked_blocks -= 1;
+      d.st.hits += 1;
+      d.st.hit_bytes += *got;
+      return 0;
+    }
+  }
+  int e = be_.alloc(be_.ctx, device, need, p);
+  if (e == be_.oom && trim(device) > 0) e = be_.alloc(be_.ctx, device, need, p);
+  if (e == be_.oom && evict && evict()) e = be_.alloc(be_.ctx, device, need, p);
+  if (e != 0) {
+    *p = nullptr;
+    return e;
+  }
+  *got = need;
+  if (counted) {
+    Device& d = dev_[device];
+    std::lock_guard<std::mutex> lk(d.mu);
+    d.st.misses += 1;
+    d.st.miss_bytes += need;
+  }
+  return 0;
+}
+
+void BlockCache::park(int device, void* p, size_t bytes) {
+  if (!p) return;
+  if (!in_range(device) || !enabled() || bytes < min_block_bytes()) {
+    (void)be_.free_block(be_.ctx, device, p);
+    return;
+  }
+  const size_t cap = cap_bytes(device);
+  if (bytes > cap || be_.synchronize(be_.ctx, device) != 0) {
+    (void)be_.free_block(be_.ctx, device, p);
+    return;
+  }
+  std::vector<Block> victims;
+  Device& d = dev_[device];
+  {
+    std::lock_guard<std::mutex> lk(d.mu);
+    d.parked.push_back(Block{p, bytes, d.next_seq++});
+    d.st.parked_bytes += bytes;
+    d.st.parked_blocks += 1;
+    d.st.parks += 1;
+    d.st.park_bytes += bytes;
+    while (d.st.parked_bytes > cap) {
+      const auto oldest = std::min_element(d.parked.begin(), d.parked.end(),
+                                           [](const Block& a, const Block& b) { return a.seq < b.seq; });
+      victims.push_back(*oldest);
+      d.st.parked_bytes -= oldest->bytes;
+      d.st.parked_blocks -= 1;
+      d.st.trimmed_bytes += oldest->bytes;
+      d.parked.erase(oldest);
+    }
+  }
+  free_blocks(device, victims);
+}
+
+size_t BlockCache::trim(int device) {
+  if (device < 0) {
+    size_t all = 0;
+    for (int i = 0; i < kMaxDevices; ++i) all += trim(i);
+    return all;
+  }
+  if (!in_range(device)) return 0;
+  std::vector<Block> victims;
+  size_t freed = 0;
+  Device& d = dev_[device];
+  {
+    std::lock_guard<std::mutex> lk(d.mu);
+    victims.swap(d.parked);
+    freed = (size_t)d.st.parked_bytes;
+    d.st.trimmed_bytes += freed;
+    d.st.parked_bytes = 0;
+    d.st.parked_blocks = 0;
+  }
+  free_blocks(device, victims);
+  return freed;
+}
+
+Stats BlockCache::stats(int device) const {
+  Stats s;
+  for (int i = 0; i < kMaxDevices; ++i) {
+    if (device >= 0 && i != device) continue;
+    std::lock_guard<std::mutex> lk(dev_[i].mu);
+    const Stats& t = dev_[i].st;
+    s.parked_bytes += t.parked_bytes;
+    s.parked_blocks += t.parked_blocks;
+    s.hits += t.hits;
+    s.misses += t.misses;
+    s.hit_bytes += t.hit_bytes;
+    s.miss_bytes += t.miss_bytes;
+    s.parks += t.parks;
+    s.park_bytes += t.park_bytes;
+    s.trimmed_bytes += t.trimmed_bytes;
+  }
+  return s;
+}
+
+int BlockCache::mem_info(int device, size_t* free_b, size_t* total_b) {
+  const int e = be_.mem_info(be_.ctx, device, free_b, total_b);
+  if (e != 0 || !in_range(device)) return e;
+  std::lock_guard<std::mutex> lk(dev_[device].mu);
+  *free_b += (size_t)dev_[device].st.parked_bytes;
+  return 0;
+}
+
+}
+}
diff --git a/slim_amd/csrc/device_cache.hpp b/slim_amd/csrc/device_cache.hpp
--- /dev/null
+++ b/slim_amd/csrc/device_cache.hpp
@@ -0,0 +1,66 @@
+#pragma once
+
+#include <cstddef>
+#include <cstdint>
+#include <functional>
+#include <mutex>
+#include <vector>
+
+namespace slimamd {
+namespace devcache {
+
+struct Backend {
+  int (*alloc)(void* ctx, int device, size_t bytes, void** out) = nullptr;
+  int (*free_block)(void* ctx, int device, void* p) = nullptr;
+  int (*synchronize)(void* ctx, int device) = nullptr;
+  int (*mem_info)(void* ctx, int device, size_t* free_b, size_t* total_b) = nullptr;
+  void* ctx = nullptr;
+  int oom = 2;
+};
+
+struct Stats {
+  uint64_t parked_bytes = 0, parked_blocks = 0;
+  uint64_t hits = 0, misses = 0, hit_bytes = 0, miss_bytes = 0;
+  uint64_t parks = 0, park_bytes = 0;
+  uint64_t trimmed_bytes = 0;
+};
+
+constexpr int kMaxDevices = 64;
+
+class BlockCache {
+ public:
+  explicit BlockCache(const Backend& b) : be_(b) {}
+  BlockCache(const BlockCache&) = delete;
+  BlockCache& operator=(const BlockCache&) = delete;
+
+  int take(int device, size_t need, void** p, size_t* got, const std::function<bool()>& evict);
+  void park(int device, void* p, size_t bytes);
+  size_t trim(int device);
+  Stats stats(int device) const;
+  int mem_info(int device, size_t* free_b, size_t* total_b);
+
+ private:
+  struct Block {
+    void* p;
+    size_t bytes;
+    uint64_t seq;
+  };
+  struct Device {
+    mutable std::mutex mu;
+    std::vector<Block> parked;
+    Stats st;
+    uint64_t next_seq = 0;
+    size_t total_b = 0;
+  };
+  size_t cap_bytes(int device);
+  void free_blocks(int device, const std::vector<Block>& blocks);
+
+  Backend be_;
+  Device dev_[kMaxDevices];
+};
+
+bool enabled();
+size_t min_block_bytes();
+
+}
+}
diff --git a/slim_amd/csrc/engine.hip b/slim_amd/csrc/engine.hip
--- a/slim_amd/csrc/engine.hip
+++ b/slim_amd/csrc/engine.hip
@@ -54,6 +54,9 @@
   int64_t* d_rowptr = nullptr;
   int32_t* d_rowind = nullptr;
   float* d_rowval = nullptr;
+  DeviceBuffer<int64_t> own_rowptr;
+  DeviceBuffer<int32_t> own_rowind;
+  DeviceBuffer<float> own_rowval;
   DeviceBuffer<int64_t> d_colptr;
   DeviceBuffer<int32_t> d_colind;
   DeviceBuffer<float> d_colval, d_cnorm, d_csq;
@@ -102,7 +105,7 @@
 
   ~slimgpu_matrix() {
     (void)hipSetDevice(device);
-    if (owns_csr) {
+    if (owns_csr && !own_rowptr.get()) {
       (void)hipFree(d_rowptr);
       (void)hipFree(d_rowind);
       (void)hipFree(d_rowval);
@@ -153,6 +156,20 @@
 void report(const HipFail& e, const char* what) {
   set_error(std::string(what) + ": HIP error '" + hipGetErrorString(e.code) + "' in " + e.where +
             " -- the SLIM CD path needs a gfx950 GPU; there is no CPU fallback");
+}
+
+void trace_blocks(const char* phase, int device, const devcache::Stats& since) {
+  const devcache::Stats now = device_cache().stats(device);
+  std::fprintf(stderr, "[trace] blocks, %s: %llu reused (%.2f GB), %llu taken fresh (%.2f GB), %llu parked (%.2f GB); "
+               "the cache holds %llu (%.2f GB)\n", phase,
+               (unsigned long long)(now.hits - since.hits), (double)(now.hit_bytes - since.hit_bytes) * 1e-9,
+               (unsigned long long)(now.misses - since.misses), (double)(now.miss_bytes - since.miss_bytes) * 1e-9,
+               (unsigned long long)(now.parks - since.parks), (double)(now.park_bytes - since.park_bytes) * 1e-9,
+               (unsigned long long)now.parked_blocks, (double)now.parked_bytes * 1e-9);
+}
+bool trace_on() {
+  const char* e = std::getenv("SLIM_GPU_TRACE");
+  return e && std::atoi(e) >= 1;
 }
 
 void drop_screen_cache(slimgpu_matrix* m) {
@@ -574,6 +591,19 @@
   int n = 0;
   if (hipGetDeviceCount(&n) != hipSuccess) return 0;
   return n;
+}
+
+int64_t device_cache_trim(int32_t device) { return (int64_t)device_cache().trim(device); }
+
+slimgpu_cache_stats_t device_cache_stats(int32_t device) {
+  const devcache::Stats s = device_cache().stats(device);
+  slimgpu_cache_stats_t o;
+  o.parked_bytes = (int64_t)s.parked_bytes;
+  o.parked_blocks = (int64_t)s.parked_blocks;
+  o.hits = (int64_t)s.hits;
+  o.misses = (int64_t)s.misses;
+  o.hit_bytes = (int64_t)s.hit_bytes;
+  return o;
 }
 
 namespace {
@@ -658,6 +688,7 @@
   }
   return make_matrix("SLIMGPU_MatrixFromHost", status, [&](slimgpu_matrix* m) {
     pick_device(m, opt);
+    const devcache::Stats blocks0 = device_cache().stats(m->device);
     m->nrows = nrows;
     m->nnz = rowptr[nrows];
     m->binary = rowval == nullptr;
@@ -665,9 +696,9 @@
     m->ncols = max_index_plus_one(m->nnz, rowind);
     if (m->ncols <= 0) m->ncols = 1;
     m->owns_csr = true;
-    m->d_rowptr = DeviceBuffer<int64_t>((size_t)nrows + 1).release();
-    m->d_rowind = DeviceBuffer<int32_t>((size_t)m->nnz).release();
-    m->d_rowval = m->binary ? nullptr : DeviceBuffer<float>((size_t)m->nnz).release();
+    m->d_rowptr = (m->own_rowptr = DeviceBuffer<int64_t>((size_t)nrows + 1)).get();
+    m->d_rowind = (m->own_rowind = DeviceBuffer<int32_t>((size_t)m->nnz)).get();
+    m->d_rowval = m->binary ? nullptr : (m->own_rowval = DeviceBuffer<float>((size_t)m->nnz)).get();
     static_assert(sizeof(ssize_t) == sizeof(int64_t), "LP64 expected");
     HIP_TRY(hipMemcpyAsync(m->d_rowptr, rowptr, sizeof(int64_t) * ((size_t)nrows + 1),
                            hipMemcpyHostToDevice, m->stream));
@@ -680,6 +711,7 @@
     }
     build_column_view(m);
     m->setup_ms = now_ms() - t0;
+    if (trace_on()) trace_blocks("staging", m->device, blocks0);
   });
 }
 
@@ -694,6 +726,7 @@
   const double t0 = now_ms();
   return make_matrix("SLIMGPU_MatrixFromDevice", status, [&](slimgpu_matrix* m) {
     pick_device(m, opt);
+    const devcache::Stats blocks0 = device_cache().stats(m->device);
     m->nrows = nrows;
     m->owns_csr = false;
     m->d_rowptr = const_cast<int64_t*>(d_rowptr);
@@ -717,6 +750,7 @@
     m->ncols = ncols > 0 ? ncols : 1;
     build_column_view(m);
     m->setup_ms = now_ms() - t0;
+    if (trace_on()) trace_blocks("staging", m->device, blocks0);
   });
 }
 
@@ -741,9 +775,9 @@
     m->owns_csr = true;
     m->h_cost = src->h_cost;
     const size_t nz = (size_t)std::max<int64_t>(m->nnz, 1);
-    m->d_rowptr = DeviceBuffer<int64_t>((size_t)m->nrows + 1).release();
-    m->d_rowind = DeviceBuffer<int32_t>(nz).release();
-    m->d_rowval = m->binary ? nullptr : DeviceBuffer<float>(nz).release();
+    m->d_rowptr = (m->own_rowptr = DeviceBuffer<int64_t>((size_t)m->nrows + 1)).get();
+    m->d_rowind = (m->own_rowind = DeviceBuffer<int32_t>(nz)).get();
+    m->d_rowval = m->binary ? nullptr : (m->own_rowval = DeviceBuffer<float>(nz)).get();
     m->d_colptr = DeviceBuffer<int64_t>((size_t)m->ncols + 1);
     m->d_colind = DeviceBuffer<int32_t>(nz + 64);
     if (!m->binary) m->d_colval = DeviceBuffer<float>(nz);
@@ -933,7 +967,7 @@
   const int64_t ldb = (int64_t)nchunks * 16;
   const size_t need = (size_t)ncols * ((size_t)ldb + kPackGroup) + (size_t)n1 + (size_t)n2 + 2 * (size_t)kPackGroup;
   size_t free_b = 0, total_b = 0;
-  HIP_TRY(hipMemGetInfo(&free_b, &total_b));
+  HIP_TRY(device_mem_info(&free_b, &total_b));
   if (need + (size_t(4) << 30) > free_b + m->ws_Glo.bytes() + m->ws_Ghi.bytes() + m->ws_Gbase.bytes()) return false;
   uint8_t* d_lo = m->ws_Glo.reserve((size_t)ncols * (size_t)ldb);
   uint8_t* d_hi = m->ws_Ghi.reserve((size_t)npool + kPackGroup);
@@ -982,7 +1016,7 @@
   if ((m->Gp_nchunks + kGramrNT - 1) / kGramrNT > kGramrMaxGroups) return;
   double min_gb = 8.0;
   if (const char* e = std::getenv("SLIM_GPU_DROP_G_MIN_GB")) min_gb = std::atof(e);
-  if ((double)m->ws_G.bytes() < min_gb * 1073741824.0) return;
+  if ((double)sizeof(float) * (double)m->ncols * (double)m->G_ld < min_gb * 1073741824.0) return;
   (void)hipStreamSynchronize(m->stream);
   m->ws_G.reset();
   m->Gf_dropped = true;
@@ -1111,7 +1145,7 @@
       m->Gf_dropped = false;
     }
     size_t free_b = 0, total_b = 0;
-    HIP_TRY(hipMemGetInfo(&free_b, &total_b));
+    HIP_TRY(device_mem_info(&free_b, &total_b));
     if (!m->G_ready && G_bytes + (size_t(4) << 30) > free_b + m->ws_gram.bytes())
       throw Refusal{SLIM_ERROR_MEMORY, "SLIMGPU_Learn: G = R^T R (4 ncols^2 bytes) does not fit the free HBM"};
     p.use_fgram = true;
@@ -1120,7 +1154,7 @@
   if (p.kernel == SLIMGPU_KERNEL_GRAM) {
     if (!gram_fits) throw Refusal{SLIM_ERROR_INPUT, "SLIMGPU_Learn: the item-space kernel has no FSLIM form"};
     size_t free_b = 0, total_b = 0;
-    HIP_TRY(hipMemGetInfo(&free_b, &total_b));
+    HIP_TRY(device_mem_info(&free_b, &total_b));
     if (!m->G_ready && G_bytes + (size_t(4) << 30) > free_b + m->ws_gram.bytes())
       throw Refusal{SLIM_ERROR_MEMORY, "SLIMGPU_Learn: G = R^T R (4 ncols^2 bytes) does not fit the free HBM"};
     p.use_gram = true;
@@ -1135,7 +1169,7 @@
       item_space = item_space && (m->G_ready || m->expect_solves >= 2);
     if (item_space) {
       size_t free_b = 0, total_b = 0;
-      HIP_TRY(hipMemGetInfo(&free_b, &total_b));
+      HIP_TRY(device_mem_info(&free_b, &total_b));
       p.use_gram = m->G_ready || G_bytes + (size_t(8) << 30) <= free_b + m->ws_gram.bytes();
     }
   }
@@ -1457,7 +1491,7 @@
     t.tile_r = std::max(t.tile_r, (size_t)(round_up(m->split[t.hi_lg].max_rows, 64) + 64) * tileP);
   }
   size_t free_b = 0, total_b = 0;
-  HIP_TRY(hipMemGetInfo(&free_b, &total_b));
+  HIP_TRY(device_mem_info(&free_b, &total_b));
   const size_t per_cl = ((t.tile_r + 2 * t.tile_x) * sizeof(float) + t.tile_u * sizeof(int32_t)) * t.clusterK;
   const size_t have = free_b + m->ws_slab.bytes() + m->ws_xslab.bytes() + m->ws_ulist.bytes() +
                       m->ws_part.bytes() + m->ws_gram.bytes();
@@ -1494,7 +1528,7 @@
     const size_t ngroups0 = std::max<size_t>(1, ((size_t)nwork + 31) / 32);
     const size_t per_tile = (size_t)32 * (size_t)p.f_stride * 12;
     size_t free_b = 0, total_b = 0;
-    HIP_TRY(hipMemGetInfo(&free_b, &total_b));
+    HIP_TRY(device_mem_info(&free_b, &total_b));
     const size_t have = free_b + m->ws_fid.bytes() + m->ws_faty.bytes() + m->ws_fslot.bytes();
     size_t tiles = ngroups0;
     if (tiles * per_tile > have / 4) tiles = std::max<size_t>(1, have / 4 / per_tile);
@@ -1643,7 +1677,7 @@
       L.gram = m->ws_gram.get();
     } else {
       size_t free_b = 0, total_b = 0;
-      HIP_TRY(hipMemGetInfo(&free_b, &total_b));
+      HIP_TRY(device_mem_info(&free_b, &total_b));
       if (need <= (size_t(32) << 30) && need <= (free_b + m->ws_gram.bytes()) / 4) {
         m->gram_order.clear();
         L.gram = m->ws_gram.reserve(need / sizeof(float));
@@ -1664,7 +1698,7 @@
       warm_dev->gsave_valid = false;
     } else {
       size_t free_b = 0, total_b = 0;
-      HIP_TRY(hipMemGetInfo(&free_b, &total_b));
+      HIP_TRY(device_mem_info(&free_b, &total_b));
       if (carry_bytes <= (size_t(8) << 30) && carry_bytes * 4 <= free_b)
         L.carry = DeviceBuffer<float>((size_t)ncols * (size_t)L.carry_stride);
     }
@@ -2412,6 +2446,7 @@
     const slimgpu_model* warm_dev = rio ? rio->warm : nullptr;
     const bool resident = rio && rio->out;
     const char* trace_env = std::getenv("SLIM_GPU_TRACE");
+    const devcache::Stats blocks0 = device_cache().stats(m->device);
     Launch L;
     L.G_block = w.G_block;
     L.p = choose_kernel(m, opt, nwork);
@@ -2443,6 +2478,7 @@
                    "%lld entries %.0f), counters %.0f ms, columns %.0f ms, row view %.0f ms\n",
                    t_prep_done - t_begin, t_kernel_done - t_prep_done, E.kernel_ms, (long long)E.total, E.d2h_ms,
                    t_counters_done - t_kernel_done, t_columns_done - t_counters_done, now_ms() - t_columns_done);
+    if (L.p.trace_level >= 1 && !opt.build_G) trace_blocks("learn_cd", m->device, blocks0);
     if ((opt.dbglvl & SLIM_DBG_PROGRESS) && model) print_progress(m, model, requested, cs, k);
 
     slimgpu_stats_t st = solve_stats(m, L, E, k, cs, requested, tnnz);
@@ -2691,7 +2727,7 @@
     const bool fresh = m->G_ready || m->ws_G.bytes() < G_bytes;
     if (fresh) {
       size_t free_b = 0, total_b = 0;
-      HIP_TRY(hipMemGetInfo(&free_b, &total_b));
+      HIP_TRY(device_mem_info(&free_b, &total_b));
       if (G_bytes + (size_t(8) << 30) > free_b + m->ws_G.bytes() + m->ws_gram.bytes()) {
         set_error("SLIMGPU_MatrixGramBuildRows: G = R^T R (4 ncols^2 bytes) does not fit the free HBM");
         return SLIM_ERROR_MEMORY;
diff --git a/slim_amd/csrc/engine.hpp b/slim_amd/csrc/engine.hpp
--- a/slim_amd/csrc/engine.hpp
+++ b/slim_amd/csrc/engine.hpp
@@ -84,6 +84,8 @@
                         int32_t* status, const int32_t* columns = nullptr, int32_t ncolumns = 0);
 
 int32_t device_count();
+int64_t device_cache_trim(int32_t device);
+slimgpu_cache_stats_t device_cache_stats(int32_t device);
 
 int32_t predict_device(const slim_csr_t* W, const slim_csr_t* hist, int32_t nrcmds,
                        int32_t* output, float* scores, int32_t* counts);
diff --git a/slim_amd/csrc/explain.hip b/slim_amd/csrc/explain.hip
--- a/slim_amd/csrc/explain.hip
+++ b/slim_amd/csrc/explain.hip
@@ -56,7 +56,7 @@
     E.allocs = 0;
     const size_t want = (size_t)entries * (places ? 8 * (size_t)nwhy + 4 : 4);
     size_t free_b = 0, total_b = 0;
-    HIP_TRY(hipMemGetInfo(&free_b, &total_b));
+    HIP_TRY(device_mem_info(&free_b, &total_b));
     if (want > (free_b + E.held()) / 2) {
       set_error(w + ": the outputs of " + std::to_string(entries) + " candidate entries at nwhy = " +
                 std::to_string(nwhy) + " need " + std::to_string(want) + " bytes of device memory, more than half of "
diff --git a/slim_amd/csrc/hip_check.hpp b/slim_amd/csrc/hip_check.hpp
--- a/slim_amd/csrc/hip_check.hpp
+++ b/slim_amd/csrc/hip_check.hpp
@@ -7,6 +7,7 @@
 #include <utility>
 
 #include "../../include/slim.h"
+#include "device_cache.hpp"
 
 namespace slimamd {
 
@@ -25,22 +26,71 @@
   return e.code == hipErrorOutOfMemory ? SLIM_ERROR_MEMORY : SLIM_ERROR;
 }
 
+namespace devcache {
+struct OnDevice {
+  int prev = -1;
+  bool switched = false;
+  explicit OnDevice(int device) {
+    if (hipGetDevice(&prev) == hipSuccess && prev != device) switched = hipSetDevice(device) == hipSuccess;
+  }
+  ~OnDevice() {
+    if (switched) (void)hipSetDevice(prev);
+  }
+};
+inline int hip_alloc(void*, int device, size_t bytes, void** out) {
+  OnDevice on(device);
+  const hipError_t e = hipMalloc(out, bytes);
+  if (e != hipSuccess) (void)hipGetLastError();
+  return (int)e;
+}
+inline int hip_free(void*, int, void* p) { return (int)hipFree(p); }
+inline int hip_sync(void*, int device) {
+  OnDevice on(device);
+  return (int)hipDeviceSynchronize();
+}
+inline int hip_mem_info(void*, int device, size_t* free_b, size_t* total_b) {
+  OnDevice on(device);
+  return (int)hipMemGetInfo(free_b, total_b);
+}
+}
+
+inline devcache::BlockCache& device_cache() {
+  static devcache::BlockCache* const cache = [] {
+    devcache::Backend b;
+    b.alloc = devcache::hip_alloc;
+    b.free_block = devcache::hip_free;
+    b.synchronize = devcache::hip_sync;
+    b.mem_info = devcache::hip_mem_info;
+    b.oom = (int)hipErrorOutOfMemory;
+    return new devcache::BlockCache(b);
+  }();
+  return *cache;
+}
+
+inline hipError_t device_mem_info(size_t* free_b, size_t* total_b) {
+  int device = 0;
+  const hipError_t e = hipGetDevice(&device);
+  if (e != hipSuccess) return e;
+  return (hipError_t)device_cache().mem_info(device, free_b, total_b);
+}
+
 template <class T>
 class DeviceBuffer {
  public:
   DeviceBuffer() = default;
   explicit DeviceBuffer(size_t n) {
-    HIP_TRY(hipMalloc(reinterpret_cast<void**>(&p), sizeof(T) * (n ? n : 1)));
-    bytes_ = sizeof(T) * (n ? n : 1);
+    const hipError_t e = take(sizeof(T) * (n ? n : 1), [] { return false; });
+    if (e != hipSuccess) throw HipFail{e, "hipMalloc(buffer)"};
   }
   ~DeviceBuffer() { reset(); }
   DeviceBuffer(DeviceBuffer&& o) noexcept
-      : p(std::exchange(o.p, nullptr)), bytes_(std::exchange(o.bytes_, 0)) {}
+      : p(std::exchange(o.p, nullptr)), bytes_(std::exchange(o.bytes_, 0)), device_(o.device_) {}
   DeviceBuffer& operator=(DeviceBuffer&& o) noexcept {
     if (this != &o) {
       reset();
       p = std::exchange(o.p, nullptr);
       bytes_ = std::exchange(o.bytes_, 0);
+      device_ = o.device_;
     }
     return *this;
   }
@@ -54,7 +104,7 @@
     return std::exchange(p, nullptr);
   }
   void reset() {
-    if (p) (void)hipFree(p);
+    if (p) device_cache().park(device_, p, bytes_);
     p = nullptr;
     bytes_ = 0;
   }
@@ -66,25 +116,29 @@
   T* reserve(size_t n, Evict&& evict) {
     const size_t need = sizeof(T) * (n ? n : 1);
     if (bytes_ >= need) return p;
-    if (p) HIP_TRY(hipFree(p));
-    p = nullptr;
-    bytes_ = 0;
-    hipError_t e = hipMalloc(reinterpret_cast<void**>(&p), need);
-    if (e == hipErrorOutOfMemory && evict()) {
-      (void)hipGetLastError();
-      e = hipMalloc(reinterpret_cast<void**>(&p), need);
-    }
-    if (e != hipSuccess) {
-      p = nullptr;
-      throw HipFail{e, "hipMalloc(workspace)"};
-    }
-    bytes_ = need;
+    reset();
+    const hipError_t e = take(need, evict);
+    if (e != hipSuccess) throw HipFail{e, "hipMalloc(workspace)"};
     return p;
   }
 
  private:
+  template <class Evict>
+  hipError_t take(size_t need, Evict&& evict) {
+    hipError_t e = hipGetDevice(&device_);
+    if (e != hipSuccess) return e;
+    void* q = nullptr;
+    size_t got = 0;
+    e = (hipError_t)device_cache().take(device_, need, &q, &got, [&evict] { return (bool)evict(); });
+    if (e != hipSuccess) return e;
+    p = static_cast<T*>(q);
+    bytes_ = got;
+    return hipSuccess;
+  }
+
   T* p = nullptr;
   size_t bytes_ = 0;
+  int device_ = 0;
 };
 
 }
diff --git a/slim_amd/csrc/slim_abi.cpp b/slim_amd/csrc/slim_abi.cpp
--- a/slim_amd/csrc/slim_abi.cpp
+++ b/slim_amd/csrc/slim_abi.cpp
@@ -1190,6 +1190,14 @@
   return SLIM_OK;
 }
 
+int64_t SLIMGPU_DeviceCacheTrim(int32_t device) { return device_cache_trim(device); }
+
+int32_t SLIMGPU_DeviceCacheStats(int32_t device, slimgpu_cache_stats_t* out) {
+  if (!out) return SLIM_ERROR_INPUT;
+  *out = device_cache_stats(device);
+  return SLIM_OK;
+}
+
 int32_t SLIMGPU_DeviceCount(void) { return device_count(); }
 
 const char* SLIMGPU_LastError(void) { return last_error(); }
diff --git a/slim_amd/csrc/topn.hip b/slim_amd/csrc/topn.hip
--- a/slim_amd/csrc/topn.hip
+++ b/slim_amd/csrc/topn.hip
@@ -384,7 +384,7 @@
     if (v >= 1) return (int32_t)std::min<long>(v, std::max(nusers, 1));
   }
   size_t free_b = 0, total_b = 0;
-  HIP_TRY(hipMemGetInfo(&free_b, &total_b));
+  HIP_TRY(device_mem_info(&free_b, &total_b));
   const size_t per_user = (size_t)nrcmds * (sizeof(int32_t) + sizeof(float)) + sizeof(int32_t);
   return (int32_t)std::max<size_t>(1, std::min<size_t>((size_t)std::max(nusers, 1), free_b / 4 / per_user));
 }
diff --git a/slim_amd/engine.py b/slim_amd/engine.py
--- a/slim_amd/engine.py
+++ b/slim_amd/engine.py
@@ -339,6 +339,16 @@
     st = _lib.ListStats()
     (lib or _lib.load()).SLIMGPU_LastListStats(C.byref(st))
     return st.as_dict()
+
+
+def device_cache_stats(device=-1, lib=None):
+    st = _lib.CacheStats()
+    (lib or _lib.load()).SLIMGPU_DeviceCacheStats(int(device), C.byref(st))
+    return st.as_dict()
+
+
+def device_cache_trim(device=-1, lib=None):
+    return int((lib or _lib.load()).SLIMGPU_DeviceCacheTrim(int(device)))
 
 
 def _wrap_rows(lib, M):
```

Result: no change. 2269 (median of 2 runs) (+1.0%).
